# alipbcs/ZetaRay

Measured on AMD Instinct MI355X. Metric: Mrays/s, higher is better.
Workload: dtype f32; 1 GPU; Cornell Box (cornell_emissive: 58 triangles, 2 emissive) 1920x1080, G-buffer + ReSTIR PT (K1 + K11-K16: initial candidates, temporal + spatial reconnection reuse, boiling suppression; 3 non-transmissive / 4 glossy-transmissive bounces, static camera); integrator=restir_pt, parallelism=screen tiles (1, 1), settle_frames=32, ramp_frames=357, arith=contract, library=libzetaray_amd.so, frame_overlap=True, kernel_class=plain

## Files before the change

### include/zetaray_amd.h

```cpp
#ifndef ZETARAY_AMD_H
#define ZETARAY_AMD_H

#include <stddef.h>
#include <stdint.h>
#include "zr_wire.h"

#ifdef __cplusplus
extern "C" {
#endif

#define ZR_ABI_VERSION 3

typedef enum zr_status {
    ZR_OK = 0,
    ZR_ERR_INVALID_ARG = 1,
    ZR_ERR_NO_DEVICE = 2,
    ZR_ERR_HIP = 3,
    ZR_ERR_OOM = 4,
    ZR_ERR_UNSUPPORTED = 5,
    ZR_ERR_NOT_INITIALIZED = 6
} zr_status;

typedef struct zr_scene   zr_scene;
typedef struct zr_gbuffer zr_gbuffer;
// ... 125 lines not shown
    uint32_t width, height;
    void*    plane[ZR_GB_COUNT];
} zr_gbuffer_planes;

typedef struct zr_counters {
    uint64_t n_closest;
    uint64_t n_shadow;
} zr_counters;

int         zr_abi_version(void);
const char* zr_last_error(void);
int         zr_device_count(int* count);
typedef struct zr_device_probe {
    char     name[64], arch[32];
    uint32_t compute_units, clock_khz_max, mem_clock_khz_max, mem_bus_bits, l2_bytes, wall_clock_khz;
    uint64_t hbm_bytes;
    float    copy_GBs, copy_ms;
    float    fma_tflops, fma_ms;
    float    sclk_mhz_under_load;
} zr_device_probe;
int         zr_device_probe_run(int device, float min_ms, zr_device_probe* out);
int         zr_wire_layout(char* buf, size_t cap);

int zr_scene_create(int device, const zr_scene_desc* desc, zr_scene** out);
int zr_scene_destroy(zr_scene* scene);
int zr_scene_update_instances(zr_scene* scene, const zr_mesh_instance* instances, const float* instance_to_world, uint32_t n);
int zr_scene_update_emissives(zr_scene* scene, const zr_emissive_triangle* triangles, uint32_t first, uint32_t count);
int zr_scene_update_instances_async(zr_scene* scene, void* hip_stream, const zr_mesh_instance* instances, const float* instance_to_world, uint32_t n);
int zr_scene_set_background_rebuild(zr_scene* scene, int enable);
int zr_scene_background_rebuild_stats(zr_scene* scene, uint64_t* started, uint64_t* installed, int* building);
int zr_scene_update_emissives_async(zr_scene* scene, void* hip_stream, const zr_emissive_triangle* triangles, uint32_t first, uint32_t count);
int zr_scene_update_materials_async(zr_scene* scene, void* hip_stream, const zr_material* materials, uint32_t first, uint32_t count);
int zr_scene_set_alias_table_async(zr_scene* scene, void* hip_stream, const zr_alias_entry* entries, uint32_t n);
int zr_scene_set_object_emissives(zr_scene* scene, const zr_emissive_triangle* object_space, uint32_t n);
int zr_scene_has_object_emissives(const zr_scene* scene);
int zr_scene_move_instances_async(zr_scene* scene, void* hip_stream, const uint32_t* instance_idx, const float* world_3x4, uint32_t n_moved);
int zr_scene_move_instances(zr_scene* scene, const uint32_t* instance_idx, const float* world_3x4, uint32_t n_moved);
int zr_scene_get_instances(const zr_scene* scene, void* hip_stream, int which, zr_mesh_instance* out, float* to_world_or_null, uint32_t n);
int zr_scene_get_emissives(const zr_scene* scene, void* hip_stream, zr_emissive_triangle* out, uint32_t first, uint32_t count);
int zr_scene_invalidate_alias_table(zr_scene* scene);
int zr_scene_invalidate_alias_table_deferred(zr_scene* scene);
int zr_scene_update_materials(zr_scene* scene, const zr_material* materials, uint32_t first, uint32_t count);
int zr_scene_set_alias_table(zr_scene* scene, const zr_alias_entry* entries, uint32_t n);
int zr_alias_table_build(const float* power, uint32_t n, uint32_t align_phase, zr_alias_entry* out_entries);
int zr_scene_get_alias_table(const zr_scene* scene, zr_alias_entry* out_entries, uint32_t n);
int zr_scene_get_light_voxel_grid(const zr_scene* scene, void* hip_stream, zr_voxel_sample* out_samples, uint32_t n);
int zr_scene_get_presampled_sets(const zr_scene* scene, void* hip_stream, zr_presampled_tri* out_samples, uint32_t n);
int zr_scene_bvh_info(const zr_scene* scene, uint32_t* num_nodes, uint32_t* num_tris, uint32_t* max_depth);

int zr_gbuffer_create(int device, uint32_t width, uint32_t height, zr_gbuffer** out);
int zr_gbuffer_destroy(zr_gbuffer* gb);
int zr_gbuffer_set_tile_origin(zr_gbuffer* gb, uint32_t x0, uint32_t y0);
int zr_gbuffer_download(const zr_gbuffer* gb, void* hip_stream, zr_gbuffer_planes* host_planes);
int zr_gbuffer_device_plane(const zr_gbuffer* gb, int plane, void** dev_ptr);

int zr_params_default(zr_params* p);
int zr_pass_create(int kind, int device, zr_pass** out);
int zr_pass_init(zr_pass* pass, uint32_t width, uint32_t height, int integrator);
int zr_pass_resize(zr_pass* pass, uint32_t width, uint32_t height);
int zr_pass_reset_temporal(zr_pass* pass);
int zr_pass_pick_pixel(zr_pass* pass, uint32_t x, uint32_t y);
int zr_pass_clear_pick(zr_pass* pass);
int zr_pass_read_pick(zr_pass* pass, void* stream, uint32_t* mesh_idx);
int zr_pass_set_params(zr_pass* pass, const zr_params* params);
int zr_pass_render(zr_pass* pass, void* hip_stream, const zr_frame_constants* cb, const zr_scene* scene,
                   zr_gbuffer* gbuffer);
#define ZR_STAGE_TEMPORAL 1
#define ZR_STAGE_SPATIAL  2
#define ZR_STAGE_ALL      3
#define ZR_STAGE_SPATIAL2 4
#define ZR_STAGE_CANDIDATES     8
#define ZR_STAGE_TEMPORAL_REUSE 16
#define ZR_STAGE_DENOISE_TEMPORAL  (1 << 8)
#define ZR_STAGE_DENOISE_VARIANCE  (1 << 9)
#define ZR_STAGE_DENOISE_ATROUS(i) (1u << (10 + (i)))
#define ZR_STAGE_DENOISE_MASK      0x3ff00
#define ZR_HALO_POST_TEMPORAL 0
#define ZR_HALO_FINAL         1
#define ZR_HALO_DENOISE_INPUT 2
#define ZR_HALO_DENOISE_ITER  3
#define ZR_HALO_BYTES_PER_PIXEL 62
int zr_pass_set_owned_rect(zr_pass* pass, uint32_t x0, uint32_t y0, uint32_t width, uint32_t height);
#define ZR_FRAME_OVERLAP       1
#define ZR_FRAME_OVERLAP_CARRY 2
int zr_pass_set_frame_overlap(zr_pass* pass, zr_gbuffer* gbuffer, int enable);
int zr_pass_frame_overlap_stream(zr_pass* pass, void** hip_stream);
int zr_device_synchronize(int device);
int zr_pass_halo_bytes_per_pixel(zr_pass* pass, uint32_t* bytes);
int zr_pass_render_stage(zr_pass* pass, void* hip_stream, const zr_frame_constants* cb, const zr_scene* scene,
                         zr_gbuffer* gbuffer, int stages);
int zr_pass_halo_pack(zr_pass* pass, void* hip_stream, const zr_gbuffer* gbuffer, int which, uint32_t x0, uint32_t y0,
                      uint32_t width, uint32_t height, void* dev_dst, size_t bytes);
int zr_pass_halo_unpack(zr_pass* pass, void* hip_stream, const zr_gbuffer* gbuffer, int which, uint32_t x0, uint32_t y0,
                        uint32_t width, uint32_t height, const void* dev_src, size_t bytes);
#define ZR_HALO_MAX_RECTS 16
typedef struct zr_halo_rect { uint32_t x0, y0, w, h; uint64_t offset; } zr_halo_rect;
int zr_pass_halo_pack_all(zr_pass* pass, void* hip_stream, const zr_gbuffer* gbuffer, int which, const zr_halo_rect* rects, uint32_t num_rects,
                          void* dev_buf, size_t bytes);
int zr_pass_halo_unpack_all(zr_pass* pass, void* hip_stream, const zr_gbuffer* gbuffer, int which, const zr_halo_rect* rects, uint32_t num_rects,
                            const void* dev_buf, size_t bytes);
int zr_pass_get_output(const zr_pass* pass, int which, void** dev_ptr, uint32_t* width, uint32_t* height,
                       uint32_t* bytes_per_pixel);
int zr_pass_download_output(const zr_pass* pass, int which, void* hip_stream, void* host_dst, size_t bytes);
#define ZR_IN_EMISSIVE_DI 0
#define ZR_IN_INDIRECT    1
#define ZR_IN_SKY_DI      2
#define ZR_IN_TAA_SIGNAL  3
#define ZR_IN_POST_SIGNAL_F16  4
#define ZR_IN_POST_SIGNAL_F32  5
#define ZR_IN_DISPLAY_EXPOSURE 6
#define ZR_IN_DENOISE_SIGNAL   7
int zr_pass_set_input(zr_pass* pass, int which, const void* dev_plane);
int zr_pass_set_inscattering(zr_pass* sky, int enable, uint32_t voxels_x, uint32_t voxels_y, float depth_map_exp, float near_z, float far_z);
int zr_pass_bind_inscattering(zr_pass* compositing, const zr_pass* sky);
#define ZR_OUT_INSCATTERING 49
#define ZR_INSCATTERING_VOXELS_X 192
#define ZR_INSCATTERING_VOXELS_Y 108
int zr_pass_set_tonemap_lut(zr_pass* pass, const uint32_t* rgb9e5, uint32_t dim);
enum zr_display_option
{
    ZR_DISPLAY_DEFAULT = 0,
    ZR_DISPLAY_BASE_COLOR,
    ZR_DISPLAY_NORMAL,
    ZR_DISPLAY_METALNESS_ROUGHNESS,
    ZR_DISPLAY_COAT_WEIGHT,
    ZR_DISPLAY_COAT_COLOR,
    ZR_DISPLAY_ROUGHNESS_TH,
    ZR_DISPLAY_EMISSIVE,
    ZR_DISPLAY_TRANSMISSION,
    ZR_DISPLAY_DEPTH,
    ZR_DISPLAY_COUNT
};
int zr_pass_set_display_option(zr_pass* pass, int option, float roughness_th);
typedef enum zr_rpt_debug_view
{
    ZR_RPT_VIEW_NONE = 0,
    ZR_RPT_VIEW_K,
    ZR_RPT_VIEW_CASE,
    ZR_RPT_VIEW_FOUND_CONNECTION,
    ZR_RPT_VIEW_LOBE_K_MIN_1,
    ZR_RPT_VIEW_LOBE_K,
    ZR_RPT_VIEW_COUNT
} zr_rpt_debug_view;
int zr_pass_set_rpt_debug_view(zr_pass* pass, int view);
int zr_pass_set_rgi_spatial(zr_pass* pass, uint32_t num_samples, float radius_px);
int zr_pass_set_picked_instances(zr_pass* pass, const uint32_t* mesh_idx, uint32_t n);
#define ZR_OUT_PICK_MASK 50
int zr_pass_read_counters(zr_pass* pass, void* hip_stream, zr_counters* out, int reset);
#define ZR_COST_MAP_TIME 1
#define ZR_COST_MAP_RAYS 2
int zr_pass_enable_cost_map(zr_pass* pass, int enable);
int zr_pass_read_cost_map(zr_pass* pass, void* hip_stream, uint32_t* out_cells, uint32_t cells_w, uint32_t cells_h, int reset);
int zr_pass_debug_trip_stats(zr_pass* pass, uint64_t out[3]);
int zr_debug_set_large_scene_nodes(uint32_t num_nodes);
int zr_debug_set_bvh_depth_cap(uint32_t levels);
int zr_debug_set_material_class_kernels(int enable);
int zr_scene_material_class(const zr_scene* scene, uint32_t* out_class);
int zr_pass_read_kernel_counters(zr_pass* pass, void* hip_stream, uint32_t max_entries, const char** names,
                                 uint64_t* n_closest, uint64_t* n_shadow, uint32_t* count);
int zr_selftest_half_conversions(int device, uint64_t* mismatches_f32_to_f16, uint64_t* mismatches_f16_to_f32);

int zr_pass_enable_timing(zr_pass* pass, int enable);
int zr_pass_get_timings(zr_pass* pass, uint32_t max_entries, const char** names, float* ms, uint32_t* launches,
                        uint32_t* count);
int zr_pass_destroy(zr_pass* pass);

int zr_trace_closest(const zr_scene* scene, void* hip_stream, const float* d_rays, uint32_t n, uint32_t mask,
                     uint32_t* d_hits);
int zr_trace_any(const zr_scene* scene, void* hip_stream, const float* d_rays, uint32_t n, uint32_t mask,
                 uint32_t* d_occluded);

#ifdef __cplusplus
}
#endif

#endif
```

### zetaray_amd/api.py

```python
import ctypes as C
import os

import numpy as np

from . import wire

_HERE = os.path.dirname(os.path.abspath(__file__))
LIB_PATH = os.environ.get("ZETARAY_AMD_LIB", os.path.join(_HERE, "libzetaray_amd.so"))

PASS_GBUFFER, PASS_PRELIGHTING, PASS_DI_EMISSIVE, PASS_DI_SKY, PASS_INDIRECT, PASS_COMPOSITING, PASS_SKY, PASS_TAA, PASS_AUTO_EXPOSURE, PASS_DISPLAY, PASS_DENOISE = range(11)
IN_TAA_SIGNAL, OUT_TAA = 3, 41
IN_POST_SIGNAL_F16, IN_POST_SIGNAL_F32, IN_DISPLAY_EXPOSURE = 4, 5, 6
OUT_EXPOSURE, OUT_AE_HISTOGRAM, OUT_DISPLAY, OUT_DISPLAY_SRGB8 = 42, 43, 44, 45
IN_DENOISE_SIGNAL, OUT_DENOISED, OUT_DENOISE_HISTORY, OUT_DENOISE_MOMENTS = 7, 46, 47, 48
TONEMAP_LUT_PATH = os.path.join(_HERE, "assets", "tony_mc_mapface_rgb9e5.bin")


def load_tonemap_lut():
    lut = np.fromfile(TONEMAP_LUT_PATH, np.uint32)
    assert lut.size == 48 ** 3, lut.size
    return lut

OUT_SKY_LUT = 40
IN_EMISSIVE_DI, IN_INDIRECT, IN_SKY_DI = range(3)
INTEGRATOR_PATH_TRACING, INTEGRATOR_RESTIR_GI, INTEGRATOR_RESTIR_PT = range(3)
OUT_FINAL = 0
RPT_OUTPUTS_EXTRA = {"denoised": (46, np.float32, 4), "denoise_history": (47, np.float32, 4), "denoise_moments": (48, np.float32, 2),
                     "taa": (41, np.uint16, 4), "sky_lut": (40, np.uint32, 1), "sdi_A": (24, np.uint8, 1), "sdi_B": (25, np.uint16, 2), "sdi_C": (26, np.float32, 2),
                     "sdi_target": (27, np.float32, 4)}
RPT_OUTPUTS = {"A": (1, np.uint32, 1), "B": (2, np.float32, 2), "C": (3, np.uint32, 4), "D": (4, np.uint32, 4),
               "E": (5, np.uint16, 1), "F": (6, np.float32, 2), "G": (7, np.uint32, 2), "target": (8, np.float32, 4),
               "neighbor": (9, np.uint8, 2), "map_ctn": (18, np.uint16, 1), "map_ntc": (19, np.uint16, 1),
               "ctn_A": (10, np.uint16, 4), "ctn_B": (11, np.uint32, 4), "ctn_C": (12, np.uint32, 4), "ctn_D": (13, np.uint16, 1),
               "gi_A": (30, np.float32, 4), "gi_B": (31, np.uint16, 4), "gi_C": (32, np.float32, 4),
               "di_A": (20, np.uint32, 4), "di_B": (21, np.float32, 2), "di_target": (22, np.float32, 4),
               "ntc_A": (14, np.uint16, 4), "ntc_B": (15, np.uint32, 4), "ntc_C": (16, np.uint32, 4), "ntc_D": (17, np.uint16, 1)}

EXPORTS = [
    "zr_abi_version", "zr_last_error", "zr_device_count", "zr_device_probe_run", "zr_wire_layout", "zr_scene_create", "zr_scene_destroy", "zr_scene_update_instances", "zr_scene_update_emissives", "zr_scene_invalidate_alias_table", "zr_scene_update_materials",
    "zr_scene_set_background_rebuild", "zr_scene_background_rebuild_stats",
    "zr_scene_invalidate_alias_table_deferred", "zr_scene_update_instances_async", "zr_scene_update_emissives_async", "zr_scene_update_materials_async", "zr_scene_set_alias_table_async",
    "zr_scene_set_alias_table", "zr_alias_table_build", "zr_scene_get_alias_table", "zr_scene_get_light_voxel_grid", "zr_scene_get_presampled_sets", "zr_scene_bvh_info", "zr_pass_enable_cost_map", "zr_pass_read_cost_map", "zr_pass_debug_trip_stats", "zr_debug_set_large_scene_nodes", "zr_debug_set_bvh_depth_cap", "zr_debug_set_material_class_kernels", "zr_scene_material_class",
    "zr_gbuffer_create", "zr_gbuffer_destroy", "zr_gbuffer_set_tile_origin", "zr_gbuffer_download", "zr_gbuffer_device_plane",
    "zr_params_default", "zr_pass_create", "zr_pass_init", "zr_pass_resize", "zr_pass_reset_temporal", "zr_pass_pick_pixel", "zr_pass_clear_pick", "zr_pass_read_pick",
    "zr_pass_set_params", "zr_pass_render", "zr_pass_get_output", "zr_pass_download_output",
    "zr_pass_read_counters", "zr_pass_read_kernel_counters", "zr_pass_enable_timing", "zr_pass_get_timings", "zr_selftest_half_conversions", "zr_pass_destroy",
    "zr_trace_closest", "zr_trace_any",
    "zr_pass_set_owned_rect", "zr_pass_render_stage", "zr_pass_halo_pack", "zr_pass_halo_unpack", "zr_pass_halo_bytes_per_pixel", "zr_pass_set_input",
    "zr_pass_set_tonemap_lut", "zr_pass_halo_pack_all", "zr_pass_halo_unpack_all",
    "zr_pass_set_frame_overlap", "zr_pass_frame_overlap_stream", "zr_device_synchronize",
    "zr_pass_set_inscattering", "zr_pass_bind_inscattering",
    "zr_pass_set_display_option", "zr_pass_set_picked_instances",
    "zr_pass_set_rpt_debug_view",
    "zr_pass_set_rgi_spatial",
    "zr_scene_set_object_emissives", "zr_scene_has_object_emissives", "zr_scene_move_instances", "zr_scene_move_instances_async", "zr_scene_get_instances", "zr_scene_get_emissives",
]
STAGE_TEMPORAL, STAGE_SPATIAL, STAGE_ALL = 1, 2, 3
STAGE_SPATIAL2 = 4
STAGE_CANDIDATES, STAGE_TEMPORAL_REUSE = 8, 16
HALO_POST_TEMPORAL, HALO_FINAL = 0, 1
HALO_DENOISE_INPUT, HALO_DENOISE_ITER = 2, 3
STAGE_DENOISE_TEMPORAL, STAGE_DENOISE_VARIANCE, STAGE_DENOISE_MASK = 1 << 8, 1 << 9, 0x3ff00


def stage_denoise_atrous(i):
    return 1 << (10 + i)


class ZetaRayError(RuntimeError):
    def __init__(self, code, msg):
        super().__init__(f"zetaray_amd error {code}: {msg}")
        self.code = code


_LIB = None


def lib():
    global _LIB
    if _LIB is None:
        if not os.path.exists(LIB_PATH):
            raise ImportError(f"{LIB_PATH} is missing: build the HIP extension first "
                              f"(python -c 'import __graft_entry__ as g; g.build()'); there is no fallback path")
        try:
            import torch
        except ImportError:
            pass
        L = C.CDLL(LIB_PATH)
        L.zr_last_error.restype = C.c_char_p
        vp, u32, i32 = C.c_void_p, C.c_uint32, C.c_int
        L.zr_device_count.argtypes = [vp]
        L.zr_scene_create.argtypes = [i32, vp, vp]
        L.zr_scene_destroy.argtypes = [vp]
        L.zr_scene_set_alias_table.argtypes = [vp, vp, u32]
        L.zr_alias_table_build.argtypes = [vp, u32, u32, vp]
        L.zr_scene_get_alias_table.argtypes = [vp, vp, u32]
        L.zr_scene_get_light_voxel_grid.argtypes = [vp, vp, vp, u32]
        L.zr_scene_get_presampled_sets.argtypes = [vp, vp, vp, u32]
        L.zr_scene_bvh_info.argtypes = [vp, vp, vp, vp]
        L.zr_gbuffer_create.argtypes = [i32, u32, u32, vp]
        L.zr_gbuffer_destroy.argtypes = [vp]
        L.zr_gbuffer_set_tile_origin.argtypes = [vp, u32, u32]
        L.zr_gbuffer_download.argtypes = [vp, vp, vp]
        L.zr_gbuffer_device_plane.argtypes = [vp, i32, vp]
        L.zr_params_default.argtypes = [vp]
        L.zr_pass_create.argtypes = [i32, i32, vp]
        L.zr_pass_init.argtypes = [vp, u32, u32, i32]
        L.zr_pass_resize.argtypes = [vp, u32, u32]
        L.zr_pass_reset_temporal.argtypes = [vp]
        L.zr_pass_set_params.argtypes = [vp, vp]
        L.zr_pass_render.argtypes = [vp, vp, vp, vp, vp]
        L.zr_pass_get_output.argtypes = [vp, i32, vp, vp, vp, vp]
        L.zr_pass_download_output.argtypes = [vp, i32, vp, vp, C.c_size_t]
        L.zr_pass_read_counters.argtypes = [vp, vp, vp, i32]
        L.zr_pass_read_kernel_counters.argtypes = [vp, vp, u32, vp, vp, vp, vp]
        L.zr_pass_set_input.argtypes = [vp, i32, vp]
        L.zr_pass_set_inscattering.argtypes = [vp, i32, u32, u32, C.c_float, C.c_float, C.c_float]
        L.zr_pass_bind_inscattering.argtypes = [vp, vp]
        L.zr_pass_set_tonemap_lut.argtypes = [vp, vp, u32]
        L.zr_pass_set_display_option.argtypes = [vp, i32, C.c_float]
        L.zr_pass_set_picked_instances.argtypes = [vp, vp, u32]
        L.zr_pass_set_rpt_debug_view.argtypes = [vp, i32]
        L.zr_pass_set_rgi_spatial.argtypes = [vp, u32, C.c_float]
        L.zr_pass_halo_pack_all.argtypes = [vp, vp, vp, i32, vp, u32, vp, C.c_size_t]
        L.zr_pass_halo_unpack_all.argtypes = [vp, vp, vp, i32, vp, u32, vp, C.c_size_t]
        L.zr_pass_set_owned_rect.argtypes = [vp, u32, u32, u32, u32]
        L.zr_pass_render_stage.argtypes = [vp, vp, vp, vp, vp, i32]
        L.zr_pass_halo_pack.argtypes = [vp, vp, vp, i32, u32, u32, u32, u32, vp, C.c_size_t]
        L.zr_pass_halo_bytes_per_pixel.argtypes = [vp, vp]
        L.zr_pass_halo_unpack.argtypes = [vp, vp, vp, i32, u32, u32, u32, u32, vp, C.c_size_t]
        L.zr_pass_enable_timing.argtypes = [vp, i32]
        L.zr_pass_get_timings.argtypes = [vp, u32, vp, vp, vp, vp]
        L.zr_pass_destroy.argtypes = [vp]
        L.zr_pass_set_frame_overlap.argtypes = [vp, vp, i32]
        L.zr_pass_frame_overlap_stream.argtypes = [vp, vp]
        L.zr_device_synchronize.argtypes = [i32]
        L.zr_trace_closest.argtypes = [vp, vp, vp, u32, u32, vp]
        L.zr_trace_any.argtypes = [vp, vp, vp, u32, u32, vp]
        _LIB = L
    return _LIB


def _check(code):
    if code != 0:
        raise ZetaRayError(code, lib().zr_last_error().decode())


def device_count():
    n = C.c_int(0)
    _check(lib().zr_device_count(C.byref(n)))
    return n.value


def alias_table_build(power, align_phase=0):
    power = np.ascontiguousarray(power, np.float32)
    out = np.zeros(len(power), wire.ALIAS_ENTRY)
    _check(lib().zr_alias_table_build(power.ctypes.data, len(power), align_phase, out.ctypes.data))
    return out


class Scene:
    def __init__(self, scene, device=0):
        self.host = scene
        self._desc = scene.desc()
        self.h = C.c_void_p()
        self.version = 0
        self.instances_in_motion = self._records_in_motion(getattr(scene, "instances", None))
        _check(lib().zr_scene_create(device, C.addressof(self._desc), C.byref(self.h)))

    @staticmethod
    def _records_in_motion(instances):
        if instances is None or len(instances) == 0:
            return False
        i = np.asarray(instances)
        return bool(((i["d_translation"] & 0x7fff) != 0).any() or (i["prev_rotation"] != i["rotation"]).any() or (i["prev_scale"] != i["scale"]).any())

    def update_instances(self, instances, instance_to_world, stream=False):
        L = lib()
        self.version += 1
        i, x = np.ascontiguousarray(instances), np.ascontiguousarray(instance_to_world, np.float32)
        self.instances_in_motion = self._records_in_motion(i)
        if stream is False:
            L.zr_scene_update_instances.argtypes = [C.c_void_p, C.c_void_p, C.c_void_p, C.c_uint32]
            _check(L.zr_scene_update_instances(self.h, i.ctypes.data, x.ctypes.data, len(i)))
        else:
            L.zr_scene_update_instances_async.argtypes = [C.c_void_p, C.c_void_p, C.c_void_p, C.c_void_p, C.c_uint32]
            _check(L.zr_scene_update_instances_async(self.h, stream, i.ctypes.data, x.ctypes.data, len(i)))

    def set_object_emissives(self, tris):
        L = lib()
        t = np.ascontiguousarray(tris, wire.EMISSIVE_TRI)
        L.zr_scene_set_object_emissives.argtypes = [C.c_void_p, C.c_void_p, C.c_uint32]
        _check(L.zr_scene_set_object_emissives(self.h, t.ctypes.data, len(t)))

    def move_instances(self, idx, world, stream=False):
# ... 139 lines not shown

class Pass:

    def __init__(self, kind, width, height, integrator=INTEGRATOR_PATH_TRACING, device=0, params=None):
        self.kind = kind
        self.w, self.h_ = width, height
        self.h = C.c_void_p()
        _check(lib().zr_pass_create(kind, device, C.byref(self.h)))
        _check(lib().zr_pass_init(self.h, width, height, integrator))
        if params is not None:
            self.set_params(params)

    def set_params(self, params):
        _check(lib().zr_pass_set_params(self.h, C.addressof(params)))

    def resize(self, width, height):
        _check(lib().zr_pass_resize(self.h, width, height))
        self.w, self.h_ = width, height

    def reset_temporal(self):
        _check(lib().zr_pass_reset_temporal(self.h))

    def pick_pixel(self, x, y):
        L = lib()
        L.zr_pass_pick_pixel.argtypes = [C.c_void_p, C.c_uint32, C.c_uint32]
        _check(L.zr_pass_pick_pixel(self.h, int(x), int(y)))

    def clear_pick(self):
        L = lib()
        L.zr_pass_clear_pick.argtypes = [C.c_void_p]
        _check(L.zr_pass_clear_pick(self.h))

    def read_pick(self, stream=None):
        L = lib()
        L.zr_pass_read_pick.argtypes = [C.c_void_p, C.c_void_p, C.c_void_p]
        out = C.c_uint32(0)
        _check(L.zr_pass_read_pick(self.h, stream, C.byref(out)))
        return int(out.value)

    def render(self, cb, scene, gbuffer=None, stream=None):
        cbb = np.ascontiguousarray(cb)
        _check(lib().zr_pass_render(self.h, stream, cbb.ctypes.data, scene.h, gbuffer.h if gbuffer is not None else None))

    def render_stage(self, cb, scene, gbuffer, stages, stream=None):
        cbb = np.ascontiguousarray(cb)
        _check(lib().zr_pass_render_stage(self.h, stream, cbb.ctypes.data, scene.h, gbuffer.h if gbuffer is not None else None, stages))

    def set_input(self, which, dev_ptr):
        _check(lib().zr_pass_set_input(self.h, which, dev_ptr))

    def set_frame_overlap(self, gbuffer, on=1):
        _check(lib().zr_pass_set_frame_overlap(self.h, gbuffer.h, int(on)))

    def frame_overlap_stream(self):
        st = C.c_void_p()
        _check(lib().zr_pass_frame_overlap_stream(self.h, C.byref(st)))
        return st.value

    def set_tonemap_lut(self, lut=None):
        lut = np.ascontiguousarray(load_tonemap_lut() if lut is None else lut, np.uint32)
        dim = int(round(lut.size ** (1.0 / 3.0)))
        _check(lib().zr_pass_set_tonemap_lut(self.h, lut.ctypes.data, dim))

    def set_display_option(self, option, roughness_th=wire.DISPLAY_ROUGHNESS_TH_DEFAULT):
        _check(lib().zr_pass_set_display_option(self.h, int(option), float(roughness_th)))

    def set_rpt_debug_view(self, view):
        _check(lib().zr_pass_set_rpt_debug_view(self.h, int(view)))

    def set_rgi_spatial(self, num_samples, radius_px=0.0):
        _check(lib().zr_pass_set_rgi_spatial(self.h, int(num_samples), float(radius_px)))

    def set_picked_instances(self, mesh_idx):
        a = np.ascontiguousarray(mesh_idx, np.uint32).reshape(-1)
        _check(lib().zr_pass_set_picked_instances(self.h, a.ctypes.data if a.size else None, a.size))

    def download_raw(self, which, dtype, shape, stream=None):
        out = np.zeros(shape, dtype)
        _check(lib().zr_pass_download_output(self.h, which, stream, out.ctypes.data, out.nbytes))
        return out

    def set_owned_rect(self, x0, y0, w, h):
        _check(lib().zr_pass_set_owned_rect(self.h, x0, y0, w, h))

    def halo_pack(self, gbuffer, which, rect, dev_ptr, nbytes, stream=None):
        _check(lib().zr_pass_halo_pack(self.h, stream, gbuffer.h, which, rect[0], rect[1], rect[2], rect[3], dev_ptr, nbytes))

    def halo_all(self, gbuffer, which, rects, dev_ptr, nbytes, pack=True, stream=None):
        class Rect(C.Structure):
            _fields_ = [("x0", C.c_uint32), ("y0", C.c_uint32), ("w", C.c_uint32), ("h", C.c_uint32), ("offset", C.c_uint64)]
        arr = (Rect * max(1, len(rects)))(*[Rect(*r) for r in rects])
        f = lib().zr_pass_halo_pack_all if pack else lib().zr_pass_halo_unpack_all
        _check(f(self.h, stream, gbuffer.h, which, arr, len(rects), dev_ptr, nbytes))

    def halo_bytes_per_pixel(self):
        b = C.c_uint32()
        _check(lib().zr_pass_halo_bytes_per_pixel(self.h, C.byref(b)))
        return b.value

    def halo_unpack(self, gbuffer, which, rect, dev_ptr, nbytes, stream=None):
        _check(lib().zr_pass_halo_unpack(self.h, stream, gbuffer.h, which, rect[0], rect[1], rect[2], rect[3], dev_ptr, nbytes))

    def output_ptr(self, which=OUT_FINAL):
        dev = C.c_void_p()
        w, h, bpp = C.c_uint32(), C.c_uint32(), C.c_uint32()
        _check(lib().zr_pass_get_output(self.h, which, C.byref(dev), C.byref(w), C.byref(h), C.byref(bpp)))
        return dev.value, w.value, h.value, bpp.value

    def download(self, which=OUT_FINAL, stream=None):
        out = np.zeros((self.h_, self.w, 4), np.float32)
        _check(lib().zr_pass_download_output(self.h, which, stream, out.ctypes.data, out.nbytes))
        return out

    def set_inscattering(self, enable=True, voxels=wire.INSCATTERING_VOXELS, depth_map_exp=wire.INSCATTERING_DEPTH_MAP_EXP,
                         near_z=wire.INSCATTERING_NEAR_Z, far_z=wire.INSCATTERING_FAR_Z):
        _check(lib().zr_pass_set_inscattering(self.h, int(enable), int(voxels[0]), int(voxels[1]), float(depth_map_exp), float(near_z), float(far_z)))

    def bind_inscattering(self, sky_pass):
        _check(lib().zr_pass_bind_inscattering(self.h, sky_pass.h if sky_pass is not None else None))

    def download_plane(self, name, stream=None):
        if name == "pick_mask":
            _, w, h, _ = self.output_ptr(wire.OUT_PICK_MASK)
            out = np.zeros((h, w), np.uint8)
            _check(lib().zr_pass_download_output(self.h, wire.OUT_PICK_MASK, stream, out.ctypes.data, out.nbytes))
            return out
        if name == "inscattering":
            _, w, h, _ = self.output_ptr(wire.OUT_INSCATTERING)
            out = np.zeros((wire.INSCATTERING_SLICES, h // wire.INSCATTERING_SLICES, w), np.uint32)
            _check(lib().zr_pass_download_output(self.h, wire.OUT_INSCATTERING, stream, out.ctypes.data, out.nbytes))
            return out
        which, dt, ch = RPT_OUTPUTS[name] if name in RPT_OUTPUTS else RPT_OUTPUTS_EXTRA[name]
        out = np.zeros((self.h_, self.w, ch), dt)
        _check(lib().zr_pass_download_output(self.h, which, stream, out.ctypes.data, out.nbytes))
        return out

    def enable_cost_map(self, on=True):
        lib().zr_pass_enable_cost_map.argtypes = [C.c_void_p, C.c_int]
        _check(lib().zr_pass_enable_cost_map(self.h, int(on)))

    def read_cost_map(self, reset=True, stream=None):
        cw, ch = (self.w + 31) // 32 + 1, (self.h_ + 31) // 32 + 1
        out = np.zeros((ch, cw), np.uint32)
        lib().zr_pass_read_cost_map.argtypes = [C.c_void_p, C.c_void_p, C.c_void_p, C.c_uint32, C.c_uint32, C.c_int]
        _check(lib().zr_pass_read_cost_map(self.h, stream, out.ctypes.data, cw, ch, int(reset)))
        return out

    def debug_trip_stats(self):
        out = (C.c_uint64 * 3)()
        lib().zr_pass_debug_trip_stats.argtypes = [C.c_void_p, C.c_void_p]
        _check(lib().zr_pass_debug_trip_stats(self.h, out))
        return int(out[0]), int(out[1]), int(out[2])

    def read_counters(self, reset=True, stream=None):
        c = wire.Counters()
        _check(lib().zr_pass_read_counters(self.h, stream, C.addressof(c), int(reset)))
        return c.n_closest, c.n_shadow

    def kernel_counters(self, stream=None):
        n = 16
        names = (C.c_char_p * n)()
        a = (C.c_uint64 * n)()
        b = (C.c_uint64 * n)()
        cnt = C.c_uint32()
        _check(lib().zr_pass_read_kernel_counters(self.h, stream, n, names, a, b, C.byref(cnt)))
        return {names[i].decode(): (a[i], b[i]) for i in range(cnt.value)}

    def enable_timing(self, on=True):
        _check(lib().zr_pass_enable_timing(self.h, int(on)))

    def timings(self):
        n = 64
        names = (C.c_char_p * n)()
        ms = (C.c_float * n)()
        launches = (C.c_uint32 * n)()
        cnt = C.c_uint32()
        _check(lib().zr_pass_get_timings(self.h, n, names, ms, launches, C.byref(cnt)))
        return {names[i].decode(): (ms[i], launches[i]) for i in range(min(cnt.value, n))}

    def close(self):
        if self.h:
            lib().zr_pass_destroy(self.h)
            self.h = C.c_void_p()

    def __del__(self):
        try:
            self.close()
        except Exception:
            pass


class Renderer:

    def __init__(self, scene_host, width, height, device=0, params=None, integrator=INTEGRATOR_PATH_TRACING,
                 tile_origin=(0, 0)):
        self.scene = Scene(scene_host, device)
        self.scene_host = scene_host
        self.gbuffer = GBuffer(width, height, device)
        if tile_origin != (0, 0):
            self.gbuffer.set_tile_origin(*tile_origin)
        self.p_gbuffer = Pass(PASS_GBUFFER, width, height, device=device)
        self.p_prelight = Pass(PASS_PRELIGHTING, width, height, device=device, params=params)
        self._presampling = bool(params is not None and params.presampling)
        self.p_indirect = Pass(PASS_INDIRECT, width, height, integrator, device=device, params=params)
        self.p_sky = Pass(PASS_SKY, 256, 128, device=device) if len(scene_host.emissives) == 0 else None
        self.p_direct = None
        self.p_sky_direct = None
        self.skip_indirect = False
        self.p_composit = None
        self._alias_ready = False
        self._overlap_stream = None
        self._inscattering = False
        self._device = device

    def enable_frame_overlap(self, on=True, carry=False):
        assert self.p_direct is None and self.p_sky_direct is None and self.p_composit is None and getattr(self, "p_taa", None) is None, \
            "frame overlap covers GBuffer + PreLighting + Indirect (ReSTIR PT) [+ denoise]"
        _check(lib().zr_device_synchronize(self._device))
        self.p_indirect.set_frame_overlap(self.gbuffer, (2 if carry else 1) if on else 0)
        self._overlap_stream = self.p_indirect.frame_overlap_stream() if on else None

    def enable_compositing(self, device=0, firefly_filter=False):
        prm = None
        if firefly_filter:
            prm = wire.default_params()
            prm.flags |= wire.COMPOSIT_FIREFLY_FILTER
        self.p_composit = Pass(PASS_COMPOSITING, self.p_indirect.w, self.p_indirect.h_, device=device, params=prm)
        self._bind_post_inputs()
        return self.p_composit

    def enable_inscattering(self, voxels=wire.INSCATTERING_VOXELS, depth_map_exp=wire.INSCATTERING_DEPTH_MAP_EXP, near_z=wire.INSCATTERING_NEAR_Z,
                            far_z=wire.INSCATTERING_FAR_Z, device=0):
        assert self._overlap_stream is None, "frame overlap covers GBuffer + PreLighting + Indirect (ReSTIR PT) [+ denoise]"
        if self.p_sky is None:
            self.p_sky = Pass(PASS_SKY, 256, 128, device=device)
        self.p_sky.set_inscattering(True, voxels, depth_map_exp, near_z, far_z)
        if self.p_composit is None:
            self.enable_compositing(device=device)
        self.p_composit.bind_inscattering(self.p_sky)
        self._inscattering = True
        return self.p_sky

    def _bind_post_inputs(self):
        if self.p_composit is None:
            return
        self.p_composit.set_input(IN_INDIRECT, None if self.skip_indirect else self.p_indirect.output_ptr()[0])
        self.p_composit.set_input(IN_EMISSIVE_DI, self.p_direct.output_ptr()[0] if self.p_direct is not None else None)
        self.p_composit.set_input(IN_SKY_DI, self.p_sky_direct.output_ptr()[0] if self.p_sky_direct is not None else None)
        if getattr(self, "p_taa", None) is not None:
            self.p_taa.set_input(IN_TAA_SIGNAL, self.p_composit.output_ptr()[0])

    def enable_denoise(self, params=None, device=0):
        self.p_denoise = Pass(PASS_DENOISE, self.p_indirect.w, self.p_indirect.h_, device=device, params=params or wire.default_params())
        self.p_denoise.set_input(IN_DENOISE_SIGNAL, self.p_indirect.output_ptr()[0])
        return self.p_denoise

    def enable_taa(self, blend_weight=0.1, device=0):
        if self.p_composit is None:
            self.enable_compositing(device=device)
        prm = wire.default_params()
        prm.taa_blend_weight = blend_weight
        self.p_taa = Pass(PASS_TAA, self.p_indirect.w, self.p_indirect.h_, device=device, params=prm)
        self._bind_post_inputs()
        return self.p_taa

    def enable_sky_direct(self, params=None, device=0):
        if self.p_sky is None:
            self.p_sky = Pass(PASS_SKY, 256, 128, device=device)
        self.p_sky_direct = Pass(PASS_DI_SKY, self.p_indirect.w, self.p_indirect.h_, device=device, params=params)
        self._bind_post_inputs()
        return self.p_sky_direct

    def enable_direct(self, params=None, device=0):
        self.p_direct = Pass(PASS_DI_EMISSIVE, self.p_indirect.w, self.p_indirect.h_, device=device, params=params)
        self._bind_post_inputs()
        return self.p_direct

    def invalidate_alias_table(self, deferred=False):
        if deferred:
            self.scene.invalidate_alias_table_deferred()
            self._alias_poll = 8
            return
        self.scene.invalidate_alias_table()
        self._alias_ready = False

    def move_instances(self, idx, world, stream=False):
        self.scene.move_instances(idx, world, stream=stream)

    def set_rgi_spatial(self, num_samples, radius_px=0.0):
        self.p_indirect.set_rgi_spatial(num_samples, radius_px)

    _SKY_FIELDS = ("sun_dir", "sun_illuminance", "planet_radius", "atmosphere_altitude", "g", "rayleigh_sigma_s_color", "rayleigh_sigma_s_scale",
                   "ozone_sigma_a_color", "ozone_sigma_a_scale", "mie_sigma_s", "mie_sigma_a")

    def render_sky(self, cb, stream=None):
        if self.p_sky is None:
            return
        key = b"".join(np.asarray(cb[f]).tobytes() for f in self._SKY_FIELDS)
        if not self._inscattering:
            if key != getattr(self, "_sky_key", None):
                self.p_sky.render(cb, self.scene, None, stream)
                self._sky_key = key
            return
        if key != getattr(self, "_sky_key", None):
            self.p_sky.render_stage(cb, self.scene, None, STAGE_TEMPORAL, stream)
            self._sky_key = key
# ... 57 lines not shown
```

### zetaray_amd/csrc/zr_api.hip

```cpp
#include <hip/hip_runtime.h>
#include <immintrin.h>
#include <string>
#include <vector>
#include <cstdio>
#include <cstdarg>
#include <cstring>
#include <new>
#include <mutex>
#include "zr_stages.h"
#include "zr_rpt.h"
#include "zr_rdi.h"
#include "zr_sdi.h"
#include "zr_rgi.h"
#include "zr_rgi_spatial.h"
#include "zr_bvh.h"
#include "zr_taa.h"
#include "zr_svgf.h"
#include "zr_post.h"
#include "../../include/zr_srgb_table.h"

static const uint16_t kRptSampleSet[1024] = {
#include "zr_rpt_sample_set.inc"
};

// ... 598 lines not shown
    bool plainAt[3] = {true, true, true};
    uint64_t sceneAt[3] = {0, 0, 0};
    bool tracked = false;
    hipEvent_t evWritten = nullptr; hipStream_t writer = nullptr; bool hasWrite = false;
    struct Reader { hipStream_t st; hipEvent_t ev; };
    std::vector<Reader> readers[3];
    ~zr_gbuffer() { if (evWritten) (void)hipEventDestroy(evWritten); for (auto& v : readers) for (auto& r : v) (void)hipEventDestroy(r.ev); }
    DevBuf<uint8_t>* Planes() { return planeSets[cur]; }
    const DevBuf<uint8_t>* Planes() const { return planeSets[cur]; }
    GBuf View() const { return ViewOf(cur); }
    GBuf PrevView() const { return ViewOf(Prev()); }
    GBuf ViewOf(int which) const
    {
        const DevBuf<uint8_t>* planes = planeSets[which];
        GBuf g; g.w = w; g.h = h; g.x0 = x0; g.y0 = y0;
        g.baseColor = (uint32_t*)planes[ZR_GB_BASE_COLOR].p; g.normal = (uint32_t*)planes[ZR_GB_NORMAL].p;
        g.mr = (uint16_t*)planes[ZR_GB_METALLIC_ROUGHNESS].p; g.motion = (uint32_t*)planes[ZR_GB_MOTION_VECTOR].p;
        g.emissive = (uint32_t*)planes[ZR_GB_EMISSIVE_COLOR].p; g.ior = (uint8_t*)planes[ZR_GB_IOR].p;
        g.coat = (uint16_t*)planes[ZR_GB_COAT].p; g.depth = (float*)planes[ZR_GB_DEPTH].p;
        g.triA = (uint32_t*)planes[ZR_GB_TRI_DIFF_GEO_A].p; g.triB = (uint32_t*)planes[ZR_GB_TRI_DIFF_GEO_B].p;
        return g;
    }
};

static int GBufferMarkRead(zr_gbuffer* gb, int set, hipStream_t s)
{
    if (!gb || !gb->tracked) return ZR_OK;
    for (auto& r : gb->readers[set]) if (r.st == s) { HIP_TRY(hipEventRecord(r.ev, s)); return ZR_OK; }
    hipEvent_t ev; HIP_TRY(hipEventCreateWithFlags(&ev, hipEventDisableTiming));
    gb->readers[set].push_back({s, ev});
    HIP_TRY(hipEventRecord(ev, s));
    return ZR_OK;
}
static int GBufferAcquireRead(zr_gbuffer* gb, hipStream_t s)
{
    if (!gb || !gb->tracked || !gb->hasWrite || gb->writer == s) return ZR_OK;
    HIP_TRY(hipStreamWaitEvent(s, gb->evWritten, 0));
    return ZR_OK;
}
static int GBufferAcquireWrite(zr_gbuffer* gb, int set, hipStream_t s)
{
    if (!gb->tracked) return ZR_OK;
    for (auto& r : gb->readers[set]) if (r.st != s) HIP_TRY(hipStreamWaitEvent(s, r.ev, 0));
    return ZR_OK;
}
static int GBufferMarkWritten(zr_gbuffer* gb, hipStream_t s)
{
    if (!gb->tracked) return ZR_OK;
    if (!gb->evWritten) HIP_TRY(hipEventCreateWithFlags(&gb->evWritten, hipEventDisableTiming));
    HIP_TRY(hipEventRecord(gb->evWritten, s));
    gb->writer = s; gb->hasWrite = true;
    return ZR_OK;
}

struct QueueStorage
{
    DevBuf<U4> s0; DevBuf<F4> f[8]; DevBuf<F4> rays[6]; DevBuf<uint32_t> lightID; DevBuf<U4> hitC, hitM; DevBuf<uint32_t> visS, rayList;
    DevBuf<F4> t[8];
    int AllocTex(size_t cap)
    {
        int r;
        for (auto& b : t) if (b.n != cap && (r = b.Alloc(cap))) return r;
        return ZR_OK;
    }
    int Alloc(size_t cap)
    {
        int r;
        if ((r = s0.Alloc(cap))) return r;
        for (auto& b : f) if ((r = b.Alloc(cap))) return r;
        for (auto& b : rays) if ((r = b.Alloc(cap))) return r;
        if ((r = lightID.Alloc(cap))) return r;
        if ((r = hitC.Alloc(cap))) return r;
        if ((r = hitM.Alloc(cap))) return r;
        if ((r = visS.Alloc(cap))) return r;
        if ((r = rayList.Alloc(3 * cap))) return r;
        return ZR_OK;
    }
    PathQueue View() const
    {
        PathQueue q;
        q.s0 = s0.p; q.s1 = f[0].p; q.s2 = f[1].p; q.s3 = f[2].p; q.s4 = f[3].p; q.s5 = f[4].p; q.s6 = f[5].p; q.s7 = f[6].p; q.s8 = f[7].p;
        q.rayC_o = rays[0].p; q.rayC_d = rays[1].p; q.rayM_o = rays[2].p; q.rayM_d = rays[3].p; q.rayS_o = rays[4].p; q.rayS_d = rays[5].p;
        q.sLightID = lightID.p; q.hitC = hitC.p; q.hitM = hitM.p; q.visS = visS.p; q.rayList = rayList.p;
        for (int k = 0; k < 8; k++) q.t[k] = t[k].p;
        return q;
    }
};

static constexpr uint32_t kRptListWords = 12;
static constexpr uint32_t kLargeSceneNodes = 1;
static std::atomic<uint32_t> g_largeSceneNodes{kLargeSceneNodes};
static std::atomic<bool> g_materialClassKernels{true};
static bool PlainClass(const zr_scene* sc, const zr_gbuffer* gb)
{
    if (!sc->plainMaterials.load(std::memory_order_relaxed) || !g_materialClassKernels.load(std::memory_order_relaxed)) return false;
    const int c = gb->cur;
    if (!(gb->plainAt[c] && gb->sceneAt[c] == sc->uid)) return false;
    if (gb->numRendered >= 2 && !(gb->plainAt[gb->Prev()] && gb->sceneAt[gb->Prev()] == sc->uid)) return false;
    return true;
}
static constexpr int kMaxRounds = 16;
static constexpr int kMaxTimers = 64;
static constexpr int kCounterSlots = 16;
static const char* const kCounterNames[kCounterSlots] = {"trace", "rpt_pathtrace", "rpt_replay_ctt", "rpt_replay_ttc", "rpt_reconnect_temporal",
    "rpt_replay_cts", "rpt_replay_stc", "rpt_reconnect_spatial", "rdi_temporal", "rdi_spatial", "rgi", "sdi_temporal", "sdi_spatial", "rgi_spatial", "", ""};

struct zr_pass
{
    int kind = 0, device = 0, integrator = 0;
    bool initialized = false;
    uint32_t w = 0, h = 0;
    zr_params params{};
    QueueStorage q[2];
    DevBuf<uint32_t> skyLut;
    bool inscatterOn = false; InscatterParams inscatter{}; DevBuf<uint32_t> inscatterGrid;
    const zr_pass* inscatterSky = nullptr;
    Plane<float, 4> finalRGBA; Plane<F4> firstBOP; DevBuf<uint32_t> counts; DevBuf<unsigned long long> counters;
    DevBuf<uint32_t> groupMax;
    zr_counters hostCounters{0, 0};
    uint32_t pickXY = 0xffffffffu; DevBuf<uint32_t> pickBuf; bool pickWritten = false;
    struct ResStorage
    {
        Plane<uint32_t> A; Plane<float, 2> B; Plane<U4> C, D; Plane<uint16_t> E; Plane<float, 2> F; Plane<uint32_t, 2> G;
        template<typename S, typename Fn> static int Each(S& s, Fn f)
        { int r; if ((r = f(s.A)) || (r = f(s.B)) || (r = f(s.C)) || (r = f(s.D)) || (r = f(s.E)) || (r = f(s.F)) || (r = f(s.G))) return r; return ZR_OK; }
        rpt::ResPlanes View() const { rpt::ResPlanes v; v.A = A.p; v.B = B.p; v.C = C.p; v.D = D.p; v.E = E.p; v.F = F.p; v.G = G.p; return v; }
    } res[3];
    struct RBufStorage
    {
        Plane<uint16_t, 4> A; Plane<U4> B, C; Plane<uint16_t> D;
        template<typename S, typename Fn> static int Each(S& s, Fn f) { int r; if ((r = f(s.A)) || (r = f(s.B)) || (r = f(s.C)) || (r = f(s.D))) return r; return ZR_OK; }
        rpt::RBuf View() const { rpt::RBuf v; v.A = A.p; v.B = B.p; v.C = C.p; v.D = D.p; return v; }
    } rb[2];
    Plane<F4> rptTarget, rptTargetAlt; Plane<uint8_t, 2> rptNeighbor; DevBuf<uint16_t> rptSampleSet;
    bool overlap = false, overlapCarry = false; int rptSet[3] = {0, 1, 2}; int tgtIdx = 0, finIdx = 0, finOut = 0;
    Plane<float, 4> finalAlt, finalAlt2;
    hipEvent_t evDone[2] = {nullptr, nullptr}; bool haveDone[2] = {false, false}; hipStream_t doneStream[2] = {nullptr, nullptr}; uint64_t ovFrame = 0;
    hipStream_t overlapStream = nullptr;
    hipEvent_t evCand = nullptr, evTemporal = nullptr;
    hipStream_t candStream = nullptr, reuseStream = nullptr; bool haveCand = false, haveTemporal = false;
    zr_pass::ResStorage& RptCur() { return res[rptSet[currIdx]]; }
    zr_pass::ResStorage& RptOth() { return res[rptSet[1 - currIdx]]; }
    const zr_pass::ResStorage& RptOth() const { return res[rptSet[1 - currIdx]]; }
    const Plane<F4>& TargetPlane() const { return tgtIdx ? rptTargetAlt : rptTarget; }
    const Plane<float, 4>& FinalPlane(int i) const { return i == 0 ? finalRGBA : (i == 1 ? finalAlt : finalAlt2); }
    F4* Target() const { return TargetPlane().p; }
    float* Final(int i) const { return FinalPlane(i).p; }
    Plane<uint16_t> rptMap[2];
    DevBuf<uint32_t> trip; DevBuf<unsigned long long> tripStats;
    DevBuf<uint32_t> carry[2], carryCount;
    bool frameOpen = false;
    DevBuf<uint32_t> costMap; bool costOn = false, costRays = false;
    DevBuf<uint32_t> rptLists, rptListCounts;
    Plane<U4> diA[2]; Plane<float, 2> diB[2]; Plane<F4> diTarget; DevBuf<uint16_t> diSampleSet;
    Plane<uint8_t> skyA[2]; Plane<uint16_t, 2> skyB[2]; Plane<float, 2> skyC[2];
    Plane<F4> giA[2], giC[2]; Plane<uint16_t, 4> giB[2];
    bool temporalValid = false, doTemporal = false, doSpatial = false; int currIdx = 0;
    const F4* compIn[4] = {nullptr, nullptr, nullptr, nullptr};
    Plane<F4> svgfHist, svgfAccum, svgfPing, svgfPong; Plane<float, 2> svgfMoments[2]; Plane<float> svgfGuideFw; Plane<svgf::GuideN> svgfGuide; int svgfMomIdx = 0; const F4* svgfOut = nullptr; F4* svgfCur = nullptr; uint32_t svgfStepsDone = 0;
    Plane<uint16_t, 4> taaOut[2]; int taaIdx = 0;
    const uint16_t* postIn16 = nullptr; const F4* postIn32 = nullptr; const float* exposureIn = nullptr;
    DevBuf<uint32_t> aeHist; DevBuf<float> aeExposure;
    DevBuf<uint32_t> tonemapLut; uint32_t tonemapLutDim = 0; Plane<F4> displayOut; Plane<uint32_t> displaySrgb;
    int displayOption = ZR_DISPLAY_DEFAULT; float roughnessTh = 1.0f;
    int rptView = ZR_RPT_VIEW_NONE, rptViewFrame = ZR_RPT_VIEW_NONE;
    rgi::SpatialParams rgiSpatial{0u, rgi::kSpatialDefaultRadius}, rgiSpatialFrame{0u, rgi::kSpatialDefaultRadius}; Plane<float, 4> rgiScratch;
    std::vector<uint32_t> picks; DevBuf<uint8_t> pickMask; DevBuf<int4> pickTris; DevBuf<uint32_t> pickCount;
    uint32_t pickMaskW = 0, pickMaskH = 0;
    uint32_t own[4] = {0, 0, 0, 0};
    DevBuf<float> power;
    float* powerHost = nullptr; size_t powerHostCap = 0; hipEvent_t powerEv = nullptr; bool powerPending = false;
    bool timing = false;
    struct Timer { const char* name; hipEvent_t a, b; bool used; };
    std::vector<Timer> timers;
    int numTimers = 0;
    std::vector<std::string> timerNames; std::vector<float> timerMs; std::vector<uint32_t> timerLaunches;
};

static void TimerBegin(zr_pass* p, hipStream_t s, const char* name)
{
    if (!p->timing) return;
    if (p->numTimers >= (int)p->timers.size())
    {
        zr_pass::Timer t; t.name = name; t.used = false;
        if (hipEventCreate(&t.a) != hipSuccess || hipEventCreate(&t.b) != hipSuccess) return;
        p->timers.push_back(t);
    }
    zr_pass::Timer& t = p->timers[p->numTimers];
    t.name = name; t.used = true;
    (void)hipEventRecord(t.a, s);
}
static void TimerEnd(zr_pass* p, hipStream_t s)
{
    if (!p->timing) return;
    if (p->numTimers >= (int)p->timers.size()) return;
    (void)hipEventRecord(p->timers[p->numTimers].b, s);
    p->numTimers++;
}

static float KahanSumAVX2(const float* data, int64_t N, int64_t phase)
{
    float sum = 0.0f, compensation = 0.0f;
    const int64_t start = phase < N ? phase : N;
    for (int64_t i = 0; i < start; i++)
    {
        volatile float corrected = data[i] - compensation;
        volatile float newSum = sum + corrected;
        compensation = (newSum - sum) - corrected;
        sum = newSum;
    }
    int64_t numSimd = (N - start);
    numSimd -= numSimd & 15;
    __m256 vSum = _mm256_setzero_ps(), vComp = _mm256_setzero_ps();
    for (int64_t c = start; c < start + numSimd; c += 16)
    {
        __m256 V1 = _mm256_loadu_ps(data + c), V2 = _mm256_loadu_ps(data + c + 8);
        __m256 vCurr = _mm256_add_ps(V1, V2);
        __m256 vCorrected = _mm256_sub_ps(vCurr, vComp);
        __m256 vNewSum = _mm256_add_ps(vSum, vCorrected);
        vComp = _mm256_sub_ps(vNewSum, vSum);
        vComp = _mm256_sub_ps(vComp, vCorrected);
        vSum = vNewSum;
    }
    alignas(32) float simdSum[8], simdComp[8];
    _mm256_store_ps(simdSum, vSum); _mm256_store_ps(simdComp, vComp);
    for (int i = 0; i < 8; i++)
    {
        volatile float corrected = simdSum[i] - compensation - simdComp[i];
        volatile float newSum = sum + corrected;
        compensation = (newSum - sum) - corrected;
        sum = newSum;
    }
    for (int64_t i = start + numSimd; i < N; i++)
    {
        volatile float corrected = data[i] - compensation;
        volatile float newSum = sum + corrected;
        compensation = (newSum - sum) - corrected;
        sum = newSum;
    }
    return sum;
}

static void BuildAliasTableHost(std::vector<float>& probs, zr_alias_entry* table, uint32_t phase)
{
    const int64_t N = (int64_t)probs.size();
    const float oneDivN = 1.0f / (float)N;
    const float sum = KahanSumAVX2(probs.data(), N, phase);
    const float sumRcp = (float)N / sum;
    for (int64_t i = 0; i < N; i++) probs[i] *= sumRcp;
    for (int64_t i = 0; i < N; i++) { table[i].cached_p_orig = probs[i] * oneDivN; table[i].alias = 0xffffffffu; table[i].p_curr = 0.0f; }
    std::vector<uint32_t> larger, smaller;
    larger.reserve(N); smaller.reserve(N);
    for (int64_t i = 0; i < N; i++) (probs[i] < 1.0f ? smaller : larger).push_back((uint32_t)i);
    while (!smaller.empty() && !larger.empty())
    {
        const uint32_t si = smaller.back(); smaller.pop_back();
        const float sp = probs[si];
        const uint32_t li = larger.back();
        float lp = probs[li];
        table[si].alias = li; table[si].p_curr = sp;
        lp = (sp + lp) - 1.0f;
        probs[li] = lp;
        if (lp < 1.0f) { larger.pop_back(); smaller.push_back(li); }
    }
    for (; !larger.empty(); larger.pop_back()) { table[larger.back()].alias = larger.back(); table[larger.back()].p_curr = 1.0f; }
    for (; !smaller.empty(); smaller.pop_back()) { table[smaller.back()].alias = smaller.back(); table[smaller.back()].p_curr = 1.0f; }
    for (int64_t i = 0; i < N; i++) table[i].cached_p_alias = table[table[i].alias].cached_p_orig;
}

__global__ void __launch_bounds__(256) k_refit_tris(BvhTri* tris, uint32_t n, const TriMeta* meta, const zr_mesh_instance* instances, const float* toWorld,
    const zr_vertex* vertices, const uint32_t* indices)
{
    const uint32_t i = blockIdx.x * blockDim.x + threadIdx.x;
    if (i >= n) return;
    BvhTri t = tris[i];
    const TriMeta tm = meta[t.gidx];
    const zr_mesh_instance mi = instances[tm.mesh];
    const float* M = toWorld + 12 * (size_t)tm.mesh;
    float w[3][3];
    for (int k = 0; k < 3; k++)
    {
        const uint32_t vi = indices[mi.base_idx_offset + 3 * tm.prim + k] + mi.base_vtx_offset;
        const float* P = vertices[vi].pos;
        for (int r = 0; r < 3; r++) w[k][r] = M[4 * r + 0] * P[0] + M[4 * r + 1] * P[1] + M[4 * r + 2] * P[2] + M[4 * r + 3];
    }
    for (int r = 0; r < 3; r++) { t.v0[r] = w[0][r]; t.e1[r] = w[1][r] - w[0][r]; t.e2[r] = w[2][r] - w[0][r]; }
    tris[i] = t;
}
__global__ void __launch_bounds__(256) k_install_topology(Bvh4Node* nodes, const uint32_t* children, uint32_t numNodes, BvhTri* tris, const uint32_t* slotTri, uint32_t numTris,
    const TriMeta* meta, const uint8_t* instanceMask)
{
    const uint32_t i = blockIdx.x * blockDim.x + threadIdx.x;
    if (i < numNodes)
    {
        const uint4 c = ((const uint4*)children)[i];
        Bvh4Node N; N.ox = N.oy = N.oz = 0.0f; N.exps = 0; N.child[0] = c.x; N.child[1] = c.y; N.child[2] = c.z; N.child[3] = c.w;
        N.qlox = N.qloy = N.qloz = N.qhix = N.qhiy = N.qhiz = 0; N.pad0 = 0; N.pad1 = 0;
        nodes[i] = N;
    }
    if (i < numTris)
    {
        const uint32_t g = slotTri[i];
        const TriMeta tm = meta[g];
        BvhTri t; for (int r = 0; r < 3; r++) { t.v0[r] = 0.0f; t.e1[r] = 0.0f; t.e2[r] = 0.0f; }
        t.gidx = g; t.mask = instanceMask[tm.mesh]; t.id = TriID(tm.mesh, tm.prim);
        tris[i] = t;
// ... 1356 lines not shown
        TimerBegin(p, s, "sdi_spatial");
        hipLaunchKernelGGL(plainDi ? k_sdi_spatial<true> : k_sdi_spatial<false>, dim3(grid.x * (256 / kSdiBlock)), dim3(kSdiBlock), 0, s, F, *cb, tilesX, p->counters.p + 2 * 12);
        TimerEnd(p, s);
    }
    HIP_TRY(hipGetLastError());
    p->temporalValid = true;
    p->currIdx = 1 - p->currIdx;
    return ZR_OK;
}

static int RenderReSTIR_GI(zr_pass* p, hipStream_t s, const zr_frame_constants* cb, const zr_scene* sc, zr_gbuffer* gb, int stages)
{
    using namespace rgi;
    const zr_params& ip = p->params;
    GiFrame F;
    F.sc = FrameView(sc, cb); F.gb = gb->View(); F.gbPrev = gb->PrevView();
    F.sc.texFilter = ip.tex_filter;
    if (int orc = ResolveOwnedRect(p, gb, cb, &F.ox0, &F.oy0, &F.ow, &F.oh)) return orc;
    GiParams& prm = F.prm;
    prm.flags = ip.flags; prm.maxNonTrBounces = ip.max_non_tr_bounces; prm.maxGlossyTrBounces = ip.max_glossy_tr_bounces;
    prm.numSampleSets = ip.presampling ? ip.num_sample_sets : 0u;
    prm.accumulate = (cb->accumulate && cb->camera_static) ? 1u : 0u;
    prm.M_max = (float)ip.m_max_temporal;
    prm.useLVG = (ip.use_lvg && ip.presampling) ? 1u : 0u;
    prm.textured = sc->view.tex.count ? 1u : 0u;
    const uint32_t tilesX = (F.ow + 15) / 16, tilesY = (F.oh + 15) / 16;
    if (stages & ZR_STAGE_TEMPORAL)
    {
        p->rgiSpatialFrame = p->rgiSpatial;
        const bool spatial = p->rgiSpatialFrame.numSamples != 0;
        F.cur.A = p->giA[p->currIdx].p; F.cur.B = p->giB[p->currIdx].p; F.cur.C = p->giC[p->currIdx].p;
        F.prev.A = p->giA[1 - p->currIdx].p; F.prev.B = p->giB[1 - p->currIdx].p; F.prev.C = p->giC[1 - p->currIdx].p;
        F.finalRGBA = p->finalRGBA.p;
        prm.doTemporal = ((ip.flags & ZR_IND_TEMPORAL_RESAMPLE) && p->temporalValid && gb->numRendered >= 2) ? 1u : 0u;
        prm.writeReservoirs = (prm.doTemporal || !p->temporalValid) ? 1u : 0u;
        if (spatial)
        {
            const size_t cap = (size_t)p->w * p->h;
            if (p->rgiScratch.Pixels() != cap) { int r; if ((r = p->rgiScratch.Alloc(cap))) return r; HIP_TRY(hipMemsetAsync(p->rgiScratch.p, 0, cap * p->rgiScratch.bpp, s)); }
            F.finalRGBA = p->rgiScratch.p; prm.accumulate = 0u; prm.writeReservoirs = 1u;
        }
        if (prm.useLVG && !sc->view.lvg) return Fail(ZR_ERR_NOT_INITIALIZED, "light voxel grid missing: render the PRELIGHTING pass with use_lvg first");
        TimerBegin(p, s, "rgi");
        hipLaunchKernelGGL(sc->view.tex.count ? k_rgi_tex : PlainClass(sc, gb) ? k_rgi<true> : k_rgi<false>, dim3(tilesX * tilesY * (256 / kRgiBlock)), dim3(kRgiBlock), 0, s, F, *cb, tilesX, p->counters.p + 2 * 10);
        TimerEnd(p, s);
        HIP_TRY(hipGetLastError());
        p->temporalValid = true;
        p->currIdx = 1 - p->currIdx;
    }
    if ((stages & ZR_STAGE_SPATIAL) && p->rgiSpatialFrame.numSamples != 0)
    {
        if (!p->temporalValid) return Fail(ZR_ERR_NOT_INITIALIZED, "ReSTIR GI: ZR_STAGE_SPATIAL before the frame's ZR_STAGE_TEMPORAL");
        const int set = 1 - p->currIdx;
        F.cur.A = p->giA[set].p; F.cur.B = p->giB[set].p; F.cur.C = p->giC[set].p; F.prev = F.cur;
        F.finalRGBA = p->finalRGBA.p;
        prm.accumulate = (cb->accumulate && cb->camera_static) ? 1u : 0u;
        prm.doTemporal = 0u; prm.writeReservoirs = 0u; prm.textured = 0u;
        TimerBegin(p, s, "rgi_spatial");
        hipLaunchKernelGGL(k_rgi_spatial, dim3(tilesX * tilesY), dim3(kBlock), 0, s, F, *cb, tilesX, p->counters.p + 2 * 13, p->rgiSpatialFrame);
        TimerEnd(p, s);
        HIP_TRY(hipGetLastError());
    }
    return ZR_OK;
}

__global__ void __launch_bounds__(256) k_rpt_carry(rpt::ResPlanes dst, rpt::ResPlanes src, F4* tdst, const F4* tsrc, size_t n)
{
    for (size_t i = (size_t)blockIdx.x * blockDim.x + threadIdx.x; i < n; i += (size_t)gridDim.x * blockDim.x)
    {
        dst.A[i] = src.A[i]; dst.B[2 * i] = src.B[2 * i]; dst.B[2 * i + 1] = src.B[2 * i + 1]; dst.C[i] = src.C[i]; dst.D[i] = src.D[i]; dst.E[i] = src.E[i];
        dst.F[2 * i] = src.F[2 * i]; dst.F[2 * i + 1] = src.F[2 * i + 1]; dst.G[2 * i] = src.G[2 * i]; dst.G[2 * i + 1] = src.G[2 * i + 1];
        tdst[i] = tsrc[i];
    }
}
static bool FewerRoundsAtFourWaves(uint32_t waves)
{
    static const bool off = [] { const char* e = ZR_EXP_ENV("ZR_K11_ROUNDS"); return e && !strcmp(e, "0"); }();
    return !off && waves > 3072u && waves <= 4096u;
}

static int RenderReSTIR_PT(zr_pass* p, hipStream_t s, const zr_frame_constants* cb, const zr_scene* sc, zr_gbuffer* gb, int stages)
{
    using namespace rpt;
    const zr_pass::ResStorage* carryFrom = nullptr;
    const bool stageCand = (stages & (ZR_STAGE_TEMPORAL | ZR_STAGE_CANDIDATES)) != 0, stageReuseT = (stages & (ZR_STAGE_TEMPORAL | ZR_STAGE_TEMPORAL_REUSE)) != 0;
    if (stageCand && p->overlap)
    {
        if (!gb->tracked || gb->numSets < 3) return Fail(ZR_ERR_INVALID_ARG, "ReSTIR PT with frame overlap: this G-buffer is not the one given to zr_pass_set_frame_overlap (call it again with the new G-buffer)");
        if (p->frameOpen) return Fail(ZR_ERR_INVALID_ARG, "ReSTIR PT with frame overlap: the previous frame's last stage has not been enqueued (stage order: CANDIDATES, TEMPORAL_REUSE, SPATIAL[, SPATIAL2])");
        std::swap(p->rptSet[p->currIdx], p->rptSet[2]);
        p->tgtIdx ^= 1;
        carryFrom = p->overlapCarry ? &p->res[p->rptSet[2]] : nullptr;
        if (!(cb->accumulate && cb->camera_static)) p->finIdx = (p->finIdx + 1) % 3;
        if (p->overlapCarry)
        {
            if (p->haveTemporal && p->reuseStream != s) HIP_TRY(hipStreamWaitEvent(s, p->evTemporal, 0));
        }
        else
        {
            const int k = (int)(p->ovFrame & 1);
            if (p->haveDone[k] && p->doneStream[k] != s) HIP_TRY(hipStreamWaitEvent(s, p->evDone[k], 0));
        }
    }
    RptFrame F;
    F.sc = FrameView(sc, cb); F.gb = gb->View(); F.gbPrev = gb->PrevView();
    F.scPrev = FrameViewPrev(sc, cb);
    F.sc.texFilter = F.scPrev.texFilter = p->params.tex_filter;
    if (int orc = ResolveOwnedRect(p, gb, cb, &F.ox0, &F.oy0, &F.ow, &F.oh)) return orc;
    F.rbCtN = p->rb[0].View(); F.rbNtC = p->rb[1].View(); F.tex.target = p->Target(); F.tex.neighbor = p->rptNeighbor.p;
    F.finalRGBA = p->Final(p->finIdx); F.sampleSet = p->rptSampleSet.p;
    F.mapCtN = p->rptMap[0].p; F.mapNtC = p->rptMap[1].p;
    F.costMap = p->costOn ? p->costMap.p : nullptr; F.costW = (p->w + 31u) / 32u + 1u; F.costMode = p->costRays ? 1u : 0u;
    F.trip = nullptr; F.tripStats = nullptr; F.tripStride = 0;
    F.carryOut = nullptr; F.carryIn = nullptr; F.carryCount = nullptr; F.carryCap = 0; F.carryBounce = 0;
    if (((F.ox0 + F.ow) & 31u) && F.ox0 + F.ow != cb->render_width) return Fail(ZR_ERR_INVALID_ARG, "ReSTIR PT: the owned rect must end on a 32-pixel boundary or at the right edge of the render target");
    if (((F.oy0 + F.oh) & 31u) && F.oy0 + F.oh != cb->render_height) return Fail(ZR_ERR_INVALID_ARG, "ReSTIR PT: the owned rect must end on a 32-pixel boundary or at the bottom edge of the render target");
    RptParams& prm = F.prm;
    const zr_params& ip = p->params;
    const bool havePrevGBuffer = gb->numRendered >= 2;
    prm.maxNonTrBounces = ip.max_non_tr_bounces; prm.maxGlossyTrBounces = ip.max_glossy_tr_bounces;
    prm.russianRoulette = (ip.flags & ZR_IND_RUSSIAN_ROULETTE) ? 1u : 0u;
    prm.numSampleSets = ip.presampling ? ip.num_sample_sets : 0u;
    prm.accumulate = (cb->accumulate && cb->camera_static) ? 1u : 0u;
    prm.boiling = (ip.flags & ZR_IND_BOILING_SUPPRESSION) ? 1u : 0u;
    prm.M_max_temporal = ip.m_max_temporal & 0xf; prm.M_max_spatial = ip.m_max_spatial & 0xf; prm.alpha_min = ip.alpha_min;
    prm.emissive = cb->num_emissive_triangles ? 1u : 0u;
    prm.textured = sc->view.tex.count ? 1u : 0u;
    prm.sortTemporal = (ip.flags & ZR_IND_SORT_TEMPORAL) ? 1u : 0u; prm.sortSpatial = (ip.flags & ZR_IND_SORT_SPATIAL) ? 1u : 0u;
    static const uint32_t temporalMapEnv = [] { const char* e = ZR_EXP_ENV("ZR_TEMPORAL_MAP"); return e ? (uint32_t)atoi(e) : 1u; }();
    prm.temporalMap = prm.sortTemporal ? temporalMapEnv : 0u;
    if (stageCand)
    {
        p->rptViewFrame = p->rptView;
        p->doTemporal = (ip.flags & ZR_IND_TEMPORAL_RESAMPLE) && p->temporalValid && havePrevGBuffer;
        p->doSpatial = (ip.flags & ZR_IND_SPATIAL_RESAMPLE) && p->doTemporal && ip.num_spatial_passes > 0;
    }
    if (ip.num_spatial_passes > 2u) return Fail(ZR_ERR_INVALID_ARG, "ReSTIR PT: num_spatial_passes must be 0, 1 or 2");
    const uint32_t numSpatialPasses = ip.num_spatial_passes;
    prm.doTemporal = p->doTemporal ? 1u : 0u;
    prm.doSpatial = p->doSpatial ? 1u : 0u;
    prm.writeReservoirs = (prm.doTemporal || !p->temporalValid) ? 1u : 0u;
    F.cur = p->RptCur().View(); F.prev = p->RptOth().View();
    const uint32_t tilesX = (F.ow + 15) / 16, tilesY = (F.oh + 15) / 16;
    const dim3 grid(tilesX * tilesY), block(kBlock);
    const dim3 gridRpt(tilesX * tilesY * (256 / kRptBlock)), blockRpt(kRptBlock);
    const dim3 gridRecon(tilesX * tilesY * (256 / kReconBlock)), blockRecon(kReconBlock);
    const dim3 gridStc(tilesX * tilesY * (256 / kStcBlock)), blockStc(kStcBlock);
    const uint32_t sortTilesX = (F.ow + 31) / 32;
    const dim3 gridSort(sortTilesX * ((F.oh + 31) / 32));
    uint32_t* listCnt = p->rptListCounts.p;
    const size_t cap = (size_t)p->w * p->h;
    uint32_t* lists[4] = {p->rptLists.p, p->rptLists.p + cap, p->rptLists.p + 2 * cap, p->rptLists.p + 3 * cap};
    const dim3 gridList((uint32_t)std::min<size_t>((cap + kBlock - 1) / kBlock, 1024));
    const dim3 gridLight((tilesX * tilesY + kLightTilesPerBlock - 1u) / kLightTilesPerBlock), gridSearch((tilesX * tilesY + kSearchTilesPerBlock - 1u) / kSearchTilesPerBlock);
    const dim3 gridReplay((uint32_t)std::min<size_t>((cap + kBlock - 1) / kBlock, kReplayPersistentBlocks));
    unsigned long long* ctr = p->counters.p;
#define RPT_TIMED(name, ...) do { TimerBegin(p, s, name); __VA_ARGS__; TimerEnd(p, s); } while (0)
    const bool emissiveVariant = prm.emissive != 0;
    const uint32_t largeSceneNodes = g_largeSceneNodes.load(std::memory_order_relaxed);
    const bool texVariant = prm.textured != 0;
    const bool plainVariant = PlainClass(sc, gb) && !texVariant;
#define RPT_LAUNCH_E(kern, ...) do { \
        if (plainVariant) { if (emissiveVariant) hipLaunchKernelGGL((kern<true, false, true>), __VA_ARGS__); else hipLaunchKernelGGL((kern<false, false, true>), __VA_ARGS__); } \
        else if (emissiveVariant) { if (texVariant) hipLaunchKernelGGL((kern<true, true, false>), __VA_ARGS__); else hipLaunchKernelGGL((kern<true, false, false>), __VA_ARGS__); } \
        else { if (texVariant) hipLaunchKernelGGL((kern<false, true, false>), __VA_ARGS__); else hipLaunchKernelGGL((kern<false, false, false>), __VA_ARGS__); } } while (0)
#define RPT_LAUNCH_PE(kern, PASS, ...) do { \
        if (emissiveVariant) { if (texVariant) hipLaunchKernelGGL((kern<PASS, true, true>), __VA_ARGS__); else hipLaunchKernelGGL((kern<PASS, true, false>), __VA_ARGS__); } \
        else { if (texVariant) hipLaunchKernelGGL((kern<PASS, false, true>), __VA_ARGS__); else hipLaunchKernelGGL((kern<PASS, false, false>), __VA_ARGS__); } } while (0)
    const uint32_t view = (uint32_t)p->rptViewFrame;
#define RPT_LAUNCH_VIEW(kern, ...) do { \
        if (emissiveVariant) { if (texVariant) hipLaunchKernelGGL((kern<true, true>), __VA_ARGS__, view); else hipLaunchKernelGGL((kern<true, false>), __VA_ARGS__, view); } \
        else { if (texVariant) hipLaunchKernelGGL((kern<false, true>), __VA_ARGS__, view); else hipLaunchKernelGGL((kern<false, false>), __VA_ARGS__, view); } } while (0)
    if (stageCand)
    {
        if (int ar = GBufferAcquireRead(gb, s)) return ar;
        if (carryFrom)
        {
            const size_t n = (size_t)p->w * p->h;
            RPT_TIMED("rpt_overlap_carry", hipLaunchKernelGGL(k_rpt_carry, dim3((uint32_t)std::min<size_t>((n + 255) / 256, 4096)), dim3(256), 0, s, F.cur, carryFrom->View(), p->Target(),
                (const F4*)(p->tgtIdx ? p->rptTarget.p : p->rptTargetAlt.p), n));
        }
        TimerBegin(p, s, "rpt_pathtrace");
        if (view != ZR_RPT_VIEW_NONE) RPT_LAUNCH_VIEW(k_rpt_pathtrace_view, gridRpt, blockRpt, 0, s, F, *cb, tilesX, ctr + 2 * 1);
        else
        {
#ifdef ZR_EXPERIMENTS
        static const int k11Mode = [] { const char* e = getenv("ZR_K11"); return e && !strcmp(e, "inline") ? 0 : (e && !strcmp(e, "pool") ? 1 : (e && !strcmp(e, "trip") ? 2 : (e && !strcmp(e, "compact") ? 3 : ZR_K11_DEFAULT))); }();
        static const bool park = [] { const char* e = getenv("ZR_K11_PARK"); return e ? atoi(e) != 0 : (ZR_K11_PARK_DEFAULT != 0); }();
        if (k11Mode == 1 && emissiveVariant && !texVariant)
        {
            const dim3 gridCoop(tilesX * tilesY), blockCoop(kCoopBlock);
            if (sc->view.numNodes >= largeSceneNodes) hipLaunchKernelGGL(k_rpt_pathtrace_coop_w4<false>, gridCoop, blockCoop, 0, s, F, *cb, tilesX, ctr + 2 * 1);
            else hipLaunchKernelGGL(k_rpt_pathtrace_coop<false>, gridCoop, blockCoop, 0, s, F, *cb, tilesX, ctr + 2 * 1);
        }
        else if (k11Mode == 3 && !texVariant)
        {
            const size_t cap = (size_t)F.gb.w * F.gb.h;
            if (p->carry[0].n != cap * rpt::kPtCarryWords) { int rr; for (int k = 0; k < 2; k++) if ((rr = p->carry[k].Alloc(cap * rpt::kPtCarryWords))) return rr; if ((rr = p->carryCount.Alloc(16))) return rr; }
            HIP_TRY(hipMemsetAsync(p->carryCount.p, 0, 16 * sizeof(uint32_t), s));
            uint32_t maxB = prm.maxNonTrBounces > prm.maxGlossyTrBounces ? prm.maxNonTrBounces : prm.maxGlossyTrBounces;
            if (prm.russianRoulette && maxB > 3u) maxB = 3u;
            F.carryCap = cap; F.carryCount = p->carryCount.p; F.carryBounce = 0; F.carryOut = p->carry[0].p; F.carryIn = nullptr;
            if (emissiveVariant) hipLaunchKernelGGL(k_rpt_pt_first<true>, gridRpt, blockRpt, 0, s, F, *cb, tilesX, ctr + 2 * 1);
            else hipLaunchKernelGGL(k_rpt_pt_first<false>, gridRpt, blockRpt, 0, s, F, *cb, tilesX, ctr + 2 * 1);
            const dim3 gridNext((uint32_t)((cap + kRptBlock - 1) / kRptBlock));
            for (uint32_t b = 1; b + 1 <= maxB && b < 15u; b++)
            {
                F.carryBounce = b; F.carryIn = p->carry[(b - 1) & 1].p; F.carryOut = p->carry[b & 1].p;
                if (emissiveVariant) hipLaunchKernelGGL(k_rpt_pt_next<true>, gridNext, blockRpt, 0, s, F, *cb, tilesX, ctr + 2 * 1);
                else hipLaunchKernelGGL(k_rpt_pt_next<false>, gridNext, blockRpt, 0, s, F, *cb, tilesX, ctr + 2 * 1);
            }
        }
        else if (k11Mode == 2 && emissiveVariant && !texVariant)
        {
            const size_t stride = (size_t)F.gb.w * F.gb.h;
            if (!p->trip.p) { int rr; if ((rr = p->trip.Alloc(stride * rpt::kPtCarryWords))) return rr; if ((rr = p->tripStats.Alloc(4))) return rr; HIP_TRY(hipMemsetAsync(p->tripStats.p, 0, 32, s)); }
            F.trip = p->trip.p; F.tripStats = p->tripStats.p; F.tripStride = stride;
            if (sc->view.numNodes >= largeSceneNodes) hipLaunchKernelGGL(k_rpt_pathtrace_trip_w4<false>, gridRpt, blockRpt, 0, s, F, *cb, tilesX, ctr + 2 * 1);
            else hipLaunchKernelGGL(k_rpt_pathtrace_trip<false>, gridRpt, blockRpt, 0, s, F, *cb, tilesX, ctr + 2 * 1);
        }
        else if (k11Mode == 0 && park && !texVariant && !(sc->view.numNodes >= largeSceneNodes || FewerRoundsAtFourWaves(gridRpt.x)))
        { if (emissiveVariant) hipLaunchKernelGGL(k_rpt_pathtrace_park<true>, gridRpt, blockRpt, 0, s, F, *cb, tilesX, ctr + 2 * 1); else hipLaunchKernelGGL(k_rpt_pathtrace_park<false>, gridRpt, blockRpt, 0, s, F, *cb, tilesX, ctr + 2 * 1); }
        else
#endif
        if (texVariant) { if (emissiveVariant) hipLaunchKernelGGL(k_rpt_pathtrace_tex<true>, gridRpt, blockRpt, 0, s, F, *cb, tilesX, ctr + 2 * 1); else hipLaunchKernelGGL(k_rpt_pathtrace_tex<false>, gridRpt, blockRpt, 0, s, F, *cb, tilesX, ctr + 2 * 1); }
        else if (sc->view.numNodes >= largeSceneNodes || FewerRoundsAtFourWaves(gridRpt.x))
        {
            if (plainVariant) { if (emissiveVariant) hipLaunchKernelGGL((k_rpt_pathtrace_w4<true, true>), gridRpt, blockRpt, 0, s, F, *cb, tilesX, ctr + 2 * 1); else hipLaunchKernelGGL((k_rpt_pathtrace_w4<false, true>), gridRpt, blockRpt, 0, s, F, *cb, tilesX, ctr + 2 * 1); }
            else if (emissiveVariant) hipLaunchKernelGGL((k_rpt_pathtrace_w4<true, false>), gridRpt, blockRpt, 0, s, F, *cb, tilesX, ctr + 2 * 1); else hipLaunchKernelGGL((k_rpt_pathtrace_w4<false, false>), gridRpt, blockRpt, 0, s, F, *cb, tilesX, ctr + 2 * 1);
        }
        else
        {
            if (plainVariant) { if (emissiveVariant) hipLaunchKernelGGL((k_rpt_pathtrace<true, true>), gridRpt, blockRpt, 0, s, F, *cb, tilesX, ctr + 2 * 1); else hipLaunchKernelGGL((k_rpt_pathtrace<false, true>), gridRpt, blockRpt, 0, s, F, *cb, tilesX, ctr + 2 * 1); }
            else if (emissiveVariant) hipLaunchKernelGGL((k_rpt_pathtrace<true, false>), gridRpt, blockRpt, 0, s, F, *cb, tilesX, ctr + 2 * 1); else hipLaunchKernelGGL((k_rpt_pathtrace<false, false>), gridRpt, blockRpt, 0, s, F, *cb, tilesX, ctr + 2 * 1);
        }
        }
        TimerEnd(p, s);
        if (p->overlap) { HIP_TRY(hipEventRecord(p->evCand, s)); p->candStream = s; p->haveCand = true; }
    }
    if (stageReuseT)
    {
        if (p->overlap && p->haveCand && p->candStream != s) HIP_TRY(hipStreamWaitEvent(s, p->evCand, 0));
        else if (int ar = GBufferAcquireRead(gb, s)) return ar;
        HIP_TRY(hipMemsetAsync(listCnt, 0, kRptListWords * sizeof(uint32_t), s));
        if (prm.doTemporal)
        {
            RPT_TIMED("rpt_sort_temporal", hipLaunchKernelGGL((k_rpt_sort<rpt::RPT_SORT_TTC, rpt::RPT_SORT_CTT>), dim3(gridSort.x * 2), dim3(256), 0, s, F, *cb, sortTilesX, F.ox0 / 32u, F.oy0 / 32u, F.mapNtC, F.mapCtN));
            RPT_TIMED("rpt_classify_temporal", hipLaunchKernelGGL(k_rpt_light<0>, gridLight, block, 0, s, F, *cb, tilesX, lists[0], lists[1], listCnt + 0));
            RPT_TIMED("rpt_replay_temporal", RPT_LAUNCH_PE(k_rpt_replay, RPT_REPLAY_CTT, gridReplay, block, 0, s, F, *cb, lists[0], lists[1], listCnt + 0, ctr + 2 * 2));
            if (view != ZR_RPT_VIEW_NONE) RPT_TIMED("rpt_reconnect_temporal", RPT_LAUNCH_VIEW(k_rpt_temporal_view, gridRecon, blockRecon, 0, s, F, *cb, tilesX, ctr + 2 * 4));
            else RPT_TIMED("rpt_reconnect_temporal", RPT_LAUNCH_E(k_rpt_temporal, gridRecon, blockRecon, 0, s, F, *cb, tilesX, ctr + 2 * 4));
        }
        if (p->overlap) { HIP_TRY(hipEventRecord(p->evTemporal, s)); p->reuseStream = s; p->haveTemporal = true; }
        if (int mr = GBufferMarkRead(gb, gb->Prev(), s)) return mr;
    }
    for (uint32_t spass = 0; spass < numSpatialPasses && prm.doSpatial; spass++)
    {
        if (!(stages & (spass == 0 ? ZR_STAGE_SPATIAL : ZR_STAGE_SPATIAL2))) continue;
        F.cur = p->RptCur().View(); F.prev = p->RptOth().View();
        uint32_t* const sCnt = listCnt + (spass == 0 ? 2 : 6);
#ifdef ZR_EXPERIMENTS
        static const bool searchTile = [] { const char* e = getenv("ZR_SEARCH"); return e && !strcmp(e, "tile"); }();
        if (searchTile) RPT_TIMED("rpt_spatial_search", hipLaunchKernelGGL(k_rpt_light<2>, grid, block, 0, s, F, *cb, tilesX, lists[2], lists[3], sCnt));
        else
#endif
        RPT_TIMED("rpt_spatial_search", hipLaunchKernelGGL(k_rpt_light<1>, gridSearch, block, 0, s, F, *cb, tilesX, lists[2], lists[3], sCnt));
        if (prm.sortSpatial)
        {
            RPT_TIMED("rpt_sort_spatial", hipLaunchKernelGGL((k_rpt_sort<rpt::RPT_SORT_CTS, rpt::RPT_SORT_STC>), dim3(gridSort.x * 2), dim3(256), 0, s, F, *cb, sortTilesX, F.ox0 / 32u, F.oy0 / 32u, F.mapCtN, F.mapNtC));
        }
        RPT_TIMED("rpt_replay_spatial", RPT_LAUNCH_PE(k_rpt_replay, RPT_REPLAY_CTS, dim3(gridList.x * 2), block, 0, s, F, *cb, lists[2], lists[3], sCnt, ctr + 2 * 5));
        if (view != ZR_RPT_VIEW_NONE) RPT_TIMED("rpt_reconnect_spatial", RPT_LAUNCH_VIEW(k_rpt_stc_view, gridStc, blockStc, 0, s, F, *cb, tilesX, ctr + 2 * 7));
        else RPT_TIMED("rpt_reconnect_spatial", RPT_LAUNCH_E(k_rpt_stc, gridStc, blockStc, 0, s, F, *cb, tilesX, ctr + 2 * 7));
        p->currIdx = 1 - p->currIdx;
    }
#undef RPT_TIMED
#undef RPT_LAUNCH_E
#undef RPT_LAUNCH_PE
#undef RPT_LAUNCH_VIEW
    HIP_TRY(hipGetLastError());
    if (stageCand) p->frameOpen = true;
    const bool lastStage = (prm.doSpatial && numSpatialPasses == 2u) ? (stages & ZR_STAGE_SPATIAL2) != 0 : (stages & ZR_STAGE_SPATIAL) != 0;
    if (lastStage && p->frameOpen)
    {
        p->temporalValid = true;
        p->currIdx = 1 - p->currIdx;
        p->frameOpen = false;
        p->finOut = p->finIdx;
        if (p->overlap) { const int k = (int)(p->ovFrame & 1); HIP_TRY(hipEventRecord(p->evDone[k], s)); p->haveDone[k] = true; p->doneStream[k] = s; p->ovFrame++; }
        if (int mr = GBufferMarkRead(gb, gb->cur, s)) return mr;
    }
    return ZR_OK;
}

static int RenderIndirect(zr_pass* p, hipStream_t s, const zr_frame_constants* cb, const zr_scene* sc, zr_gbuffer* gb, int stages)
{
    if (!gb) return Fail(ZR_ERR_INVALID_ARG, "INDIRECT pass needs a gbuffer");
    if (gb->w != p->w || gb->h != p->h || gb->x0 + gb->w > cb->render_width || gb->y0 + gb->h > cb->render_height)
        return Fail(ZR_ERR_INVALID_ARG, "frame constants / gbuffer tile / pass size mismatch");
    if (sc->view.numEmissives == 0)
    {
        if (!sc->view.sky.data) return Fail(ZR_ERR_NOT_INITIALIZED, "sky-view LUT missing: render a ZR_PASS_SKY pass first");
    }
    else if (!sc->view.alias) return Fail(ZR_ERR_NOT_INITIALIZED, "emissive alias table missing: render the PRELIGHTING pass (or zr_scene_set_alias_table) first");
    if (cb->num_emissive_triangles != sc->view.numEmissives) return Fail(ZR_ERR_INVALID_ARG, "cbFrameConstants.NumEmissiveTriangles != scene");
    if (p->params.presampling && (!sc->view.sampleSets || sc->numSampleSets != p->params.num_sample_sets || sc->view.sampleSetSize != p->params.sample_set_size))
        return Fail(ZR_ERR_NOT_INITIALIZED, "presampled light sets missing or of another size: render the PRELIGHTING pass with the same presampling params first");
    if (p->integrator == ZR_INTEGRATOR_RESTIR_PT) return RenderReSTIR_PT(p, s, cb, sc, gb, stages);
    if (p->integrator == ZR_INTEGRATOR_RESTIR_GI) return RenderReSTIR_GI(p, s, cb, sc, gb, stages);
    if (!(stages & ZR_STAGE_TEMPORAL)) return ZR_OK;
    PtParams prm;
    prm.maxNonTrBounces = p->params.max_non_tr_bounces; prm.maxGlossyTrBounces = p->params.max_glossy_tr_bounces;
    prm.russianRoulette = (p->params.flags & ZR_IND_RUSSIAN_ROULETTE) ? 1u : 0u;
    prm.numSampleSets = p->params.presampling ? p->params.num_sample_sets : 0u;
    prm.accumulate = (cb->accumulate && cb->camera_static) ? 1u : 0u;
    prm.tileW = p->w; prm.groupsX = (p->w + 7) / 8;
    const uint32_t numGroups = prm.groupsX * ((p->h + 7) / 8);
    const uint32_t maxB = prm.maxNonTrBounces > prm.maxGlossyTrBounces ? prm.maxNonTrBounces : prm.maxGlossyTrBounces;
    const int rounds = (int)maxB + 1;
    if (rounds > kMaxRounds) return Fail(ZR_ERR_INVALID_ARG, "too many bounces");

    HIP_TRY(hipMemsetAsync(p->counts.p, 0, 5 * (kMaxRounds + 2) * kCounterStride * sizeof(uint32_t), s));
    auto Ctr = [&](int kind, int round) { return p->counts.p + ((size_t)round * 5 + kind) * kCounterStride; };
    const bool rrPossible = prm.russianRoulette && maxB >= 4;
    if (rrPossible) HIP_TRY(hipMemsetAsync(p->groupMax.p, 0, (size_t)rounds * numGroups * sizeof(uint32_t), s));
    const uint32_t tilesX = (p->w + 15) / 16, tilesY = (p->h + 15) / 16;
    const GBuf gbv = gb->View();
    SceneView scv = FrameView(sc, cb);
    scv.texFilter = p->params.tex_filter;
    const bool tex = scv.tex.count != 0;
    const bool plainPt = PlainClass(sc, gb);
    if (tex) { int r; if ((r = p->q[0].AllocTex((size_t)p->w * p->h)) || (r = p->q[1].AllocTex((size_t)p->w * p->h))) return r; }
    TimerBegin(p, s, "pt_init");
    hipLaunchKernelGGL((tex ? k_pt_init<true, false> : plainPt ? k_pt_init<false, true> : k_pt_init<false, false>), dim3(tilesX * tilesY), dim3(kBlock), 0, s, scv, *cb, gbv, prm, p->finalRGBA.p, p->firstBOP.p,
        p->q[0].View(), Ctr(0, 0), Ctr(2, 0), (uint32_t)((size_t)p->w * p->h), tilesX);
    TimerEnd(p, s);
    const size_t cap = (size_t)p->w * p->h;
    const uint32_t gridShade = (uint32_t)std::min<size_t>((cap + kBlock - 1) / kBlock, 4096);
    const uint32_t gridTrace = (uint32_t)std::min<size_t>((3 * cap + kBlock - 1) / kBlock, 2048);
    const uint32_t gridTraceSimple = (uint32_t)std::min<size_t>((3 * cap + kBlock - 1) / kBlock, 8192);
    static const int traceMode = [] { const char* e = ZR_EXP_ENV("ZR_TRACE_MODE"); return e ? atoi(e) : 0; }();
    for (int r = 0; r < rounds; r++)
    {
        const PathQueue qin = p->q[r & 1].View(), qout = p->q[(r + 1) & 1].View();
        TimerBegin(p, s, "trace");
        if (traceMode == 0) hipLaunchKernelGGL(k_trace_simple, dim3(gridTraceSimple), dim3(kBlock), 0, s, scv, qin, Ctr(2, r), (uint32_t)cap, p->counters.p);
        else hipLaunchKernelGGL(k_trace, dim3(gridTrace), dim3(kBlock), 0, s, scv, qin, Ctr(2, r), (uint32_t)cap, Ctr(1, r), p->counters.p);
        TimerEnd(p, s);
        TimerBegin(p, s, "pt_shade");
        hipLaunchKernelGGL(tex ? k_pt_shade_tex : plainPt ? k_pt_shade<true> : k_pt_shade<false>, dim3(gridShade), dim3(kBlock), 0, s, scv, *cb, prm, qin, Ctr(0, r), qout, Ctr(0, r + 1), Ctr(2, r + 1), (uint32_t)cap,
            p->finalRGBA.p, p->firstBOP.p, p->groupMax.p + (size_t)r * numGroups);
        TimerEnd(p, s);
        if (rrPossible && r >= 2)
        {
            TimerBegin(p, s, "pt_rr");
            hipLaunchKernelGGL(tex ? k_pt_rr<true> : k_pt_rr<false>, dim3(gridShade), dim3(kBlock), 0, s, scv, prm, qout, Ctr(0, r + 1), Ctr(2, r + 1), (uint32_t)cap, p->groupMax.p + (size_t)r * numGroups);
            TimerEnd(p, s);
        }
    }
    HIP_TRY(hipGetLastError());
    return ZR_OK;
}

int zr_pass_render(zr_pass* p, void* stream, const zr_frame_constants* cb, const zr_scene* sc, zr_gbuffer* gb)
{ return zr_pass_render_stage(p, stream, cb, sc, gb, ZR_STAGE_ALL | ZR_STAGE_SPATIAL2); }

int zr_pass_set_input(zr_pass* p, int which, const void* dev)
{
    if (p && p->kind == ZR_PASS_TAA && which == ZR_IN_TAA_SIGNAL) { p->compIn[3] = (const F4*)dev; return ZR_OK; }
    if (p && p->kind == ZR_PASS_DENOISE && which == ZR_IN_DENOISE_SIGNAL) { p->compIn[3] = (const F4*)dev; return ZR_OK; }
    if (p && (p->kind == ZR_PASS_AUTO_EXPOSURE || p->kind == ZR_PASS_DISPLAY))
    {
        if (which == ZR_IN_POST_SIGNAL_F16) { p->postIn16 = (const uint16_t*)dev; p->postIn32 = nullptr; return ZR_OK; }
        if (which == ZR_IN_POST_SIGNAL_F32) { p->postIn32 = (const F4*)dev; p->postIn16 = nullptr; return ZR_OK; }
        if (which == ZR_IN_DISPLAY_EXPOSURE && p->kind == ZR_PASS_DISPLAY) { p->exposureIn = (const float*)dev; return ZR_OK; }
        return Fail(ZR_ERR_INVALID_ARG, "zr_pass_set_input: bad input id for an AUTO_EXPOSURE / DISPLAY pass");
    }
    if (!p || p->kind != ZR_PASS_COMPOSITING || which < 0 || which > 2) return Fail(ZR_ERR_INVALID_ARG, "zr_pass_set_input: not a COMPOSITING / TAA pass or bad input id");
    p->compIn[which] = (const F4*)dev;
    return ZR_OK;
}
extern "C" int zr_pass_set_inscattering(zr_pass* p, int enable, uint32_t voxels_x, uint32_t voxels_y, float depth_map_exp, float near_z, float far_z)
{
    if (!p || p->kind != ZR_PASS_SKY) return Fail(ZR_ERR_INVALID_ARG, "zr_pass_set_inscattering: needs a SKY pass");
    if (!p->initialized) return Fail(ZR_ERR_NOT_INITIALIZED, "zr_pass_set_inscattering: pass not initialised (zr_pass_init)");
    HIP_TRY(hipSetDevice(p->device));
    if (!enable)
    {
        p->inscatterOn = false; p->inscatterGrid.Free();
        return ZR_OK;
    }
    if (voxels_x == 0 && voxels_y == 0) { voxels_x = ZR_INSCATTERING_VOXELS_X; voxels_y = ZR_INSCATTERING_VOXELS_Y; }
    if (voxels_x == 0 || voxels_y == 0 || voxels_x > 4096 || voxels_y > 4096)
        return Fail(ZR_ERR_INVALID_ARG, "zr_pass_set_inscattering: voxel counts %u x %u outside 1..4096 (0 x 0 = the default)", voxels_x, voxels_y);
    if (!(depth_map_exp >= 1.0f && depth_map_exp <= 5.0f))
        return Fail(ZR_ERR_INVALID_ARG, "zr_pass_set_inscattering: depth_map_exp %g outside 1..5", (double)depth_map_exp);
    if (!(near_z >= 0.0f && near_z < far_z && far_z <= ZR_FLT_MAX))
        return Fail(ZR_ERR_INVALID_ARG, "zr_pass_set_inscattering: needs 0 <= near_z < far_z (got %g, %g)", (double)near_z, (double)far_z);
    const size_t n = (size_t)voxels_x * voxels_y * kInscatterSlices;
    if (!p->inscatterOn || p->inscatterGrid.n != n)
    {
        int r; if ((r = p->inscatterGrid.Alloc(n))) { p->inscatterOn = false; return r; }
        HIP_TRY(hipMemset(p->inscatterGrid.p, 0, n * sizeof(uint32_t)));
    }
    p->inscatter.numVoxelsX = voxels_x; p->inscatter.numVoxelsY = voxels_y;
    p->inscatter.depthMappingExp = depth_map_exp; p->inscatter.nearZ = near_z; p->inscatter.farZ = far_z;
    p->inscatterOn = true;
    return ZR_OK;
}
extern "C" int zr_pass_bind_inscattering(zr_pass* p, const zr_pass* sky)
{
    if (!p || p->kind != ZR_PASS_COMPOSITING) return Fail(ZR_ERR_INVALID_ARG, "zr_pass_bind_inscattering: needs a COMPOSITING pass");
    if (sky && sky->kind != ZR_PASS_SKY) return Fail(ZR_ERR_INVALID_ARG, "zr_pass_bind_inscattering: the grid comes from a SKY pass");
    p->inscatterSky = sky;
    return ZR_OK;
}
extern "C" int zr_pass_set_tonemap_lut(zr_pass* p, const uint32_t* rgb9e5, uint32_t dim)
{
    if (!p || p->kind != ZR_PASS_DISPLAY || !rgb9e5 || dim == 0 || dim > 256) return Fail(ZR_ERR_INVALID_ARG, "zr_pass_set_tonemap_lut: needs a DISPLAY pass and a dim^3 LUT");
    HIP_TRY(hipSetDevice(p->device));
    const size_t n = (size_t)dim * dim * dim;
    int r; if ((r = p->tonemapLut.Alloc(n))) return r;
    HIP_TRY(hipMemcpy(p->tonemapLut.p, rgb9e5, n * sizeof(uint32_t), hipMemcpyHostToDevice));
// ... 447 lines not shown

int zr_pass_get_output(const zr_pass* p, int which, void** dev, uint32_t* w, uint32_t* h, uint32_t* bpp)
{
    if (!p || !dev) return Fail(ZR_ERR_INVALID_ARG, "null argument");
    if (!p->initialized) return Fail(ZR_ERR_NOT_INITIALIZED, "pass not initialised");
    if (p->kind == ZR_PASS_SKY && which == ZR_OUT_INSCATTERING)
    {
        if (!p->inscatterOn) return Fail(ZR_ERR_INVALID_ARG, "SKY pass: inscattering is disabled (zr_pass_set_inscattering)");
        *dev = p->inscatterGrid.p;
        if (w) *w = p->inscatter.numVoxelsX;
        if (h) *h = p->inscatter.numVoxelsY * kInscatterSlices;
        if (bpp) *bpp = 4;
        return ZR_OK;
    }
    if (p->kind == ZR_PASS_SKY)
    {
        if (which != ZR_OUT_SKY_LUT) return Fail(ZR_ERR_INVALID_ARG, "pass has no such output");
        *dev = p->skyLut.p;
        if (w) *w = p->w;
        if (h) *h = p->h;
        if (bpp) *bpp = 4;
        return ZR_OK;
    }
    if (p->kind == ZR_PASS_AUTO_EXPOSURE)
    {
        if (which == ZR_OUT_EXPOSURE) { *dev = p->aeExposure.p; if (w) *w = 1; if (h) *h = 1; if (bpp) *bpp = 8; return ZR_OK; }
        if (which == ZR_OUT_AE_HISTOGRAM) { *dev = p->aeHist.p; if (w) *w = post::kHistBins; if (h) *h = 1; if (bpp) *bpp = 4; return ZR_OK; }
        return Fail(ZR_ERR_INVALID_ARG, "pass has no such output");
    }
    if (p->kind == ZR_PASS_DISPLAY)
    {
        if (which == ZR_OUT_DISPLAY) { p->displayOut.Output(dev, bpp); if (w) *w = p->w; if (h) *h = p->h; return ZR_OK; }
        if (which == ZR_OUT_DISPLAY_SRGB8) { p->displaySrgb.Output(dev, bpp); if (w) *w = p->w; if (h) *h = p->h; return ZR_OK; }
        if (which == ZR_OUT_PICK_MASK)
        {
            if (!p->pickMaskW) return Fail(ZR_ERR_INVALID_ARG, "DISPLAY: no picked instance has been rendered (zr_pass_set_picked_instances)");
            *dev = p->pickMask.p; if (w) *w = p->pickMaskW; if (h) *h = p->pickMaskH; if (bpp) *bpp = 1; return ZR_OK;
        }
        return Fail(ZR_ERR_INVALID_ARG, "pass has no such output");
    }
    if (p->kind == ZR_PASS_DENOISE)
    {
        if (w) *w = p->w;
        if (h) *h = p->h;
        if (which == ZR_OUT_DENOISED) { *dev = (void*)p->svgfOut; if (bpp) *bpp = (uint32_t)p->svgfPing.bpp; return ZR_OK; }
        if (which == ZR_OUT_DENOISE_HISTORY) { p->svgfHist.Output(dev, bpp); return ZR_OK; }
        if (which == ZR_OUT_DENOISE_MOMENTS) { p->svgfMoments[p->svgfMomIdx].Output(dev, bpp); return ZR_OK; }
        return Fail(ZR_ERR_INVALID_ARG, "pass has no such output");
    }
    if (p->kind == ZR_PASS_TAA)
    {
        if (which != ZR_OUT_TAA) return Fail(ZR_ERR_INVALID_ARG, "pass has no such output");
        p->taaOut[p->taaIdx].Output(dev, bpp);
        if (w) *w = p->w;
        if (h) *h = p->h;
        return ZR_OK;
    }
    if (p->kind == ZR_PASS_COMPOSITING)
    {
        if (which != ZR_OUT_FINAL) return Fail(ZR_ERR_INVALID_ARG, "pass has no such output");
        p->finalRGBA.Output(dev, bpp);
        if (w) *w = p->w;
        if (h) *h = p->h;
        return ZR_OK;
    }
    if (p->kind == ZR_PASS_DI_SKY)
    {
        const int last = 1 - p->currIdx;
        if (which == ZR_OUT_FINAL) p->finalRGBA.Output(dev, bpp);
        else if (which == ZR_OUT_SDI_RESERVOIR_A) p->skyA[last].Output(dev, bpp);
        else if (which == ZR_OUT_SDI_RESERVOIR_B) p->skyB[last].Output(dev, bpp);
        else if (which == ZR_OUT_SDI_RESERVOIR_C) p->skyC[last].Output(dev, bpp);
        else if (which == ZR_OUT_SDI_TARGET) p->diTarget.Output(dev, bpp);
        else return Fail(ZR_ERR_INVALID_ARG, "pass has no such output");
        if (w) *w = p->w;
        if (h) *h = p->h;
        return ZR_OK;
    }
    if (p->kind == ZR_PASS_DI_EMISSIVE)
    {
        const int last = 1 - p->currIdx;
        if (which == ZR_OUT_FINAL) p->finalRGBA.Output(dev, bpp);
        else if (which == ZR_OUT_RDI_RESERVOIR_A) p->diA[last].Output(dev, bpp);
        else if (which == ZR_OUT_RDI_RESERVOIR_B) p->diB[last].Output(dev, bpp);
        else if (which == ZR_OUT_RDI_TARGET) p->diTarget.Output(dev, bpp);
        else return Fail(ZR_ERR_INVALID_ARG, "pass has no such output");
        if (w) *w = p->w;
        if (h) *h = p->h;
        return ZR_OK;
    }
    if (p->kind != ZR_PASS_INDIRECT) return Fail(ZR_ERR_INVALID_ARG, "pass has no such output");
    if (which == ZR_OUT_FINAL) p->FinalPlane(p->finOut).Output(dev, bpp);
    else if (which >= ZR_OUT_RGI_RESERVOIR_A && which <= ZR_OUT_RGI_RESERVOIR_C && p->integrator == ZR_INTEGRATOR_RESTIR_GI)
    {
        const int last = 1 - p->currIdx;
        if (which == ZR_OUT_RGI_RESERVOIR_A) p->giA[last].Output(dev, bpp);
        else if (which == ZR_OUT_RGI_RESERVOIR_B) p->giB[last].Output(dev, bpp);
        else p->giC[last].Output(dev, bpp);
    }
    else if (which >= ZR_OUT_RPT_RBUF_CTN_A && which <= ZR_OUT_RPT_RBUF_NTC_D && p->integrator == ZR_INTEGRATOR_RESTIR_PT)
        PlanesOutput(p->rb[(which - ZR_OUT_RPT_RBUF_CTN_A) / 4], (which - ZR_OUT_RPT_RBUF_CTN_A) % 4, dev, bpp);
    else if ((which == ZR_OUT_RPT_THREAD_MAP_CTN || which == ZR_OUT_RPT_THREAD_MAP_NTC) && p->integrator == ZR_INTEGRATOR_RESTIR_PT)
        p->rptMap[which - ZR_OUT_RPT_THREAD_MAP_CTN].Output(dev, bpp);
    else if (which >= ZR_OUT_RPT_RESERVOIR_A && which <= ZR_OUT_RPT_NEIGHBOR && p->integrator == ZR_INTEGRATOR_RESTIR_PT)
    {
        if (which <= ZR_OUT_RPT_RESERVOIR_G) PlanesOutput(p->RptOth(), which - ZR_OUT_RPT_RESERVOIR_A, dev, bpp);
        else if (which == ZR_OUT_RPT_TARGET) p->TargetPlane().Output(dev, bpp);
        else p->rptNeighbor.Output(dev, bpp);
    }
    else return Fail(ZR_ERR_INVALID_ARG, "pass has no such output");
    if (w) *w = p->w;
    if (h) *h = p->h;
    return ZR_OK;
}
int zr_pass_download_output(const zr_pass* p, int which, void* stream, void* dst, size_t bytes)
{
    void* dev = nullptr; uint32_t w, h, bpp;
    int r = zr_pass_get_output(p, which, &dev, &w, &h, &bpp);
    if (r) return r;
    if (!dst || bytes != (size_t)w * h * bpp) return Fail(ZR_ERR_INVALID_ARG, "destination must hold %zu bytes", (size_t)w * h * bpp);
    HIP_TRY(hipSetDevice(p->device));
    HIP_TRY(hipStreamSynchronize((hipStream_t)stream));
    HIP_TRY(hipMemcpy(dst, dev, bytes, hipMemcpyDeviceToHost));
    return ZR_OK;
}
int zr_pass_enable_cost_map(zr_pass* p, int enable)
{
    if (!p || !p->initialized) return Fail(ZR_ERR_NOT_INITIALIZED, "pass not initialised");
    if (p->kind != ZR_PASS_INDIRECT || p->integrator != ZR_INTEGRATOR_RESTIR_PT) return Fail(ZR_ERR_UNSUPPORTED, "the cost map is an output of the ReSTIR PT pass");
    p->costOn = enable != 0;
    p->costRays = enable == ZR_COST_MAP_RAYS;
    return ZR_OK;
}
int zr_scene_material_class(const zr_scene* s, uint32_t* out)
{
    if (!s || !out) return Fail(ZR_ERR_INVALID_ARG, "zr_scene_material_class: null argument");
    *out = s->plainMaterials.load() ? 1u : 0u;
    return ZR_OK;
}
int zr_debug_set_material_class_kernels(int enable) { g_materialClassKernels.store(enable != 0, std::memory_order_relaxed); return ZR_OK; }
int zr_debug_set_bvh_depth_cap(uint32_t levels) { DeviceBvhSetDepthCap(levels); return ZR_OK; }
int zr_debug_set_large_scene_nodes(uint32_t n) { g_largeSceneNodes.store(n ? n : kLargeSceneNodes, std::memory_order_relaxed); return ZR_OK; }
int zr_pass_debug_trip_stats(zr_pass* p, uint64_t out[3])
{
    if (!p || !out) return Fail(ZR_ERR_INVALID_ARG, "null argument");
    out[0] = out[1] = out[2] = 0;
    if (!p->tripStats.p) return ZR_OK;
    HIP_TRY(hipDeviceSynchronize());
    unsigned long long h[4];
    HIP_TRY(hipMemcpy(h, p->tripStats.p, 32, hipMemcpyDeviceToHost));
    out[0] = h[0]; out[1] = h[1]; out[2] = h[2];
    return ZR_OK;
}
int zr_pass_read_cost_map(zr_pass* p, void* stream, uint32_t* out, uint32_t cells_w, uint32_t cells_h, int reset)
{
    if (!p || !out || !p->initialized) return Fail(ZR_ERR_INVALID_ARG, "zr_pass_read_cost_map: bad argument");
    const uint32_t cw = (p->w + 31u) / 32u + 1u, ch = (p->h + 31u) / 32u + 1u;
    if (!p->costMap.p || cells_w != cw || cells_h != ch) return Fail(ZR_ERR_INVALID_ARG, "the cost map is %u x %u cells", cw, ch);
    HIP_TRY(hipSetDevice(p->device));
    HIP_TRY(hipMemcpyAsync(out, p->costMap.p, (size_t)cw * ch * 4, hipMemcpyDeviceToHost, (hipStream_t)stream));
    if (reset) HIP_TRY(hipMemsetAsync(p->costMap.p, 0, (size_t)cw * ch * 4, (hipStream_t)stream));
    HIP_TRY(hipStreamSynchronize((hipStream_t)stream));
    return ZR_OK;
}
int zr_pass_read_counters(zr_pass* p, void* stream, zr_counters* out, int reset)
{
    if (!p || !out) return Fail(ZR_ERR_INVALID_ARG, "null argument");
    HIP_TRY(hipSetDevice(p->device));
    out->n_closest = p->hostCounters.n_closest; out->n_shadow = p->hostCounters.n_shadow;
    if ((p->kind == ZR_PASS_INDIRECT || p->kind == ZR_PASS_DI_EMISSIVE || p->kind == ZR_PASS_DI_SKY) && p->initialized)
    {
        unsigned long long c[2 * kCounterSlots];
        HIP_TRY(hipStreamSynchronize((hipStream_t)stream));
        if (p->haveCand) HIP_TRY(hipStreamSynchronize(p->candStream));
        HIP_TRY(hipMemcpy(c, p->counters.p, sizeof(c), hipMemcpyDeviceToHost));
        for (int i = 0; i < kCounterSlots; i++) { out->n_closest += c[2 * i]; out->n_shadow += c[2 * i + 1]; }
        if (reset) { HIP_TRY(hipMemsetAsync(p->counters.p, 0, sizeof(c), (hipStream_t)stream)); HIP_TRY(hipStreamSynchronize((hipStream_t)stream)); }
    }
    if (reset) { p->hostCounters.n_closest = 0; p->hostCounters.n_shadow = 0; }
    return ZR_OK;
}
int zr_pass_read_kernel_counters(zr_pass* p, void* stream, uint32_t max_entries, const char** names, uint64_t* closest, uint64_t* shadow,
    uint32_t* count)
{
    if (!p || !names || !closest || !shadow || !count) return Fail(ZR_ERR_INVALID_ARG, "null argument");
    if ((p->kind != ZR_PASS_INDIRECT && p->kind != ZR_PASS_DI_EMISSIVE && p->kind != ZR_PASS_DI_SKY) || !p->initialized) return Fail(ZR_ERR_NOT_INITIALIZED, "pass has no ray counters or is not initialised");
    HIP_TRY(hipSetDevice(p->device));
    unsigned long long c[2 * kCounterSlots];
    HIP_TRY(hipStreamSynchronize((hipStream_t)stream));
    if (p->haveCand) HIP_TRY(hipStreamSynchronize(p->candStream));
    HIP_TRY(hipMemcpy(c, p->counters.p, sizeof(c), hipMemcpyDeviceToHost));
    uint32_t n = 0;
    for (int i = 0; i < kCounterSlots && n < max_entries; i++)
    {
        if (!kCounterNames[i][0] || (c[2 * i] == 0 && c[2 * i + 1] == 0)) continue;
        names[n] = kCounterNames[i]; closest[n] = c[2 * i]; shadow[n] = c[2 * i + 1]; n++;
    }
    *count = n;
    return ZR_OK;
}
int zr_pass_enable_timing(zr_pass* p, int enable)
{
    if (!p) return Fail(ZR_ERR_INVALID_ARG, "null pass");
    p->timing = enable != 0;
    return ZR_OK;
}
int zr_pass_get_timings(zr_pass* p, uint32_t max_entries, const char** names, float* ms, uint32_t* launches, uint32_t* count)
{
    if (!p || !count) return Fail(ZR_ERR_INVALID_ARG, "null argument");
    HIP_TRY(hipSetDevice(p->device));
    p->timerNames.clear(); p->timerMs.clear(); p->timerLaunches.clear();
    for (int i = 0; i < p->numTimers; i++)
    {
        zr_pass::Timer& t = p->timers[i];
        HIP_TRY(hipEventSynchronize(t.b));
        float dt = 0;
        HIP_TRY(hipEventElapsedTime(&dt, t.a, t.b));
        size_t k = 0;
        for (; k < p->timerNames.size(); k++) if (p->timerNames[k] == t.name) break;
        if (k == p->timerNames.size()) { p->timerNames.push_back(t.name); p->timerMs.push_back(0); p->timerLaunches.push_back(0); }
        p->timerMs[k] += dt; p->timerLaunches[k]++;
    }
    *count = (uint32_t)p->timerNames.size();
    for (uint32_t k = 0; k < *count && k < max_entries; k++)
    {
        if (names) names[k] = p->timerNames[k].c_str();
        if (ms) ms[k] = p->timerMs[k];
        if (launches) launches[k] = p->timerLaunches[k];
    }
    return ZR_OK;
}
int zr_pass_destroy(zr_pass* p)
{
    if (!p) return ZR_OK;
    (void)hipSetDevice(p->device);
    for (auto& t : p->timers) { (void)hipEventDestroy(t.a); (void)hipEventDestroy(t.b); }
    if (p->powerEv) (void)hipEventDestroy(p->powerEv);
    if (p->powerHost) (void)hipHostFree(p->powerHost);
    if (p->overlapStream) { (void)hipStreamSynchronize(p->overlapStream); (void)hipStreamDestroy(p->overlapStream); }
    if (p->evCand) (void)hipEventDestroy(p->evCand);
    if (p->evTemporal) (void)hipEventDestroy(p->evTemporal);
    for (auto& e : p->evDone) if (e) (void)hipEventDestroy(e);
    delete p;
    return ZR_OK;
}

int zr_trace_closest(const zr_scene* sc, void* stream, const float* d_rays, uint32_t n, uint32_t mask, uint32_t* d_hits)
{
    if (!sc || !d_rays || !d_hits) return Fail(ZR_ERR_INVALID_ARG, "null argument");
    if (n == 0) return ZR_OK;
    HIP_TRY(hipSetDevice(sc->device));
    const uint32_t grid = std::min<uint32_t>((n + kBlock - 1) / kBlock, 8192u);
    hipLaunchKernelGGL(k_trace_rays, dim3(grid), dim3(kBlock), 0, (hipStream_t)stream, FrameView(sc, nullptr), (const F4*)d_rays, n, mask, (U4*)d_hits);
    HIP_TRY(hipGetLastError());
    return ZR_OK;
}
int zr_trace_any(const zr_scene* sc, void* stream, const float* d_rays, uint32_t n, uint32_t mask, uint32_t* d_occ)
{
    if (!sc || !d_rays || !d_occ) return Fail(ZR_ERR_INVALID_ARG, "null argument");
    if (n == 0) return ZR_OK;
    HIP_TRY(hipSetDevice(sc->device));
    const uint32_t grid = std::min<uint32_t>((n + kBlock - 1) / kBlock, 8192u);
    hipLaunchKernelGGL(k_trace_rays_any, dim3(grid), dim3(kBlock), 0, (hipStream_t)stream, FrameView(sc, nullptr), (const F4*)d_rays, n, mask, d_occ);
    HIP_TRY(hipGetLastError());
    return ZR_OK;
}

}
```

### zetaray_amd/csrc/zr_kernels.h

```cpp
#pragma once
#include <hip/hip_runtime.h>
#include "zr_stages.h"
#include "zr_rpt.h"

using namespace zr;

static constexpr int kBlock = 256;
#ifndef ZR_RPT_BLOCK
#define ZR_RPT_BLOCK 64
#endif
static constexpr int kRptBlock = ZR_RPT_BLOCK;
#define ZR_WAVES(n) __attribute__((amdgpu_waves_per_eu(n, n)))
#define ZR_WAVES_MIN(n) __attribute__((amdgpu_waves_per_eu(n)))
#ifndef ZR_WAVES_PATHTRACE_N
#define ZR_WAVES_PATHTRACE_N 3
#endif
#ifndef ZR_WAVES_PATHTRACE_LARGE_N
#define ZR_WAVES_PATHTRACE_LARGE_N 4
#endif
#ifndef ZR_WAVES_TEMPORAL_N
#define ZR_WAVES_TEMPORAL_N 4
#endif
#ifndef ZR_WAVES_STC_N
#define ZR_WAVES_STC_N 4
// ... 89 lines not shown
    for (int k = 0; k < 4; k++)
    {
        uint32_t before = 0;
        for (uint32_t w = 0; w < wave; w++) before += sCnt[k][w];
        slot[k] = sBase[k] + before + (uint32_t)__popcll(m[k] & below);
    }
    __syncthreads();
}
__device__ __forceinline__ uint32_t AllocPathAndRaysBlock(uint32_t* outCount, uint32_t* rayList, uint32_t cap, uint32_t* rayCount, bool alive, bool c, bool m, bool sh,
    bool haveSlot = false, uint32_t givenSlot = 0)
{
    uint32_t* const ctr[4] = {haveSlot ? nullptr : outCount, rayCount, rayCount + kCounterStride, rayCount + 2 * kCounterStride};
    const bool want[4] = {!haveSlot && alive, c, m, sh};
    uint32_t s[4];
    AllocSlotsBlock(ctr, want, s);
    const uint32_t slot = haveSlot ? givenSlot : s[0];
    if (c) rayList[s[1]] = slot;
    if (m) rayList[cap + s[2]] = slot;
    if (sh) rayList[2 * cap + s[3]] = slot;
    return slot;
}
__device__ __forceinline__ void RayOfIndex(const uint32_t* rayList, uint32_t cap, uint32_t nC, uint32_t nM, uint32_t j, uint32_t& type, uint32_t& slot)
{
    type = j < nC ? 0u : (j < nC + nM ? 1u : 2u);
    slot = rayList[type * cap + (j - (type == 0 ? 0u : (type == 1 ? nC : nC + nM)))];
}

__device__ __forceinline__ void CountWave(unsigned long long* counter, bool pred)
{
    const uint64_t m = __ballot(pred);
    if (m && __lane_id() == (uint32_t)(__ffsll((long long)m) - 1)) atomicAdd(counter, (unsigned long long)__popcll(m));
}

__device__ __forceinline__ void PixelOfThread(uint32_t tilesX, uint32_t x0, uint32_t y0, uint32_t* x, uint32_t* y)
{
    const uint32_t tile = blockIdx.x;
    const uint32_t tx = tile % tilesX, ty = tile / tilesX;
    const uint32_t wave = threadIdx.x >> 6, lane = threadIdx.x & 63u;
    *x = x0 + tx * 16u + (wave & 1u) * 8u + (lane & 7u);
    *y = y0 + ty * 16u + (wave >> 1) * 8u + (lane >> 3);
}

template<int B>
__device__ __forceinline__ void TileWaveLaneB(uint32_t* tile, uint32_t* wave, uint32_t* lane)
{
    if (B == 256) { *tile = blockIdx.x; *wave = threadIdx.x >> 6; *lane = threadIdx.x & 63u; }
    else if (B == 128) { *tile = blockIdx.x >> 1; *wave = ((blockIdx.x & 1u) << 1) | (threadIdx.x >> 6); *lane = threadIdx.x & 63u; }
    else { *tile = blockIdx.x >> 2; *wave = blockIdx.x & 3u; *lane = threadIdx.x; }
}
__device__ __forceinline__ void RptTileWaveLane(uint32_t* tile, uint32_t* wave, uint32_t* lane) { TileWaveLaneB<kRptBlock>(tile, wave, lane); }
template<int B>
__device__ __forceinline__ void PixelOfThreadB(uint32_t tilesX, uint32_t x0, uint32_t y0, uint32_t* x, uint32_t* y)
{
    uint32_t tile, wave, lane; TileWaveLaneB<B>(&tile, &wave, &lane);
    const uint32_t tx = tile % tilesX, ty = tile / tilesX;
    *x = x0 + tx * 16u + (wave & 1u) * 8u + (lane & 7u);
    *y = y0 + ty * 16u + (wave >> 1) * 8u + (lane >> 3);
}
#ifndef ZR_RGI_BLOCK
#define ZR_RGI_BLOCK 64
#endif
static constexpr int kRgiBlock = ZR_RGI_BLOCK;

__device__ __forceinline__ void FlushRayCounters(unsigned long long* counters, const uint32_t* cnt)
{
#ifdef ZR_NO_RAY_COUNTERS
    return;
#endif
    uint32_t a = cnt[0], b = cnt[1];
    for (int s = 1; s < 64; s <<= 1) { a += __shfl_xor(a, s); b += __shfl_xor(b, s); }
    if (__lane_id() == 0)
    {
        if (a) atomicAdd(counters + 0, (unsigned long long)a);
        if (b) atomicAdd(counters + 1, (unsigned long long)b);
    }
}

__device__ __forceinline__ void FlushRayCountersCost(const rpt::RptFrame& F, unsigned long long* counters, const uint32_t* cnt, uint32_t x, uint32_t y, bool inFrame,
    unsigned long long t0)
{
    if (F.costMap != nullptr)
    {
        const uint64_t m = __ballot(inFrame);
        if (m != 0)
        {
            const int leader = __ffsll((long long)m) - 1;
            unsigned long long dt = (__builtin_readcyclecounter() - t0) >> 4;
            if (F.costMode)
            {
                uint32_t r = cnt[0] + cnt[1];
                for (int s = 1; s < 64; s <<= 1) r += __shfl_xor(r, s);
                dt = r;
            }
            if ((int)__lane_id() == leader && dt) atomicAdd(&F.costMap[((y - F.gb.y0) >> 5) * F.costW + ((x - F.gb.x0) >> 5)], (uint32_t)(dt > 0xffffffull ? 0xffffffull : dt));
        }
    }
    FlushRayCounters(counters, cnt);
}

template<bool EMISSIVE, bool TEX, bool NODE_CACHE = false, bool PARK = false, bool PLAIN = false, bool VIEW = false>
__device__ __forceinline__ void RptPathtraceBody(rpt::RptFrame& F, const zr_frame_constants& g, uint32_t tilesX, unsigned long long* counters, uint32_t view = 0)
{
    const unsigned long long t0 = __builtin_readcyclecounter();
    F.prm.emissive = EMISSIVE ? 1u : 0u; F.prm.textured = TEX ? 1u : 0u;
    rpt::SetMaterialClass(F, PLAIN);
    uint32_t tile, wave, lane; RptTileWaveLane(&tile, &wave, &lane);
    const uint32_t tx = tile % tilesX, ty = tile / tilesX;
    const uint32_t x = F.ox0 + tx * 16u + (lane & 15u), y = F.oy0 + ty * 16u + wave * 4u + (lane >> 4);
    ZR_TRAV_STACK_B(stack, kRptBlock);
    if (NODE_CACHE) { ZR_NODE_CACHE_FILL(stack, F.sc, kRptBlock); }
#if ZR_SCENE_LDS
    else { ZR_SCENE_CACHE_FILL(stack, F.sc, kRptBlock); }
#endif
    ZR_PROF_KERNEL(F.sc, 1);
    uint32_t cnt[2] = {0u, 0u};
    rpt::PTLane P;
    { ZR_PROF_SCOPE(ZRP_MISC0); rpt::PtInitLane_Fused(F.sc, g, F.gb, F.prm, F.Owns(x, y), x, y, F.finalRGBA, stack, cnt, P); }
    __shared__ uint32_t rcParkLds[PARK ? rpt::kRcParkWords * kRptBlock : 1];
    if (PARK) { P.r.park.p = (ZR_LDS_AS uint32_t*)rcParkLds + threadIdx.x; P.r.park.stride = kRptBlock; P.r.parked = false; }
    for (;;)
    {
        const bool any = __ballot(P.active) != 0;
        rpt::PtPhaseA_Fused(F.sc, g, F.prm, stack, cnt, P);
        if (!any) break;
        uint32_t key = rpt::PtRRKey(P);
        if (__ballot(key != 0) != 0)
        {
            for (int s = 1; s < 64; s <<= 1) { uint32_t o = __shfl_xor(key, s); key = o > key ? o : key; }
        }
        { ZR_PROF_SCOPE(ZRP_MISC1); rpt::PtPhaseB(F.sc, F.prm, P, key); }
    }
    { ZR_PROF_SCOPE(ZRP_MISC2); rpt::PtFinishLane<VIEW>(F.gb, F.prm, F.cur, F.tex, F.finalRGBA, P, view); }
    FlushRayCountersCost(F, counters, cnt, x, y, F.Owns(x, y), t0);
}
template<bool EMISSIVE, bool PLAIN = false>
__global__ void __launch_bounds__(kRptBlock) ZR_WAVES_PATHTRACE k_rpt_pathtrace(rpt::RptFrame F, zr_frame_constants g, uint32_t tilesX, unsigned long long* counters)
{ RptPathtraceBody<EMISSIVE, false, false, false, PLAIN>(F, g, tilesX, counters); }
template<bool EMISSIVE, bool PLAIN = false>
__global__ void __launch_bounds__(kRptBlock) ZR_WAVES_PATHTRACE_LARGE k_rpt_pathtrace_w4(rpt::RptFrame F, zr_frame_constants g, uint32_t tilesX, unsigned long long* counters)
{ RptPathtraceBody<EMISSIVE, false, true, false, PLAIN>(F, g, tilesX, counters); }
#ifndef ZR_WAVES_PATHTRACE_TEX
#define ZR_WAVES_PATHTRACE_TEX ZR_WAVES(6)
#endif
template<bool EMISSIVE>
__global__ void __launch_bounds__(kRptBlock) ZR_WAVES_PATHTRACE_TEX k_rpt_pathtrace_tex(rpt::RptFrame F, zr_frame_constants g, uint32_t tilesX, unsigned long long* counters)
{ RptPathtraceBody<EMISSIVE, true>(F, g, tilesX, counters); }

#ifdef ZR_EXPERIMENTS
#include "zr_kernels_exp.h"
#endif

enum RptPixelPass { RPT_REPLAY_CTT = 0, RPT_REPLAY_TTC, RPT_RECONNECT_TEMPORAL, RPT_SPATIAL_SEARCH, RPT_REPLAY_CTS, RPT_REPLAY_STC };

static constexpr uint32_t kLightTilesPerBlock = 4, kSearchTilesPerBlock = 2;
template<int PASS>
__global__ void __launch_bounds__(kBlock) k_rpt_light(rpt::RptFrame F, zr_frame_constants g, uint32_t tilesX, uint32_t* listA, uint32_t* listB, uint32_t* counts)
{
    constexpr uint32_t TPB = PASS == 0 ? kLightTilesPerBlock : (PASS == 1 ? kSearchTilesPerBlock : 1u);
    constexpr uint32_t VW = TPB * (uint32_t)(kBlock / 64);
    const uint32_t numTiles = tilesX * ((F.oh + 15u) / 16u);
    const uint32_t wave = threadIdx.x >> 6, lane = threadIdx.x & 63u;
    uint32_t a[TPB], b[TPB], pid[TPB];
    __shared__ uint32_t sCnt[2][3][VW], sBase[2];
    for (uint32_t t = 0; t < TPB; t++)
    {
        const uint32_t tile = blockIdx.x * TPB + t;
        const uint32_t tx = tile % tilesX, ty = tile / tilesX;
        const uint32_t x = F.ox0 + tx * 16u + (wave & 1u) * 8u + (lane & 7u), y = F.oy0 + ty * 16u + (wave >> 1) * 8u + (lane >> 3);
        const bool in = tile < numTiles && F.Owns(x, y);
        a[t] = 0; b[t] = 0;
        if (PASS == 0)
        {
            if (in) { a[t] = rpt::NeedsReplayCtT(F, x, y); b[t] = rpt::NeedsReplayTtC(F, g, x, y); }
        }
        else
        {
            if (PASS == 2)
            {
                constexpr int R = rpt::kSearchRadius, T = 16 + 2 * R;
                __shared__ uint16_t tMr[T * T]; __shared__ float tDepth[T * T]; __shared__ uint32_t tNormal[T * T];
                const uint32_t tx0 = F.ox0 + tx * 16u, ty0 = F.oy0 + ty * 16u;
                for (uint32_t i = threadIdx.x; i < (uint32_t)(T * T); i += kBlock)
                {
                    const int gx = (int)tx0 - R + (int)(i % T), gy = (int)ty0 - R + (int)(i / T);
                    const bool ok = gx >= 0 && gy >= 0 && gx < (int)g.render_width && gy < (int)g.render_height && rpt::InPlanes(F.gb, gx, gy);
                    const size_t sp = ok ? rpt::Pix(F.gb, (uint32_t)gx, (uint32_t)gy) : 0;
                    tMr[i] = ok ? F.gb.mr[sp] : (uint16_t)0; tDepth[i] = ok ? F.gb.depth[sp] : 0.0f; tNormal[i] = ok ? F.gb.normal[sp] : 0u;
                }
                __syncthreads();
                struct TileFetch
                {
                    const uint16_t* mr; const float* depth; const uint32_t* normal; int x0, y0;
                    __device__ void operator()(int sx, int sy, uint16_t& m, float& d, uint32_t& n) const
                    { const int i = (sy - y0) * T + (sx - x0); m = mr[i]; d = depth[i]; n = normal[i]; }
                } tf{tMr, tDepth, tNormal, (int)tx0 - R, (int)ty0 - R};
                if (in) { rpt::SpatialSearchPixelT(F, g, x, y, tf); a[t] = rpt::NeedsReplayCtS(F, x, y); b[t] = rpt::NeedsReplayStC(F, x, y); }
            }
            else if (in) { rpt::SpatialSearchPixel(F, g, x, y); a[t] = rpt::NeedsReplayCtS(F, x, y); b[t] = rpt::NeedsReplayStC(F, x, y); }
        }
        pid[t] = in ? (uint32_t)rpt::Pix(F.gb, x, y) : 0u;
        for (uint32_t c = 0; c < 3u; c++)
        {
            const uint64_t ma = __ballot(a[t] == c + 1u), mb = __ballot(b[t] == c + 1u);
            if (lane == 0) { sCnt[0][c][t * (kBlock / 64) + wave] = (uint32_t)__popcll(ma); sCnt[1][c][t * (kBlock / 64) + wave] = (uint32_t)__popcll(mb); }
        }
    }
    __syncthreads();
    if (threadIdx.x < 2)
    {
        uint32_t total = 0;
        for (uint32_t c = 0; c < 3u; c++) for (uint32_t w = 0; w < VW; w++) total += sCnt[threadIdx.x][c][w];
        sBase[threadIdx.x] = total ? atomicAdd(counts + threadIdx.x, total) : 0u;
    }
    __syncthreads();
    const uint64_t below = (1ull << lane) - 1ull;
    uint32_t oa = sBase[0], ob = sBase[1];
    for (uint32_t c = 0; c < 3u; c++)
        for (uint32_t t = 0; t < TPB; t++)
        {
            const uint64_t ma = __ballot(a[t] == c + 1u), mb = __ballot(b[t] == c + 1u);
            uint32_t wa = 0, wb = 0, ta = 0, tb = 0;
            for (uint32_t w = 0; w < (uint32_t)(kBlock / 64); w++) { const uint32_t na = sCnt[0][c][t * (kBlock / 64) + w], nb = sCnt[1][c][t * (kBlock / 64) + w]; ta += na; tb += nb; if (w < wave) { wa += na; wb += nb; } }
            if (a[t] == c + 1u) listA[oa + wa + (uint32_t)__popcll(ma & below)] = pid[t];
            if (b[t] == c + 1u) listB[ob + wb + (uint32_t)__popcll(mb & below)] = pid[t];
            oa += ta; ob += tb;
        }
}

template<int PASS, bool EMISSIVE, bool TEX>
__device__ __forceinline__ void RptReplayPixel(rpt::RptFrame& F, const zr_frame_constants& g, uint32_t pid, const TravStack& stack, uint32_t* cnt)
{
    const uint32_t x = F.gb.x0 + pid % F.gb.w, y = F.gb.y0 + pid / F.gb.w;
    const uint32_t before = cnt[0] + cnt[1];
    if (PASS == RPT_REPLAY_CTT) rpt::ReplayTemporalPixel(F, g, 0, x, y, stack, cnt);
    else if (PASS == RPT_REPLAY_TTC) rpt::ReplayTemporalPixel(F, g, 1, x, y, stack, cnt);
    else if (PASS == RPT_REPLAY_CTS) rpt::ReplaySpatialPixel(F, g, 0, x, y, stack, cnt);
    else rpt::ReplaySpatialPixel(F, g, 1, x, y, stack, cnt);
    if (F.costMap != nullptr && F.costMode && cnt[0] + cnt[1] != before) atomicAdd(&F.costMap[((y - F.gb.y0) >> 5) * F.costW + ((x - F.gb.x0) >> 5)], cnt[0] + cnt[1] - before);
}
template<int PASS, bool EMISSIVE, bool TEX, bool DYNAMIC>
__device__ __forceinline__ void RptReplayList(rpt::RptFrame& F, const zr_frame_constants& g, const uint32_t* list, uint32_t n, uint32_t* cursor,
    unsigned long long* counters, uint32_t block, uint32_t numBlocks, const TravStack& stack)
{
    uint32_t cnt[2] = {0u, 0u};
    if (DYNAMIC)
    {
        const uint32_t lane = threadIdx.x & 63u;
        const uint32_t chunk = n < 128u * gridDim.x * (blockDim.x / 64u) ? 64u : 128u;
        for (; n != 0;)
        {
            uint32_t base = 0;
            if (lane == 0) base = atomicAdd(cursor, chunk);
            base = __shfl(base, 0);
            if (base >= n) break;
            if (base + lane < n) RptReplayPixel<PASS, EMISSIVE, TEX>(F, g, list[base + lane], stack, cnt);
            if (chunk == 128u && base + 64u + lane < n) RptReplayPixel<PASS, EMISSIVE, TEX>(F, g, list[base + 64u + lane], stack, cnt);
        }
    }
    else
        for (uint32_t i = block * blockDim.x + threadIdx.x; i < n; i += numBlocks * blockDim.x) RptReplayPixel<PASS, EMISSIVE, TEX>(F, g, list[i], stack, cnt);
    if (n) FlushRayCounters(counters, cnt);
}
#ifndef ZR_WAVES_REPLAY_N
#define ZR_WAVES_REPLAY_N 4
#endif
#define ZR_WAVES_REPLAY __attribute__((amdgpu_waves_per_eu(ZR_WAVES_REPLAY_N, ZR_WAVES_REPLAY_N)))
static constexpr uint32_t kReplayPersistentBlocks = 256u * ZR_WAVES_REPLAY_N;
template<int PASS_A, bool EMISSIVE, bool TEX>
__global__ void __launch_bounds__(kBlock) ZR_WAVES_REPLAY k_rpt_replay(rpt::RptFrame F, zr_frame_constants g, const uint32_t* listA, const uint32_t* listB, uint32_t* counts,
    unsigned long long* counters)
{
    F.prm.emissive = EMISSIVE ? 1u : 0u; F.prm.textured = TEX ? 1u : 0u;
    rpt::SetMaterialClass(F, false);
    ZR_TRAV_STACK(stack);
#ifdef ZR_NODE_CACHE_MORE
    ZR_NODE_CACHE_FILL(stack, F.sc, kBlock);
#endif
    if (PASS_A == RPT_REPLAY_CTT)
    {
        RptReplayList<PASS_A, EMISSIVE, TEX, true>(F, g, listA, counts[0], counts + 4, counters, 0, 0, stack);
        RptReplayList<PASS_A + 1, EMISSIVE, TEX, true>(F, g, listB, counts[1], counts + 5, counters + 2, 0, 0, stack);
    }
    else
    {
        const uint32_t half = gridDim.x / 2u;
        if (blockIdx.x < half) RptReplayList<PASS_A, EMISSIVE, TEX, false>(F, g, listA, counts[0], nullptr, counters, blockIdx.x, half, stack);
        else RptReplayList<PASS_A + 1, EMISSIVE, TEX, false>(F, g, listB, counts[1], nullptr, counters + 2, blockIdx.x - half, half, stack);
    }
}

template<int VARIANT>
__device__ __forceinline__ void RptSortTile(const rpt::RptFrame& F, const zr_frame_constants& g, uint32_t tile, uint32_t tilesX, uint32_t tile0x, uint32_t tile0y, uint16_t* map)
{
    const uint32_t W = g.render_width, H = g.render_height, dimX = (W + 31u) / 32u, dimY = (H + 31u) / 32u;
    const uint32_t gx = tile0x + tile % tilesX, gy = tile0y + tile / tilesX;
    const uint32_t gidx = threadIdx.x, wave = gidx >> 6, lane = gidx & 63u;
    const bool againstEdge = gx == dimX - 1u || gy == dimY - 1u, lastGroup = gx == dimX - 1u && gy == dimY - 1u;
    uint32_t cls[4], res[4], px[4], py[4], gtx[4], gty[4];
    for (int i = 0; i < 4; i++)
    {
        gtx[i] = (gidx & 15u) * 2u + (uint32_t)(i & 1); gty[i] = (gidx >> 4) * 2u + (uint32_t)(i >> 1);
        px[i] = gx * 32u + gtx[i]; py[i] = gy * 32u + gty[i];
        cls[i] = rpt::SortClassify(F, g, VARIANT, px[i], py[i], againstEdge, res[i]);
    }
    __shared__ uint32_t sCnt[4][5];
    const uint64_t lt = (1ull << lane) - 1ull;
    uint32_t lanePrefix[5];
    for (uint32_t c = 0; c < 5u; c++)
    {
        uint32_t n = 0, pre = 0;
        for (int i = 0; i < 4; i++) { const uint64_t m = __ballot(cls[i] == c); n += (uint32_t)__popcll(m); pre += (uint32_t)__popcll(m & lt); }
        lanePrefix[c] = pre;
        if (lane == 0) sCnt[wave][c] = n;
    }
    __syncthreads();
    uint32_t base[5], run = 0;
    for (uint32_t c = 0; c < 5u; c++)
    {
        uint32_t before = 0, total = 0;
        for (uint32_t w = 0; w < 4u; w++) { const uint32_t n = sCnt[w][c]; total += n; if (w < wave) before += n; }
        base[c] = run + before; run += total;
    }
    const bool spatialResample = F.prm.doSpatial != 0;
    for (int i = 0; i < 4; i++)
    {
        uint32_t mgx = gtx[i], mgy = gty[i];
        if (!lastGroup)
        {
            uint32_t in2x2 = 0;
            for (int j = 0; j < i; j++) in2x2 += cls[j] == cls[i] ? 1u : 0u;
            uint32_t b = base[4], lp = lanePrefix[4];
            for (uint32_t c = 0; c < 4u; c++) if (cls[i] == c) { b = base[c]; lp = lanePrefix[c]; }
            const uint32_t idx = b + lp + in2x2;
            mgx = idx & 31u; mgy = idx >> 5;
        }
        if (gx == dimX - 1u && gy != dimY - 1u) { const uint32_t t = mgx; mgx = mgy; mgy = t; }
        const uint32_t mx = gx * 32u + mgx, my = gy * 32u + mgy;
        if (mx < W && my < H && rpt::InPlanes(F.gb, (int)mx, (int)my))
            map[rpt::Pix(F.gb, mx, my)] = rpt::EncodeSorted(px[i], py[i], mx, my, rpt::SortErrorBits(VARIANT, res[i], spatialResample));
    }
}

template<int VA, int VB>
__global__ void __launch_bounds__(256) k_rpt_sort(rpt::RptFrame F, zr_frame_constants g, uint32_t tilesX, uint32_t tile0x, uint32_t tile0y, uint16_t* mapA, uint16_t* mapB)
{
    const uint32_t half = gridDim.x / 2u;
    if (blockIdx.x < half) RptSortTile<VA>(F, g, blockIdx.x, tilesX, tile0x, tile0y, mapA);
    else RptSortTile<VB>(F, g, blockIdx.x - half, tilesX, tile0x, tile0y, mapB);
}

#ifndef ZR_RECON_BLOCK
#define ZR_RECON_BLOCK 256
#endif
static constexpr int kReconBlock = ZR_RECON_BLOCK;
#ifndef ZR_STC_BLOCK
#define ZR_STC_BLOCK ZR_RECON_BLOCK
#endif
#ifndef ZR_STC_LDS
#define ZR_STC_LDS 0
#endif
static constexpr int kStcBlock = ZR_STC_BLOCK;
#ifndef ZR_VOTE_WT_STC
#define ZR_VOTE_WT_STC 2
#endif

template<bool EMISSIVE, bool TEX, bool PLAIN = false>
__global__ void __launch_bounds__(kReconBlock) ZR_WAVES_TEMPORAL k_rpt_temporal(rpt::RptFrame F, zr_frame_constants g, uint32_t tilesX, unsigned long long* counters)
{
    const unsigned long long t0 = __builtin_readcyclecounter();
    F.prm.emissive = EMISSIVE ? 1u : 0u; F.prm.textured = TEX ? 1u : 0u;
    rpt::SetMaterialClass(F, PLAIN);
    uint32_t x, y; PixelOfThreadB<kReconBlock>(tilesX, F.ox0, F.oy0, &x, &y);
    if (F.prm.temporalMap && F.Owns(x, y)) { const uint16_t e = (F.prm.temporalMap == 1u ? F.mapCtN : F.mapNtC)[rpt::Pix(F.gb, x, y)]; rpt::DecodeSorted(e & 0x7fffu, x, y); }
    ZR_TRAV_STACK_B(stack, kReconBlock);
#if ZR_SCENE_LDS
    ZR_SCENE_CACHE_FILL(stack, F.sc, kReconBlock);
#endif
    ZR_PROF_KERNEL(F.sc, 2);
    uint32_t cnt[2] = {0u, 0u};
    if (F.Owns(x, y)) rpt::ReconnectTemporalPixel(F, g, x, y, stack, cnt);
    FlushRayCountersCost(F, counters, cnt, x, y, F.Owns(x, y), t0);
}

__device__ __forceinline__ float WaveSumButterfly(float v)
{
    for (int s = 1; s < 64; s <<= 1) v = v + __shfl_xor(v, s);
    return v;
}

template<bool EMISSIVE, bool TEX, bool PLAIN = false>
__global__ void __launch_bounds__(kStcBlock) ZR_WAVES_STC k_rpt_stc(rpt::RptFrame F, zr_frame_constants g, uint32_t tilesX, unsigned long long* counters)
{
    const unsigned long long t0 = __builtin_readcyclecounter();
    F.prm.emissive = EMISSIVE ? 1u : 0u; F.prm.textured = TEX ? 1u : 0u;
    rpt::SetMaterialClass(F, PLAIN);
    uint32_t x, y; PixelOfThreadB<kStcBlock>(tilesX, F.ox0, F.oy0, &x, &y);
    if (F.prm.sortSpatial && F.Owns(x, y) && !rpt::DecodeSorted(F.mapNtC[rpt::Pix(F.gb, x, y)], x, y)) x = 0xffffffffu;
    ZR_TRAV_STACK_B(stack, kStcBlock);
    stack.voteTri = ZR_VOTE_WT_STC;
#if ZR_SCENE_LDS
    ZR_SCENE_CACHE_FILL(stack, F.sc, kStcBlock);
#endif
    uint32_t cnt[2] = {0u, 0u};
    ZR_PROF_KERNEL(F.sc, 3);
#if ZR_STC_LDS
    __shared__ __attribute__((aligned(16))) uint32_t stcLaneLds[kStcBlock * ((sizeof(rpt::StcLane) + 15) / 16 * 4)];
    rpt::StcLane& a = *reinterpret_cast<rpt::StcLane*>(stcLaneLds + threadIdx.x * ((sizeof(rpt::StcLane) + 15) / 16 * 4));
    a.r_curr.park.p = nullptr; a.r_curr.park.stride = 0; a.r_curr.parked = false; a.r_spatial.park.p = nullptr; a.r_spatial.park.stride = 0; a.r_spatial.parked = false;
#else
    rpt::StcLane a;
    if (!PLAIN) ZR_KEEP_IN_MEMORY(a);
#endif
    float v1, v2, v3, v4;
    { ZR_PROF_SCOPE(ZRP_MISC0); rpt::StcPhase0(F, g, x, y, a, v1, v2); }
    { ZR_PROF_SCOPE(ZRP_MISC1);
    if (a.valid && a.hasN) rpt::ReconnectCtSPixel(F, g, x, y, stack, cnt); }
    const float sum1 = WaveSumButterfly(v1), sum2 = WaveSumButterfly(v2);
    rpt::StcPhase1(F, g, a, sum1, v3);
    const float sum3 = WaveSumButterfly(v3);
    ZR_PROF_SCOPE(ZRP_MISC2);
    rpt::StcPhase2(F, g, a, sum1, stack, cnt, v4);
    const float sum4 = WaveSumButterfly(v4);
    rpt::StcPhase3(F, g, a, sum2 + sum3 + sum4);
    FlushRayCountersCost(F, counters, cnt, x, y, x != 0xffffffffu && F.Owns(x, y), t0);
}

template<bool EMISSIVE, bool TEX>
__global__ void __launch_bounds__(kRptBlock) __attribute__((amdgpu_waves_per_eu(TEX ? 6 : ZR_WAVES_PATHTRACE_LARGE_N, TEX ? 6 : ZR_WAVES_PATHTRACE_LARGE_N)))
k_rpt_pathtrace_view(rpt::RptFrame F, zr_frame_constants g, uint32_t tilesX, unsigned long long* counters, uint32_t view)
{ RptPathtraceBody<EMISSIVE, TEX, !TEX, false, false, true>(F, g, tilesX, counters, view); }
template<bool EMISSIVE, bool TEX>
__global__ void __launch_bounds__(kReconBlock) ZR_WAVES(ZR_WAVES_TEMPORAL_N) k_rpt_temporal_view(rpt::RptFrame F, zr_frame_constants g, uint32_t tilesX, unsigned long long* counters, uint32_t view)
{
    const unsigned long long t0 = __builtin_readcyclecounter();
    F.prm.emissive = EMISSIVE ? 1u : 0u; F.prm.textured = TEX ? 1u : 0u;
    rpt::SetMaterialClass(F, false);
    uint32_t x, y; PixelOfThreadB<kReconBlock>(tilesX, F.ox0, F.oy0, &x, &y);
    if (F.prm.temporalMap && F.Owns(x, y)) { const uint16_t e = (F.prm.temporalMap == 1u ? F.mapCtN : F.mapNtC)[rpt::Pix(F.gb, x, y)]; rpt::DecodeSorted(e & 0x7fffu, x, y); }
    ZR_TRAV_STACK_B(stack, kReconBlock);
#if ZR_SCENE_LDS
    ZR_SCENE_CACHE_FILL(stack, F.sc, kReconBlock);
#endif
    ZR_PROF_KERNEL(F.sc, 2);
    uint32_t cnt[2] = {0u, 0u};
    if (F.Owns(x, y)) rpt::ReconnectTemporalPixel<true>(F, g, x, y, stack, cnt, view);
    FlushRayCountersCost(F, counters, cnt, x, y, F.Owns(x, y), t0);
}
template<bool EMISSIVE, bool TEX>
__global__ void __launch_bounds__(kStcBlock) ZR_WAVES(ZR_WAVES_STC_N) k_rpt_stc_view(rpt::RptFrame F, zr_frame_constants g, uint32_t tilesX, unsigned long long* counters, uint32_t view)
{
    const unsigned long long t0 = __builtin_readcyclecounter();
    F.prm.emissive = EMISSIVE ? 1u : 0u; F.prm.textured = TEX ? 1u : 0u;
    rpt::SetMaterialClass(F, false);
    uint32_t x, y; PixelOfThreadB<kStcBlock>(tilesX, F.ox0, F.oy0, &x, &y);
    if (F.prm.sortSpatial && F.Owns(x, y) && !rpt::DecodeSorted(F.mapNtC[rpt::Pix(F.gb, x, y)], x, y)) x = 0xffffffffu;
    ZR_TRAV_STACK_B(stack, kStcBlock);
    stack.voteTri = ZR_VOTE_WT_STC;
#if ZR_SCENE_LDS
    ZR_SCENE_CACHE_FILL(stack, F.sc, kStcBlock);
#endif
    uint32_t cnt[2] = {0u, 0u};
    ZR_PROF_KERNEL(F.sc, 3);
#if ZR_STC_LDS
    __shared__ __attribute__((aligned(16))) uint32_t stcLaneLds[kStcBlock * ((sizeof(rpt::StcLane) + 15) / 16 * 4)];
    rpt::StcLane& a = *reinterpret_cast<rpt::StcLane*>(stcLaneLds + threadIdx.x * ((sizeof(rpt::StcLane) + 15) / 16 * 4));
    a.r_curr.park.p = nullptr; a.r_curr.park.stride = 0; a.r_curr.parked = false; a.r_spatial.park.p = nullptr; a.r_spatial.park.stride = 0; a.r_spatial.parked = false;
#else
    rpt::StcLane a;
    ZR_KEEP_IN_MEMORY(a);
#endif
    float v1, v2, v3, v4;
    { ZR_PROF_SCOPE(ZRP_MISC0); rpt::StcPhase0(F, g, x, y, a, v1, v2); }
    { ZR_PROF_SCOPE(ZRP_MISC1);
    if (a.valid && a.hasN) rpt::ReconnectCtSPixel(F, g, x, y, stack, cnt); }
    const float sum1 = WaveSumButterfly(v1), sum2 = WaveSumButterfly(v2);
    rpt::StcPhase1<true>(F, g, a, sum1, v3, view);
    const float sum3 = WaveSumButterfly(v3);
    ZR_PROF_SCOPE(ZRP_MISC2);
    rpt::StcPhase2<true>(F, g, a, sum1, stack, cnt, v4, view);
    const float sum4 = WaveSumButterfly(v4);
    rpt::StcPhase3<true>(F, g, a, sum2 + sum3 + sum4, view);
    FlushRayCountersCost(F, counters, cnt, x, y, x != 0xffffffffu && F.Owns(x, y), t0);
}


#define ZR_RPT_ARGS_TILE (rpt::RptFrame, zr_frame_constants, uint32_t, unsigned long long*)
#define ZR_RPT_ARGS_LIST (rpt::RptFrame, zr_frame_constants, const uint32_t*, const uint32_t*, uint32_t*, unsigned long long*)
#define ZR_RPT_GROUP_A(X) \
    X __global__ void k_rpt_pathtrace<true, false> ZR_RPT_ARGS_TILE; X __global__ void k_rpt_pathtrace<false, false> ZR_RPT_ARGS_TILE; \
    X __global__ void k_rpt_pathtrace_w4<true, false> ZR_RPT_ARGS_TILE; X __global__ void k_rpt_pathtrace_w4<false, false> ZR_RPT_ARGS_TILE;
#define ZR_RPT_GROUP_G(X) \
    X __global__ void k_rpt_pathtrace_tex<true> ZR_RPT_ARGS_TILE; X __global__ void k_rpt_pathtrace_tex<false> ZR_RPT_ARGS_TILE; \
    X __global__ void k_rpt_temporal<true, true, false> ZR_RPT_ARGS_TILE; X __global__ void k_rpt_temporal<false, true, false> ZR_RPT_ARGS_TILE;
#define ZR_RPT_GROUP_H(X) \
    X __global__ void k_rpt_temporal<true, false, false> ZR_RPT_ARGS_TILE; X __global__ void k_rpt_temporal<false, false, false> ZR_RPT_ARGS_TILE; \
    X __global__ void k_rpt_stc<true, false, false> ZR_RPT_ARGS_TILE; X __global__ void k_rpt_stc<false, false, false> ZR_RPT_ARGS_TILE;
#define ZR_RPT_GROUP_D(X) \
    X __global__ void k_rpt_stc<true, true, false> ZR_RPT_ARGS_TILE; X __global__ void k_rpt_stc<false, true, false> ZR_RPT_ARGS_TILE;
#define ZR_RPT_GROUP_E(X) \
    X __global__ void k_rpt_pathtrace<true, true> ZR_RPT_ARGS_TILE; X __global__ void k_rpt_pathtrace<false, true> ZR_RPT_ARGS_TILE; \
    X __global__ void k_rpt_pathtrace_w4<true, true> ZR_RPT_ARGS_TILE; X __global__ void k_rpt_pathtrace_w4<false, true> ZR_RPT_ARGS_TILE; \
// ... 25 lines not shown
```

### zetaray_amd/csrc/zr_rpt.h

```cpp
#pragma once
#include "zr_stages.h"

namespace zr {
namespace rpt {

static constexpr float kMaxPlaneDistReuse = 1.0f;
static constexpr float kMaxRoughDiffTemporal = 0.3f;
static constexpr float kMaxRoughDiffSpatial = 0.05f;
static constexpr float kMinNormalSimSpatial = 0.9f;
static constexpr uint32_t kMmaxXkTransmissive = 4, kMmaxXkInMotion = 4;
static constexpr int kNeighborOffset = 32;
#if defined(__HIP_DEVICE_COMPILE__)
#define ZR_KEEP_IN_MEMORY(obj) asm volatile("" :: "v"(&(obj)) : "memory")
#else
#define ZR_KEEP_IN_MEMORY(obj) ((void)0)
#endif
#ifndef ZR_PIN_TEMPORAL
#define ZR_PIN_TEMPORAL 0
#endif
#ifndef ZR_PREP_SHIFT
#define ZR_PREP_SHIFT 1
#endif
static constexpr uint32_t kPrepShift = ZR_PREP_SHIFT;
#ifndef ZR_PREP_SHIFT_PLAIN
// ... 2171 lines not shown
    const uint32_t W = g.render_width, H = g.render_height;
    const size_t px = Pix(gb, x, y);
    const uint16_t mrp = gb.mr[px];
    GFlags flags = DecodeFlags(mrp);
    if (flags.invalid || flags.emissive) return;
    const V2 renderDim = v2((float)g.render_width, (float)g.render_height);
    const V2 jitter = v2(g.curr_camera_jitter[0], g.curr_camera_jitter[1]);
    const float roughness = RoughnessOf(mrp);
    const float viewDepth = gb.depth[px];
    const V3 pos = WorldPosSS((float)x, (float)y, renderDim, viewDepth, g.tan_half_fov, g.aspect_ratio, g.curr_view_inv, jitter);
    const V3 normal = DecodeOct32u(gb.normal[px]);
    uint32_t sx = x, sy = y, sz = g.frame_num; zr_pcg3d(&sx, &sy, &sz);
    Rng rng = Rng::Init(sx, sy, g.frame_num);
    const float u0 = rng.Uniform();
    const uint32_t offset = rng.UniformUint();
    const float theta = u0 * ZR_TWO_PI;
    float sinTheta, cosTheta; zr_sincos(theta, &sinTheta, &cosTheta);
    int nx = 0xffff, ny = 0xffff;
    for (uint32_t i = 0; i < 3; i++)
    {
        const uint32_t si = (offset + i) & 511u;
        const float ux = zr_f16_to_f32(F.sampleSet[2 * si]), uy = zr_f16_to_f32(F.sampleSet[2 * si + 1]);
        float rx = ux * cosTheta + uy * -sinTheta, ry = ux * sinTheta + uy * cosTheta;
        rx = rx * (float)kSearchRadius; ry = ry * (float)kSearchRadius;
        const int sxp = (int)__builtin_rintf((float)x + rx), syp = (int)__builtin_rintf((float)y + ry);
        if (sxp < 0 || syp < 0 || sxp >= (int)W || syp >= (int)H) continue;
        if (sxp == (int)x && syp == (int)y) continue;
        if (!InPlanes(gb, sxp, syp)) continue;
        uint16_t smr; float sdepth; uint32_t snormal;
        fetch(sxp, syp, smr, sdepth, snormal);
        GFlags sf = DecodeFlags(smr);
        if (sf.invalid || sf.emissive) continue;
        if (flags.metallic != sf.metallic) continue;
        if (flags.transmissive != sf.transmissive) continue;
        if (zr_abs(RoughnessOf(smr) - roughness) > kMaxRoughDiffSpatial) continue;
        const V3 samplePos = WorldPosSS((float)sxp, (float)syp, renderDim, sdepth, g.tan_half_fov, g.aspect_ratio, g.curr_view_inv, jitter);
        const V3 sampleNormal = DecodeOct32u(snormal);
        float planeDist = zr_abs(dot(normal, samplePos - pos));
        if (!(planeDist <= 0.01f * viewDepth)) continue;
        if (dot(sampleNormal, normal) < kMinNormalSimSpatial) continue;
        nx = sxp; ny = syp;
        break;
    }
    if (nx == 0xffff) { F.tex.neighbor[2 * px] = 255; F.tex.neighbor[2 * px + 1] = 255; }
    else { F.tex.neighbor[2 * px] = (uint8_t)(nx - (int)x + kNeighborOffset); F.tex.neighbor[2 * px + 1] = (uint8_t)(ny - (int)y + kNeighborOffset); }
}

ZR_HD void SpatialSearchPixel(const RptFrame& F, const zr_frame_constants& g, uint32_t x, uint32_t y)
{ PlaneFetch f; f.gb = &F.gb; SpatialSearchPixelT(F, g, x, y, f); }

ZR_HD bool NeighborOf(const RptFrame& F, uint32_t x, uint32_t y, int& sx, int& sy)
{
    const size_t px = Pix(F.gb, x, y);
    if (F.tex.neighbor[2 * px] == 255) return false;
    sx = (int)F.tex.neighbor[2 * px] - kNeighborOffset + (int)x; sy = (int)F.tex.neighbor[2 * px + 1] - kNeighborOffset + (int)y;
    return true;
}

ZR_HD_FLAT void ReplaySpatialPixel(const RptFrame& F, const zr_frame_constants& g, int variant, uint32_t x, uint32_t y, TravStack stack, uint32_t* cnt)
{
    const size_t px = Pix(F.gb, x, y);
    GFlags flags = DecodeFlags(F.gb.mr[px]);
    if (flags.invalid || flags.emissive) return;
    Globals gl = MakeGlobals(F, g, flags.transmissive, stack, cnt);
    const Camera cam = CurrCamera(g);
    int sx, sy;
    if (variant == 0)
    {
        Reservoir r = Load_Metadata(F.cur, px);
        if (!r.rc.Empty() && (r.rc.k > 2))
        {
            r.Load_Reconnection(F.cur, px, F.prm.emissive != 0);
            if (!NeighborOf(F, x, y, sx, sy)) return;
            const size_t sp = Pix(F.gb, (uint32_t)sx, (uint32_t)sy);
            PixelSurface pn = LoadPixelSurface(F.gb, cam, (uint32_t)sx, (uint32_t)sy, g.frame_num, sp);
            OffsetCtx ctx = Replay_kGt2(gl, true, pn.pos, pn.normal, pn.eta_next, pn.surface, r.rc, MakePrimaryDiffs(cam, sx, sy, pn, F.gb, sp));
            WriteOffsetCtx(ctx, F.rbCtN, px, r.rc.IsCase3(), gl.textured);
        }
    }
    else
    {
        if (!NeighborOf(F, x, y, sx, sy)) return;
        const size_t sp = Pix(F.gb, (uint32_t)sx, (uint32_t)sy);
        Reservoir r = Load_Metadata(F.cur, sp);
        if (!r.rc.Empty() && (r.rc.k > 2))
        {
            r.Load_Reconnection(F.cur, sp, F.prm.emissive != 0);
            PixelSurface ps = LoadPixelSurface(F.gb, cam, x, y, g.frame_num, px);
            OffsetCtx ctx = Replay_kGt2(gl, true, ps.pos, ps.normal, ps.eta_next, ps.surface, r.rc, MakePrimaryDiffs(cam, (int)x, (int)y, ps, F.gb, px));
            WriteOffsetCtx(ctx, F.rbNtC, px, r.rc.IsCase3(), gl.textured);
        }
    }
}

ZR_HD uint32_t NeedsReplayCtS(const RptFrame& F, uint32_t x, uint32_t y)
{
    const size_t px = Pix(F.gb, x, y);
    GFlags flags = DecodeFlags(F.gb.mr[px]);
    if (flags.invalid || flags.emissive) return false;
    if (F.tex.neighbor[2 * px] == 255) return false;
    return ReplayClass(F.cur.A[px]);
}
ZR_HD uint32_t NeedsReplayStC(const RptFrame& F, uint32_t x, uint32_t y)
{
    const size_t px = Pix(F.gb, x, y);
    GFlags flags = DecodeFlags(F.gb.mr[px]);
    if (flags.invalid || flags.emissive) return false;
    int sx, sy;
    if (!NeighborOf(F, x, y, sx, sy)) return false;
    return ReplayClass(F.cur.A[Pix(F.gb, (uint32_t)sx, (uint32_t)sy)]);
}

ZR_HD void ReconnectCtSPixel(const RptFrame& F, const zr_frame_constants& g, uint32_t x, uint32_t y, TravStack stack, uint32_t* cnt)
{
    const size_t px = Pix(F.gb, x, y);
    int sx, sy;
    if (!NeighborOf(F, x, y, sx, sy)) return;
    GFlags flags = DecodeFlags(F.gb.mr[px]);
    if (flags.invalid || flags.emissive) return;
    const size_t sp = Pix(F.gb, (uint32_t)sx, (uint32_t)sy);
    Reservoir r_curr = Load_NonReconnection(F.cur, px);
    Reservoir r_spatial = Load_Metadata(F.cur, sp);
    if ((r_curr.w_sum != 0) && !r_curr.rc.Empty())
    {
        r_curr.Load_Reconnection(F.cur, px, F.prm.emissive != 0);
        Globals gl = MakeGlobals(F, g, flags.transmissive, stack, cnt);
        const Camera cam = CurrCamera(g);
        PixelSurface pn = LoadPixelSurface(F.gb, cam, (uint32_t)sx, (uint32_t)sy, g.frame_num, px);
        OffsetPath shift = Shift2(gl, true, px, pn.pos, pn.normal, pn.eta_next, pn.surface, r_curr.rc, F.rbCtN, MakePrimaryDiffs(cam, sx, sy, pn, F.gb, sp));
        float target_spatial = Luminance(shift.target);
        if (target_spatial > 0)
        {
            float targetLum_curr = r_curr.W > 0 ? r_curr.w_sum / r_curr.W : 0;
            float jacobian = r_curr.rc.partialJacobian > 0 ? shift.partialJacobian / r_curr.rc.partialJacobian : 0;
            float numerator = (float)r_curr.M * targetLum_curr;
            float denom = numerator + (float)r_spatial.M * target_spatial * jacobian;
            float m_curr = denom > 0 ? numerator / denom : 0;
            r_curr.w_sum *= m_curr;
        }
        F.prev.B[2 * px] = r_curr.w_sum;
    }
}

enum { RPT_SORT_CTT = 0, RPT_SORT_TTC = 1, RPT_SORT_CTS = 2, RPT_SORT_STC = 3 };
static constexpr uint32_t kSeInvalidPixel = 1, kSeNotFound = 2, kSeEmpty = 4;
ZR_HD uint16_t EncodeSorted(uint32_t x, uint32_t y, uint32_t mx, uint32_t my, uint32_t error)
{ return (uint16_t)(((uint32_t)((int)x - (int)mx + 31)) | (((uint32_t)((int)y - (int)my + 31)) << 7) | ((error ? 1u : 0u) << 15)); }
ZR_HD bool DecodeSorted(uint16_t e, uint32_t& x, uint32_t& y)
{
    if (e & 0x8000u) return false;
    x = (uint32_t)((int)x + (int)(e & 0x3fu) - 31); y = (uint32_t)((int)y + (int)((e >> 7) & 0x3fu) - 31);
    return true;
}
ZR_HD uint32_t SortClassify(const RptFrame& F, const zr_frame_constants& g, int variant, uint32_t x, uint32_t y, bool againstEdge, uint32_t& result)
{
    const uint32_t W = g.render_width, H = g.render_height;
    uint32_t err = 0; int nx = 0, ny = 0;
    if (x >= W || y >= H || !InPlanes(F.gb, (int)x, (int)y)) err = kSeInvalidPixel;
    else
    {
        const size_t px = Pix(F.gb, x, y);
        const GFlags flags = DecodeFlags(F.gb.mr[px]);
        if (flags.invalid || flags.emissive) err = kSeInvalidPixel;
        else if (variant == RPT_SORT_TTC)
        {
            const V2 motionVec = DecodeMotion(F.gb.motion[px]);
            const float rw = (float)W, rh = (float)H;
            const float pu = ((float)x + 0.5f) / rw - motionVec.x, pv = ((float)y + 0.5f) / rh - motionVec.y;
            nx = (int)(pu * rw); ny = (int)(pv * rh);
            if (pu < 0.0f || pv < 0.0f || pu > 1.0f || pv > 1.0f) err = kSeNotFound;
        }
        else if (variant == RPT_SORT_STC)
        {
            const uint32_t ox = F.tex.neighbor[2 * px], oy = F.tex.neighbor[2 * px + 1];
            if (ox == 255u) err = kSeNotFound;
            nx = (int)ox - kNeighborOffset + (int)x; ny = (int)oy - kNeighborOffset + (int)y;
        }
    }
    bool skip = err != 0;
    result = err;
    uint32_t k = Reconnection::EMPTY;
    if (err == 0)
    {
        const bool fromNeighbor = variant == RPT_SORT_TTC || variant == RPT_SORT_STC;
        const int rx = fromNeighbor ? nx : (int)x, ry = fromNeighbor ? ny : (int)y;
        uint32_t a = 0;
        if (rx >= 0 && ry >= 0 && rx < (int)W && ry < (int)H && InPlanes(F.gb, rx, ry))
            a = (variant == RPT_SORT_TTC ? F.prev.A : F.cur.A)[Pix(F.gb, (uint32_t)rx, (uint32_t)ry)];
        const uint32_t kk = a & 0xfu;
        k = kk == Reconnection::EMPTY ? kk : kk + 2u;
    }
    if (k == Reconnection::EMPTY) { result |= kSeEmpty; skip = true; }
    if (skip && againstEdge && x < W && y < H) { result = 0; skip = false; }
    if (skip) return 4u;
    if (k == 2u) return 0u;
    if (k == 3u) return 1u;
    if (k == 4u) return 2u;
    return 3u;
}
ZR_HD uint32_t SortErrorBits(int variant, uint32_t result, bool spatialResample)
{
    if (variant == RPT_SORT_TTC) return result & (spatialResample ? (kSeInvalidPixel | kSeNotFound) : kSeInvalidPixel);
    if (variant == RPT_SORT_STC) return result & kSeInvalidPixel;
    return result & (kSeInvalidPixel | kSeEmpty);
}

struct StcLane
{
    bool valid, hasN, spatialEmpty, resample, changed; size_t px, sp; Reservoir r_curr, r_spatial; uint32_t M_max, M_new; GFlags flags;
    uint32_t x, y; float w_sum_loaded;
};
ZR_HD void StcCopyToNextFrame(const RptFrame& F, size_t px, Reservoir& r, uint32_t M_max)
{
    if (!r.rc.Empty()) { r.Load_Reconnection(F.cur, px, F.prm.emissive != 0); r.Write(F.prev, px, M_max, F.prm.emissive != 0); }
    else r.WriteReservoirData(F.prev, px, M_max);
}
ZR_HD void StcSuppress(float waveAvgExclusive, Reservoir& r)
{ if (r.w_sum > 50 * waveAvgExclusive) { r.M = 0; r.w_sum = 0; r.W = 0; r.rc.Clear(); } }

ZR_HD void StcPhase0(const RptFrame& F, const zr_frame_constants& g, uint32_t x, uint32_t y, StcLane& a, float& s1, float& s2)
{
    a.valid = a.hasN = a.spatialEmpty = a.resample = a.changed = false; a.x = x; a.y = y; s1 = 0; s2 = 0;
    if (!F.Owns(x, y)) return;
    a.px = Pix(F.gb, x, y);
    a.flags = DecodeFlags(F.gb.mr[a.px]);
    if (a.flags.invalid || a.flags.emissive) return;
    a.valid = true;
    a.w_sum_loaded = F.cur.B[2 * a.px];
    int sx, sy;
    a.hasN = NeighborOf(F, x, y, sx, sy);
    if (a.hasN) a.sp = Pix(F.gb, (uint32_t)sx, (uint32_t)sy);
    s1 = a.w_sum_loaded;
    s2 = a.w_sum_loaded * (a.hasN ? 0.0f : 1.0f);
}
template<bool VIEW = false>
ZR_HD void StcPhase1(const RptFrame& F, const zr_frame_constants& g, StcLane& a, float sum1, float& s3, uint32_t view = RPT_VIEW_NONE)
{
    s3 = 0;
    if (!a.valid) return;
    a.r_curr = Load_NonReconnection(F.cur, a.px);
    a.r_curr.target = xyz(F.tex.target[a.px]);
    const float waveAvgExclusive = (sum1 - a.w_sum_loaded) / 64.0f;
    a.M_max = F.prm.M_max_spatial;
    a.M_max = !a.r_curr.rc.Empty() && a.r_curr.rc.lobe_k_min_1 == LOBE_GLOSSY_T ? umin(a.M_max, kMmaxXkTransmissive) : a.M_max;
    if (!a.hasN)
    {
        if (F.prm.boiling) StcSuppress(waveAvgExclusive, a.r_curr);
        WriteOutputColor<VIEW>(g, F.finalRGBA, a.px, a.r_curr.target * a.r_curr.W, view);
        StcCopyToNextFrame(F, a.px, a.r_curr, a.M_max);
        return;
    }
    a.r_spatial = Load_NonReconnection(F.cur, a.sp);
    if ((a.r_curr.w_sum != 0) && (a.r_spatial.M > 0) && !a.r_curr.rc.Empty()) a.r_curr.w_sum = F.prev.B[2 * a.px];
    a.M_new = (a.r_curr.M + a.r_spatial.M) & 0xffffu;
    a.spatialEmpty = a.r_spatial.rc.Empty();
    s3 = a.r_curr.w_sum * (a.spatialEmpty ? 1.0f : 0.0f);
}
template<bool VIEW = false>
ZR_HD void StcPhase2(const RptFrame& F, const zr_frame_constants& g, StcLane& a, float sum1, TravStack stack, uint32_t* cnt, float& s4, uint32_t view = RPT_VIEW_NONE)
{
    s4 = 0;
    if (!a.valid || !a.hasN) return;
    const float waveAvgExclusive = (sum1 - a.w_sum_loaded) / 64.0f;
    if (a.spatialEmpty)
    {
        if (F.prm.boiling) StcSuppress(waveAvgExclusive, a.r_curr);
        float targetLum = Luminance(a.r_curr.target);
        a.r_curr.W = targetLum > 0 ? a.r_curr.w_sum / targetLum : 0;
        a.r_curr.M = a.M_new;
        StcCopyToNextFrame(F, a.px, a.r_curr, a.M_max);
        WriteOutputColor<VIEW>(g, F.finalRGBA, a.px, a.r_curr.target * a.r_curr.W, view);
        return;
    }
    a.resample = true;
    a.M_max = a.r_spatial.rc.x_k_in_motion ? umin(a.M_max, kMmaxXkInMotion) : a.M_max;
    a.r_spatial.rc.x_k_in_motion = false;
    a.r_spatial.Load_Reconnection(F.cur, a.sp, F.prm.emissive != 0);
    Globals gl = MakeGlobals(F, g, a.flags.transmissive, stack, cnt);
    const Camera cam = CurrCamera(g);
    const PixelSurface ps = LoadPixelSurface(F.gb, cam, a.x, a.y, g.frame_num, a.px);
    OffsetPath shift = Shift2(gl, true, a.px, ps.pos, ps.normal, ps.eta_next, ps.surface, a.r_spatial.rc, F.rbNtC,
        MakePrimaryDiffs(cam, (int)a.x, (int)a.y, ps, F.gb, a.px));
    float targetLum_curr = Luminance(shift.target);
    float targetLum_spatial = a.r_spatial.W > 0 ? a.r_spatial.w_sum / a.r_spatial.W : 0;
    float jacobian = a.r_spatial.rc.partialJacobian > 0 ? shift.partialJacobian / a.r_spatial.rc.partialJacobian : 0;
    if (targetLum_curr > 1e-6f && jacobian > 1e-5f && jacobian < 100)
    {
        uint32_t hx = a.x, hy = a.y, hz = a.y; zr_pcg3d(&hx, &hy, &hz);
        Rng rng = Rng::Init(hx, hz, g.frame_num + 511);
        float numerator = (float)a.r_spatial.M * targetLum_spatial;
        float denom = numerator / jacobian + (float)a.r_curr.M * targetLum_curr;
        float m_spatial = denom > 0 ? numerator / denom : 0;
        float w_spatial = m_spatial * a.r_spatial.W * targetLum_curr;
        if (a.r_curr.Update(w_spatial, shift.target, a.r_spatial.rc, rng)) { a.r_curr.rc.partialJacobian = shift.partialJacobian; a.changed = true; }
    }
    float targetLum = Luminance(a.r_curr.target);
    a.r_curr.W = targetLum > 0 ? a.r_curr.w_sum / targetLum : 0;
    a.r_curr.M = a.M_new;
    a.M_max = (a.changed && shift.surfKMin1Transmissive) ? umin(a.M_max, kMmaxXkTransmissive) : a.M_max;
    s4 = a.r_curr.w_sum;
}
template<bool VIEW = false>
ZR_HD void StcPhase3(const RptFrame& F, const zr_frame_constants& g, StcLane& a, float waveSum, uint32_t view = RPT_VIEW_NONE)
{
    if (!a.resample) return;
    if (F.prm.boiling)
    {
        float waveAvgExclusive = (waveSum - a.r_curr.w_sum) / 64.0f;
        StcSuppress(waveAvgExclusive, a.r_curr);
    }
    if (a.changed) a.r_curr.Write(F.prev, a.px, a.M_max, F.prm.emissive != 0);
    else StcCopyToNextFrame(F, a.px, a.r_curr, a.M_max);
    V3 li = a.r_curr.target * a.r_curr.W;
    if (VIEW) DebugColor(a.r_curr.rc, view, li);
    WriteOutputColor<VIEW>(g, F.finalRGBA, a.px, li, view, false);
}

ZR_HD float ButterflySum64(float* v)
{
    for (int s = 1; s < 64; s <<= 1)
    {
        float t[64];
        for (int i = 0; i < 64; i++) t[i] = v[i] + v[i ^ s];
        for (int i = 0; i < 64; i++) v[i] = t[i];
    }
    return v[0];
}

}
}
```

Measured before the change: 5257 Mrays/s.

## Fuse replay list classification into sort prepass and merge spatial search launch

The separate k_rpt_light classification kernels are removed. Replay work lists are now built inside the sort kernels, which already read the reservoir A plane and G-buffer flags. The spatial search runs as extra blocks in the temporal prepass launch. When the TtC map will later be overwritten by the spatial sort, writing it is skipped. This cuts kernel launches and repeated per-pixel reads, but it moves the spatial search earlier in the schedule and changes the order of list entries. A debug readback for the replay lists is added.

```diff
diff --git a/include/zetaray_amd.h b/include/zetaray_amd.h
--- a/include/zetaray_amd.h
+++ b/include/zetaray_amd.h
@@ -301,6 +301,7 @@
 int zr_pass_enable_cost_map(zr_pass* pass, int enable);
 int zr_pass_read_cost_map(zr_pass* pass, void* hip_stream, uint32_t* out_cells, uint32_t cells_w, uint32_t cells_h, int reset);
 int zr_pass_debug_trip_stats(zr_pass* pass, uint64_t out[3]);
+int zr_pass_debug_read_replay_lists(zr_pass* pass, uint32_t counts[4], uint32_t* ids, size_t ids_per_list);
 int zr_debug_set_large_scene_nodes(uint32_t num_nodes);
 int zr_debug_set_bvh_depth_cap(uint32_t levels);
 int zr_debug_set_material_class_kernels(int enable);
diff --git a/zetaray_amd/api.py b/zetaray_amd/api.py
--- a/zetaray_amd/api.py
+++ b/zetaray_amd/api.py
@@ -40,7 +40,7 @@
     "zr_abi_version", "zr_last_error", "zr_device_count", "zr_device_probe_run", "zr_wire_layout", "zr_scene_create", "zr_scene_destroy", "zr_scene_update_instances", "zr_scene_update_emissives", "zr_scene_invalidate_alias_table", "zr_scene_update_materials",
     "zr_scene_set_background_rebuild", "zr_scene_background_rebuild_stats",
     "zr_scene_invalidate_alias_table_deferred", "zr_scene_update_instances_async", "zr_scene_update_emissives_async", "zr_scene_update_materials_async", "zr_scene_set_alias_table_async",
-    "zr_scene_set_alias_table", "zr_alias_table_build", "zr_scene_get_alias_table", "zr_scene_get_light_voxel_grid", "zr_scene_get_presampled_sets", "zr_scene_bvh_info", "zr_pass_enable_cost_map", "zr_pass_read_cost_map", "zr_pass_debug_trip_stats", "zr_debug_set_large_scene_nodes", "zr_debug_set_bvh_depth_cap", "zr_debug_set_material_class_kernels", "zr_scene_material_class",
+    "zr_scene_set_alias_table", "zr_alias_table_build", "zr_scene_get_alias_table", "zr_scene_get_light_voxel_grid", "zr_scene_get_presampled_sets", "zr_scene_bvh_info", "zr_pass_enable_cost_map", "zr_pass_read_cost_map", "zr_pass_debug_trip_stats", "zr_pass_debug_read_replay_lists", "zr_debug_set_large_scene_nodes", "zr_debug_set_bvh_depth_cap", "zr_debug_set_material_class_kernels", "zr_scene_material_class",
     "zr_gbuffer_create", "zr_gbuffer_destroy", "zr_gbuffer_set_tile_origin", "zr_gbuffer_download", "zr_gbuffer_device_plane",
     "zr_params_default", "zr_pass_create", "zr_pass_init", "zr_pass_resize", "zr_pass_reset_temporal", "zr_pass_pick_pixel", "zr_pass_clear_pick", "zr_pass_read_pick",
     "zr_pass_set_params", "zr_pass_render", "zr_pass_get_output", "zr_pass_download_output",
@@ -486,6 +486,14 @@
         _check(lib().zr_pass_debug_trip_stats(self.h, out))
         return int(out[0]), int(out[1]), int(out[2])
 
+    def debug_read_replay_lists(self):
+        cap = self.w * self.h_
+        counts = (C.c_uint32 * 4)()
+        ids = np.zeros((4, cap), np.uint32)
+        lib().zr_pass_debug_read_replay_lists.argtypes = [C.c_void_p, C.c_void_p, C.c_void_p, C.c_size_t]
+        _check(lib().zr_pass_debug_read_replay_lists(self.h, counts, ids.ctypes.data, cap))
+        return [ids[l, :int(counts[l])].copy() for l in range(4)]
+
     def read_counters(self, reset=True, stream=None):
         c = wire.Counters()
         _check(lib().zr_pass_read_counters(self.h, stream, C.addressof(c), int(reset)))
diff --git a/zetaray_amd/csrc/zr_api.hip b/zetaray_amd/csrc/zr_api.hip
--- a/zetaray_amd/csrc/zr_api.hip
+++ b/zetaray_amd/csrc/zr_api.hip
@@ -774,6 +774,7 @@
     bool frameOpen = false;
     DevBuf<uint32_t> costMap; bool costOn = false, costRays = false;
     DevBuf<uint32_t> rptLists, rptListCounts;
+    uint32_t rptSpatialCnt = 2;
     Plane<U4> diA[2]; Plane<float, 2> diB[2]; Plane<F4> diTarget; DevBuf<uint16_t> diSampleSet;
     Plane<uint8_t> skyA[2]; Plane<uint16_t, 2> skyB[2]; Plane<float, 2> skyC[2];
     Plane<F4> giA[2], giC[2]; Plane<uint16_t, 4> giB[2];
@@ -2436,7 +2437,6 @@
     const size_t cap = (size_t)p->w * p->h;
     uint32_t* lists[4] = {p->rptLists.p, p->rptLists.p + cap, p->rptLists.p + 2 * cap, p->rptLists.p + 3 * cap};
     const dim3 gridList((uint32_t)std::min<size_t>((cap + kBlock - 1) / kBlock, 1024));
-    const dim3 gridLight((tilesX * tilesY + kLightTilesPerBlock - 1u) / kLightTilesPerBlock), gridSearch((tilesX * tilesY + kSearchTilesPerBlock - 1u) / kSearchTilesPerBlock);
     const dim3 gridReplay((uint32_t)std::min<size_t>((cap + kBlock - 1) / kBlock, kReplayPersistentBlocks));
     unsigned long long* ctr = p->counters.p;
 #define RPT_TIMED(name, ...) do { TimerBegin(p, s, name); __VA_ARGS__; TimerEnd(p, s); } while (0)
@@ -2527,10 +2527,14 @@
         if (p->overlap && p->haveCand && p->candStream != s) HIP_TRY(hipStreamWaitEvent(s, p->evCand, 0));
         else if (int ar = GBufferAcquireRead(gb, s)) return ar;
         HIP_TRY(hipMemsetAsync(listCnt, 0, kRptListWords * sizeof(uint32_t), s));
+        p->rptSpatialCnt = 2;
         if (prm.doTemporal)
         {
-            RPT_TIMED("rpt_sort_temporal", hipLaunchKernelGGL((k_rpt_sort<rpt::RPT_SORT_TTC, rpt::RPT_SORT_CTT>), dim3(gridSort.x * 2), dim3(256), 0, s, F, *cb, sortTilesX, F.ox0 / 32u, F.oy0 / 32u, F.mapNtC, F.mapCtN));
-            RPT_TIMED("rpt_classify_temporal", hipLaunchKernelGGL(k_rpt_light<0>, gridLight, block, 0, s, F, *cb, tilesX, lists[0], lists[1], listCnt + 0));
+            const bool ttcMapDead = (stages & ZR_STAGE_SPATIAL) && prm.doSpatial && prm.sortSpatial && prm.temporalMap != 2u;
+            const uint32_t searchBlocks = prm.doSpatial ? grid.x : 0u;
+            const dim3 gridPre(searchBlocks + gridSort.x * 2u);
+            if (ttcMapDead) RPT_TIMED("rpt_sort_temporal", hipLaunchKernelGGL(k_rpt_prepass_temporal<false>, gridPre, dim3(256), 0, s, F, *cb, searchBlocks, tilesX, gridSort.x, sortTilesX, F.ox0 / 32u, F.oy0 / 32u, lists[0], lists[1], listCnt + 0));
+            else RPT_TIMED("rpt_sort_temporal", hipLaunchKernelGGL(k_rpt_prepass_temporal<true>, gridPre, dim3(256), 0, s, F, *cb, searchBlocks, tilesX, gridSort.x, sortTilesX, F.ox0 / 32u, F.oy0 / 32u, lists[0], lists[1], listCnt + 0));
             RPT_TIMED("rpt_replay_temporal", RPT_LAUNCH_PE(k_rpt_replay, RPT_REPLAY_CTT, gridReplay, block, 0, s, F, *cb, lists[0], lists[1], listCnt + 0, ctr + 2 * 2));
             if (view != ZR_RPT_VIEW_NONE) RPT_TIMED("rpt_reconnect_temporal", RPT_LAUNCH_VIEW(k_rpt_temporal_view, gridRecon, blockRecon, 0, s, F, *cb, tilesX, ctr + 2 * 4));
             else RPT_TIMED("rpt_reconnect_temporal", RPT_LAUNCH_E(k_rpt_temporal, gridRecon, blockRecon, 0, s, F, *cb, tilesX, ctr + 2 * 4));
@@ -2543,16 +2547,9 @@
         if (!(stages & (spass == 0 ? ZR_STAGE_SPATIAL : ZR_STAGE_SPATIAL2))) continue;
         F.cur = p->RptCur().View(); F.prev = p->RptOth().View();
         uint32_t* const sCnt = listCnt + (spass == 0 ? 2 : 6);
-#ifdef ZR_EXPERIMENTS
-        static const bool searchTile = [] { const char* e = getenv("ZR_SEARCH"); return e && !strcmp(e, "tile"); }();
-        if (searchTile) RPT_TIMED("rpt_spatial_search", hipLaunchKernelGGL(k_rpt_light<2>, grid, block, 0, s, F, *cb, tilesX, lists[2], lists[3], sCnt));
-        else
-#endif
-        RPT_TIMED("rpt_spatial_search", hipLaunchKernelGGL(k_rpt_light<1>, gridSearch, block, 0, s, F, *cb, tilesX, lists[2], lists[3], sCnt));
-        if (prm.sortSpatial)
-        {
-            RPT_TIMED("rpt_sort_spatial", hipLaunchKernelGGL((k_rpt_sort<rpt::RPT_SORT_CTS, rpt::RPT_SORT_STC>), dim3(gridSort.x * 2), dim3(256), 0, s, F, *cb, sortTilesX, F.ox0 / 32u, F.oy0 / 32u, F.mapCtN, F.mapNtC));
-        }
+        p->rptSpatialCnt = spass == 0 ? 2u : 6u;
+        if (prm.sortSpatial) RPT_TIMED("rpt_sort_spatial", hipLaunchKernelGGL(k_rpt_prepass_spatial<true>, dim3(gridSort.x * 2), dim3(256), 0, s, F, *cb, sortTilesX, F.ox0 / 32u, F.oy0 / 32u, lists[2], lists[3], sCnt));
+        else RPT_TIMED("rpt_sort_spatial", hipLaunchKernelGGL(k_rpt_prepass_spatial<false>, dim3(gridSort.x * 2), dim3(256), 0, s, F, *cb, sortTilesX, F.ox0 / 32u, F.oy0 / 32u, lists[2], lists[3], sCnt));
         RPT_TIMED("rpt_replay_spatial", RPT_LAUNCH_PE(k_rpt_replay, RPT_REPLAY_CTS, dim3(gridList.x * 2), block, 0, s, F, *cb, lists[2], lists[3], sCnt, ctr + 2 * 5));
         if (view != ZR_RPT_VIEW_NONE) RPT_TIMED("rpt_reconnect_spatial", RPT_LAUNCH_VIEW(k_rpt_stc_view, gridStc, blockStc, 0, s, F, *cb, tilesX, ctr + 2 * 7));
         else RPT_TIMED("rpt_reconnect_spatial", RPT_LAUNCH_E(k_rpt_stc, gridStc, blockStc, 0, s, F, *cb, tilesX, ctr + 2 * 7));
@@ -3306,6 +3303,25 @@
     out[0] = h[0]; out[1] = h[1]; out[2] = h[2];
     return ZR_OK;
 }
+int zr_pass_debug_read_replay_lists(zr_pass* p, uint32_t counts[4], uint32_t* ids, size_t ids_per_list)
+{
+    if (!p || !counts || !ids || !p->initialized) return Fail(ZR_ERR_INVALID_ARG, "zr_pass_debug_read_replay_lists: bad argument");
+    if (p->kind != ZR_PASS_INDIRECT || p->integrator != ZR_INTEGRATOR_RESTIR_PT || !p->rptLists.p) return Fail(ZR_ERR_UNSUPPORTED, "the replay work lists belong to the ReSTIR PT pass");
+    const size_t cap = (size_t)p->w * p->h;
+    if (ids_per_list < cap) return Fail(ZR_ERR_INVALID_ARG, "zr_pass_debug_read_replay_lists: room for %zu ids per list needed", cap);
+    HIP_TRY(hipSetDevice(p->device));
+    HIP_TRY(hipDeviceSynchronize());
+    uint32_t h[kRptListWords];
+    HIP_TRY(hipMemcpy(h, p->rptListCounts.p, sizeof(h), hipMemcpyDeviceToHost));
+    const uint32_t at[4] = {0u, 1u, p->rptSpatialCnt, p->rptSpatialCnt + 1u};
+    for (int l = 0; l < 4; l++)
+    {
+        counts[l] = h[at[l]];
+        if (counts[l] > cap) return Fail(ZR_ERR_HIP, "replay work list %d holds %u entries, more than the planes have pixels", l, counts[l]);
+        if (counts[l]) HIP_TRY(hipMemcpy(ids + (size_t)l * ids_per_list, p->rptLists.p + (size_t)l * cap, (size_t)counts[l] * sizeof(uint32_t), hipMemcpyDeviceToHost));
+    }
+    return ZR_OK;
+}
 int zr_pass_read_cost_map(zr_pass* p, void* stream, uint32_t* out, uint32_t cells_w, uint32_t cells_h, int reset)
 {
     if (!p || !out || !p->initialized) return Fail(ZR_ERR_INVALID_ARG, "zr_pass_read_cost_map: bad argument");
diff --git a/zetaray_amd/csrc/zr_kernels.h b/zetaray_amd/csrc/zr_kernels.h
--- a/zetaray_amd/csrc/zr_kernels.h
+++ b/zetaray_amd/csrc/zr_kernels.h
@@ -265,79 +265,12 @@
 
 enum RptPixelPass { RPT_REPLAY_CTT = 0, RPT_REPLAY_TTC, RPT_RECONNECT_TEMPORAL, RPT_SPATIAL_SEARCH, RPT_REPLAY_CTS, RPT_REPLAY_STC };
 
-static constexpr uint32_t kLightTilesPerBlock = 4, kSearchTilesPerBlock = 2;
-template<int PASS>
-__global__ void __launch_bounds__(kBlock) k_rpt_light(rpt::RptFrame F, zr_frame_constants g, uint32_t tilesX, uint32_t* listA, uint32_t* listB, uint32_t* counts)
-{
-    constexpr uint32_t TPB = PASS == 0 ? kLightTilesPerBlock : (PASS == 1 ? kSearchTilesPerBlock : 1u);
-    constexpr uint32_t VW = TPB * (uint32_t)(kBlock / 64);
-    const uint32_t numTiles = tilesX * ((F.oh + 15u) / 16u);
+__device__ __forceinline__ void RptSearchTile(const rpt::RptFrame& F, const zr_frame_constants& g, uint32_t tile, uint32_t tilesX)
+{
     const uint32_t wave = threadIdx.x >> 6, lane = threadIdx.x & 63u;
-    uint32_t a[TPB], b[TPB], pid[TPB];
-    __shared__ uint32_t sCnt[2][3][VW], sBase[2];
-    for (uint32_t t = 0; t < TPB; t++)
-    {
-        const uint32_t tile = blockIdx.x * TPB + t;
-        const uint32_t tx = tile % tilesX, ty = tile / tilesX;
-        const uint32_t x = F.ox0 + tx * 16u + (wave & 1u) * 8u + (lane & 7u), y = F.oy0 + ty * 16u + (wave >> 1) * 8u + (lane >> 3);
-        const bool in = tile < numTiles && F.Owns(x, y);
-        a[t] = 0; b[t] = 0;
-        if (PASS == 0)
-        {
-            if (in) { a[t] = rpt::NeedsReplayCtT(F, x, y); b[t] = rpt::NeedsReplayTtC(F, g, x, y); }
-        }
-        else
-        {
-            if (PASS == 2)
-            {
-                constexpr int R = rpt::kSearchRadius, T = 16 + 2 * R;
-                __shared__ uint16_t tMr[T * T]; __shared__ float tDepth[T * T]; __shared__ uint32_t tNormal[T * T];
-                const uint32_t tx0 = F.ox0 + tx * 16u, ty0 = F.oy0 + ty * 16u;
-                for (uint32_t i = threadIdx.x; i < (uint32_t)(T * T); i += kBlock)
-                {
-                    const int gx = (int)tx0 - R + (int)(i % T), gy = (int)ty0 - R + (int)(i / T);
-                    const bool ok = gx >= 0 && gy >= 0 && gx < (int)g.render_width && gy < (int)g.render_height && rpt::InPlanes(F.gb, gx, gy);
-                    const size_t sp = ok ? rpt::Pix(F.gb, (uint32_t)gx, (uint32_t)gy) : 0;
-                    tMr[i] = ok ? F.gb.mr[sp] : (uint16_t)0; tDepth[i] = ok ? F.gb.depth[sp] : 0.0f; tNormal[i] = ok ? F.gb.normal[sp] : 0u;
-                }
-                __syncthreads();
-                struct TileFetch
-                {
-                    const uint16_t* mr; const float* depth; const uint32_t* normal; int x0, y0;
-                    __device__ void operator()(int sx, int sy, uint16_t& m, float& d, uint32_t& n) const
-                    { const int i = (sy - y0) * T + (sx - x0); m = mr[i]; d = depth[i]; n = normal[i]; }
-                } tf{tMr, tDepth, tNormal, (int)tx0 - R, (int)ty0 - R};
-                if (in) { rpt::SpatialSearchPixelT(F, g, x, y, tf); a[t] = rpt::NeedsReplayCtS(F, x, y); b[t] = rpt::NeedsReplayStC(F, x, y); }
-            }
-            else if (in) { rpt::SpatialSearchPixel(F, g, x, y); a[t] = rpt::NeedsReplayCtS(F, x, y); b[t] = rpt::NeedsReplayStC(F, x, y); }
-        }
-        pid[t] = in ? (uint32_t)rpt::Pix(F.gb, x, y) : 0u;
-        for (uint32_t c = 0; c < 3u; c++)
-        {
-            const uint64_t ma = __ballot(a[t] == c + 1u), mb = __ballot(b[t] == c + 1u);
-            if (lane == 0) { sCnt[0][c][t * (kBlock / 64) + wave] = (uint32_t)__popcll(ma); sCnt[1][c][t * (kBlock / 64) + wave] = (uint32_t)__popcll(mb); }
-        }
-    }
-    __syncthreads();
-    if (threadIdx.x < 2)
-    {
-        uint32_t total = 0;
-        for (uint32_t c = 0; c < 3u; c++) for (uint32_t w = 0; w < VW; w++) total += sCnt[threadIdx.x][c][w];
-        sBase[threadIdx.x] = total ? atomicAdd(counts + threadIdx.x, total) : 0u;
-    }
-    __syncthreads();
-    const uint64_t below = (1ull << lane) - 1ull;
-    uint32_t oa = sBase[0], ob = sBase[1];
-    for (uint32_t c = 0; c < 3u; c++)
-        for (uint32_t t = 0; t < TPB; t++)
-        {
-            const uint64_t ma = __ballot(a[t] == c + 1u), mb = __ballot(b[t] == c + 1u);
-            uint32_t wa = 0, wb = 0, ta = 0, tb = 0;
-            for (uint32_t w = 0; w < (uint32_t)(kBlock / 64); w++) { const uint32_t na = sCnt[0][c][t * (kBlock / 64) + w], nb = sCnt[1][c][t * (kBlock / 64) + w]; ta += na; tb += nb; if (w < wave) { wa += na; wb += nb; } }
-            if (a[t] == c + 1u) listA[oa + wa + (uint32_t)__popcll(ma & below)] = pid[t];
-            if (b[t] == c + 1u) listB[ob + wb + (uint32_t)__popcll(mb & below)] = pid[t];
-            oa += ta; ob += tb;
-        }
+    const uint32_t tx = tile % tilesX, ty = tile / tilesX;
+    const uint32_t x = F.ox0 + tx * 16u + (wave & 1u) * 8u + (lane & 7u), y = F.oy0 + ty * 16u + (wave >> 1) * 8u + (lane >> 3);
+    if (F.Owns(x, y)) rpt::SpatialSearchPixel(F, g, x, y);
 }
 
 template<int PASS, bool EMISSIVE, bool TEX>
@@ -402,64 +335,103 @@
     }
 }
 
-template<int VARIANT>
-__device__ __forceinline__ void RptSortTile(const rpt::RptFrame& F, const zr_frame_constants& g, uint32_t tile, uint32_t tilesX, uint32_t tile0x, uint32_t tile0y, uint16_t* map)
+template<int VARIANT, bool MAP>
+__device__ __forceinline__ void RptPrepassTile(const rpt::RptFrame& F, const zr_frame_constants& g, uint32_t tile, uint32_t tilesX, uint32_t tile0x, uint32_t tile0y, uint16_t* map,
+    uint32_t* list, uint32_t* count)
 {
     const uint32_t W = g.render_width, H = g.render_height, dimX = (W + 31u) / 32u, dimY = (H + 31u) / 32u;
     const uint32_t gx = tile0x + tile % tilesX, gy = tile0y + tile / tilesX;
     const uint32_t gidx = threadIdx.x, wave = gidx >> 6, lane = gidx & 63u;
     const bool againstEdge = gx == dimX - 1u || gy == dimY - 1u, lastGroup = gx == dimX - 1u && gy == dimY - 1u;
-    uint32_t cls[4], res[4], px[4], py[4], gtx[4], gty[4];
+    uint32_t cls[4], res[4], rep[4], px[4], py[4], gtx[4], gty[4];
     for (int i = 0; i < 4; i++)
     {
         gtx[i] = (gidx & 15u) * 2u + (uint32_t)(i & 1); gty[i] = (gidx >> 4) * 2u + (uint32_t)(i >> 1);
         px[i] = gx * 32u + gtx[i]; py[i] = gy * 32u + gty[i];
-        cls[i] = rpt::SortClassify(F, g, VARIANT, px[i], py[i], againstEdge, res[i]);
-    }
-    __shared__ uint32_t sCnt[4][5];
+        cls[i] = rpt::SortClassifyReplay(F, g, VARIANT, px[i], py[i], againstEdge, res[i], rep[i]);
+        if (!F.Owns(px[i], py[i])) rep[i] = 0;
+    }
+    __shared__ uint32_t sCnt[4][5], sRep[3][4], sBase;
     const uint64_t lt = (1ull << lane) - 1ull;
     uint32_t lanePrefix[5];
-    for (uint32_t c = 0; c < 5u; c++)
-    {
-        uint32_t n = 0, pre = 0;
-        for (int i = 0; i < 4; i++) { const uint64_t m = __ballot(cls[i] == c); n += (uint32_t)__popcll(m); pre += (uint32_t)__popcll(m & lt); }
-        lanePrefix[c] = pre;
-        if (lane == 0) sCnt[wave][c] = n;
+    if (MAP)
+        for (uint32_t c = 0; c < 5u; c++)
+        {
+            uint32_t n = 0, pre = 0;
+            for (int i = 0; i < 4; i++) { const uint64_t m = __ballot(cls[i] == c); n += (uint32_t)__popcll(m); pre += (uint32_t)__popcll(m & lt); }
+            lanePrefix[c] = pre;
+            if (lane == 0) sCnt[wave][c] = n;
+        }
+    uint32_t pos[4] = {0u, 0u, 0u, 0u};
+    for (uint32_t c = 0; c < 3u; c++)
+    {
+        uint32_t n = 0;
+        for (int i = 0; i < 4; i++) { const uint64_t m = __ballot(rep[i] == c + 1u); if (rep[i] == c + 1u) pos[i] = n + (uint32_t)__popcll(m & lt); n += (uint32_t)__popcll(m); }
+        if (lane == 0) sRep[c][wave] = n;
     }
     __syncthreads();
-    uint32_t base[5], run = 0;
-    for (uint32_t c = 0; c < 5u; c++)
+    if (threadIdx.x == 0)
+    {
+        uint32_t total = 0;
+        for (uint32_t c = 0; c < 3u; c++) for (uint32_t w = 0; w < 4u; w++) total += sRep[c][w];
+        sBase = total ? atomicAdd(count, total) : 0u;
+    }
+    if (MAP)
+    {
+        uint32_t base[5], run = 0;
+        for (uint32_t c = 0; c < 5u; c++)
+        {
+            uint32_t before = 0, total = 0;
+            for (uint32_t w = 0; w < 4u; w++) { const uint32_t n = sCnt[w][c]; total += n; if (w < wave) before += n; }
+            base[c] = run + before; run += total;
+        }
+        const bool spatialResample = F.prm.doSpatial != 0;
+        for (int i = 0; i < 4; i++)
+        {
+            uint32_t mgx = gtx[i], mgy = gty[i];
+            if (!lastGroup)
+            {
+                uint32_t in2x2 = 0;
+                for (int j = 0; j < i; j++) in2x2 += cls[j] == cls[i] ? 1u : 0u;
+                uint32_t b = base[4], lp = lanePrefix[4];
+                for (uint32_t c = 0; c < 4u; c++) if (cls[i] == c) { b = base[c]; lp = lanePrefix[c]; }
+                const uint32_t idx = b + lp + in2x2;
+                mgx = idx & 31u; mgy = idx >> 5;
+            }
+            if (gx == dimX - 1u && gy != dimY - 1u) { const uint32_t t = mgx; mgx = mgy; mgy = t; }
+            const uint32_t mx = gx * 32u + mgx, my = gy * 32u + mgy;
+            if (mx < W && my < H && rpt::InPlanes(F.gb, (int)mx, (int)my))
+                map[rpt::Pix(F.gb, mx, my)] = rpt::EncodeSorted(px[i], py[i], mx, my, rpt::SortErrorBits(VARIANT, res[i], spatialResample));
+        }
+    }
+    __syncthreads();
+    uint32_t off = sBase;
+    for (uint32_t c = 0; c < 3u; c++)
     {
         uint32_t before = 0, total = 0;
-        for (uint32_t w = 0; w < 4u; w++) { const uint32_t n = sCnt[w][c]; total += n; if (w < wave) before += n; }
-        base[c] = run + before; run += total;
-    }
-    const bool spatialResample = F.prm.doSpatial != 0;
-    for (int i = 0; i < 4; i++)
-    {
-        uint32_t mgx = gtx[i], mgy = gty[i];
-        if (!lastGroup)
-        {
-            uint32_t in2x2 = 0;
-            for (int j = 0; j < i; j++) in2x2 += cls[j] == cls[i] ? 1u : 0u;
-            uint32_t b = base[4], lp = lanePrefix[4];
-            for (uint32_t c = 0; c < 4u; c++) if (cls[i] == c) { b = base[c]; lp = lanePrefix[c]; }
-            const uint32_t idx = b + lp + in2x2;
-            mgx = idx & 31u; mgy = idx >> 5;
-        }
-        if (gx == dimX - 1u && gy != dimY - 1u) { const uint32_t t = mgx; mgx = mgy; mgy = t; }
-        const uint32_t mx = gx * 32u + mgx, my = gy * 32u + mgy;
-        if (mx < W && my < H && rpt::InPlanes(F.gb, (int)mx, (int)my))
-            map[rpt::Pix(F.gb, mx, my)] = rpt::EncodeSorted(px[i], py[i], mx, my, rpt::SortErrorBits(VARIANT, res[i], spatialResample));
-    }
-}
-
-template<int VA, int VB>
-__global__ void __launch_bounds__(256) k_rpt_sort(rpt::RptFrame F, zr_frame_constants g, uint32_t tilesX, uint32_t tile0x, uint32_t tile0y, uint16_t* mapA, uint16_t* mapB)
+        for (uint32_t w = 0; w < 4u; w++) { const uint32_t n = sRep[c][w]; total += n; if (w < wave) before += n; }
+        for (int i = 0; i < 4; i++) if (rep[i] == c + 1u) list[off + before + pos[i]] = (uint32_t)rpt::Pix(F.gb, px[i], py[i]);
+        off += total;
+    }
+}
+
+template<bool TTC_MAP>
+__global__ void __launch_bounds__(256) k_rpt_prepass_temporal(rpt::RptFrame F, zr_frame_constants g, uint32_t searchBlocks, uint32_t searchTilesX, uint32_t sortBlocks, uint32_t tilesX,
+    uint32_t tile0x, uint32_t tile0y, uint32_t* listCtT, uint32_t* listTtC, uint32_t* counts)
+{
+    uint32_t b = blockIdx.x;
+    if (b < searchBlocks) { RptSearchTile(F, g, b, searchTilesX); return; }
+    b -= searchBlocks;
+    if (b < sortBlocks) RptPrepassTile<rpt::RPT_SORT_CTT, true>(F, g, b, tilesX, tile0x, tile0y, F.mapCtN, listCtT, counts + 0);
+    else RptPrepassTile<rpt::RPT_SORT_TTC, TTC_MAP>(F, g, b - sortBlocks, tilesX, tile0x, tile0y, F.mapNtC, listTtC, counts + 1);
+}
+template<bool MAPS>
+__global__ void __launch_bounds__(256) k_rpt_prepass_spatial(rpt::RptFrame F, zr_frame_constants g, uint32_t tilesX, uint32_t tile0x, uint32_t tile0y, uint32_t* listCtS, uint32_t* listStC,
+    uint32_t* counts)
 {
     const uint32_t half = gridDim.x / 2u;
-    if (blockIdx.x < half) RptSortTile<VA>(F, g, blockIdx.x, tilesX, tile0x, tile0y, mapA);
-    else RptSortTile<VB>(F, g, blockIdx.x - half, tilesX, tile0x, tile0y, mapB);
+    if (blockIdx.x < half) RptPrepassTile<rpt::RPT_SORT_CTS, MAPS>(F, g, blockIdx.x, tilesX, tile0x, tile0y, F.mapCtN, listCtS, counts + 0);
+    else RptPrepassTile<rpt::RPT_SORT_STC, MAPS>(F, g, blockIdx.x - half, tilesX, tile0x, tile0y, F.mapNtC, listStC, counts + 1);
 }
 
 #ifndef ZR_RECON_BLOCK
diff --git a/zetaray_amd/csrc/zr_rpt.h b/zetaray_amd/csrc/zr_rpt.h
--- a/zetaray_amd/csrc/zr_rpt.h
+++ b/zetaray_amd/csrc/zr_rpt.h
@@ -2347,16 +2347,20 @@
     x = (uint32_t)((int)x + (int)(e & 0x3fu) - 31); y = (uint32_t)((int)y + (int)((e >> 7) & 0x3fu) - 31);
     return true;
 }
-ZR_HD uint32_t SortClassify(const RptFrame& F, const zr_frame_constants& g, int variant, uint32_t x, uint32_t y, bool againstEdge, uint32_t& result)
+ZR_HD uint32_t SortClassifyReplay(const RptFrame& F, const zr_frame_constants& g, int variant, uint32_t x, uint32_t y, bool againstEdge, uint32_t& result, uint32_t& replay)
 {
     const uint32_t W = g.render_width, H = g.render_height;
     uint32_t err = 0; int nx = 0, ny = 0;
+    bool listed = false;
+    replay = 0;
     if (x >= W || y >= H || !InPlanes(F.gb, (int)x, (int)y)) err = kSeInvalidPixel;
     else
     {
         const size_t px = Pix(F.gb, x, y);
         const GFlags flags = DecodeFlags(F.gb.mr[px]);
         if (flags.invalid || flags.emissive) err = kSeInvalidPixel;
+        else if (variant == RPT_SORT_CTT) listed = true;
+        else if (variant == RPT_SORT_CTS) listed = F.tex.neighbor[2 * px] != 255;
         else if (variant == RPT_SORT_TTC)
         {
             const V2 motionVec = DecodeMotion(F.gb.motion[px]);
@@ -2364,12 +2368,14 @@
             const float pu = ((float)x + 0.5f) / rw - motionVec.x, pv = ((float)y + 0.5f) / rh - motionVec.y;
             nx = (int)(pu * rw); ny = (int)(pv * rh);
             if (pu < 0.0f || pv < 0.0f || pu > 1.0f || pv > 1.0f) err = kSeNotFound;
+            listed = err == 0;
         }
         else if (variant == RPT_SORT_STC)
         {
             const uint32_t ox = F.tex.neighbor[2 * px], oy = F.tex.neighbor[2 * px + 1];
             if (ox == 255u) err = kSeNotFound;
             nx = (int)ox - kNeighborOffset + (int)x; ny = (int)oy - kNeighborOffset + (int)y;
+            listed = err == 0;
         }
     }
     bool skip = err != 0;
@@ -2381,7 +2387,10 @@
         const int rx = fromNeighbor ? nx : (int)x, ry = fromNeighbor ? ny : (int)y;
         uint32_t a = 0;
         if (rx >= 0 && ry >= 0 && rx < (int)W && ry < (int)H && InPlanes(F.gb, rx, ry))
+        {
             a = (variant == RPT_SORT_TTC ? F.prev.A : F.cur.A)[Pix(F.gb, (uint32_t)rx, (uint32_t)ry)];
+            if (listed) replay = ReplayClass(a);
+        }
         const uint32_t kk = a & 0xfu;
         k = kk == Reconnection::EMPTY ? kk : kk + 2u;
     }
@@ -2393,6 +2402,8 @@
     if (k == 4u) return 2u;
     return 3u;
 }
+ZR_HD uint32_t SortClassify(const RptFrame& F, const zr_frame_constants& g, int variant, uint32_t x, uint32_t y, bool againstEdge, uint32_t& result)
+{ uint32_t replay; return SortClassifyReplay(F, g, variant, x, y, againstEdge, result, replay); }
 ZR_HD uint32_t SortErrorBits(int variant, uint32_t result, bool spatialResample)
 {
     if (variant == RPT_SORT_TTC) return result & (spatialResample ? (kSeInvalidPixel | kSeNotFound) : kSeInvalidPixel);
```

Measured after the change: 5278 Mrays/s (median of 6 runs). Within noise of the previous version (+0.4%).
